# pxl-th/Trace.jl

Measured on AMD Instinct MI355X. Metric: Mray/s (all bounces), higher is better.
Workload: dtype f32

## Files before the change

trace.jl_amd/csrc/th_host.h:

```cpp
#pragma once
#include <hip/hip_runtime.h>

#include <algorithm>
#include <chrono>
#include <cstdarg>
#include <cstdio>
#include <cstdlib>
#include <cstring>
#include <memory>
#include <string>
#include <thread>
#include <vector>

#pragma GCC visibility push(default)
#include "../../include/tracehip.h"
#pragma GCC visibility pop
#include "th_bvh.h"
#include "th_kernels.h"
#include "th_trace2.h"
#include "th_trace8.h"
#ifdef TRHIP_EXPERIMENTS
#include "th_trace4.h"
#include "th_trace7.h"
#endif
#include "th_trace3c.h"
#include "th_comm.h"

using namespace th;

extern thread_local std::string g_init_error;

struct DevBuf {
    void* p = nullptr;
    size_t bytes = 0;
};

constexpr int kMaxPipes = 8;
struct Pipe {
    hipStream_t st = nullptr, st2 = nullptr;
    hipEvent_t ev_shade = nullptr, ev_any = nullptr, ev_any2 = nullptr, ev_done = nullptr;
    DevBuf q[2][3], sq[3], sq2[3], hits, counters, overflow[2];
};

struct Timer;
struct trhip_ctx {
    int device = 0;
    Timer* active_timer = nullptr;
    hipStream_t stream = nullptr;
    hipStream_t stream2 = nullptr;
    std::string err;
    int num_cu = 256;
    bool count_visits = false;
    bool timing = true;
    uint64_t batch_paths = 0;
    int pipelines = 1;
    Pipe pipes[kMaxPipes];
    uint32_t debug_trace_budget = 0;
    double bvh_device_ms = 0.0;
    int bvh_builder = -1;
    bool film_transpose = false;
    bool occluder_pretest = true;
    int stream2_priority = -1;
    bool leaf_kernel = true;
    int slab_margin_log2 = 14;
    int band_tile_rows = 0;
    uint32_t tiny_scene_prims = 16;
    int film_block = 5;
    bool film_relayout = true;
    bool warned_idle_accelerator = false;
    bool warned_fallback_cliff = false;
    double last_fallback_share = 0.0;
    int any_on_accelerator = -1;
    bool wide4 = true;
    bool leaf_queue = false;
    int node_layout = 0;
    bool film_swizzle = false;
    bool film_tiled = false;
    bool overlap = true;
    int compose_spheres = -1;
    int traversal = 3;
    bool leaf_sorted = false;
    bool film_fused = true;
    uint32_t last_L_layout = 0, last_L_npix = 1, last_L_spp = 1;
    bool trace3_spec = true;
    bool hybrid = true;
    bool trace7_cheap = true;
    DevBuf q[2][3], sq[3], hits, Lbuf, pfilm, counters, sensor, table, film, scratch[4], overflow, wh_L, wh_parent, wh_coef, wh_pdf, wh_flags, occl, film_Lt, surv_list, surv_counts;
    uint64_t last_L_count = 0;
    DevBuf sp_vp[7], sp_Ld, sp_tau, sp_radius, sp_N, sp_phi, sp_M, sp_counts, sp_starts, sp_entries, sp_grid, sp_ldist, sp_snap_M, sp_snap_phi, sp_snap_p, sp_snap_beta;
    DevBuf sp_terms, sp_rec[3], sp_rec_valid, sp_raysnap;
    DevBuf st_terms, st_tags[2], st_frozen, st_counts, st_list[2][2][7];
    int streaming = 0;
    uint32_t stream_budget_shift = 12;
    uint32_t stream_list_cap = 0;
    uint32_t stream_budget_min = 2048;
    uint64_t sppm_batch = 0;
    uint32_t sp_pixels = 0;
    int64_t sp_photons = 0;
    DevBuf film_side;
    DevBuf fdesc;
    DevBuf poison;
    DevBuf cert_cold;
    DevBuf aov_rec;
    DevBuf cb_rc;
    DevBuf ov8[2], fb_list[2], fb_counts[2];
    Comm comm;
};

struct HostPrim {
    uint32_t kind;
    float v[9];
    float n[9];
    uint32_t meta;
    uint32_t sphere_id;
};

inline void release(DevBuf& b);

struct SceneGeometry {
    uint64_t id = 0;
    int max_node_primitives = -1;
    std::vector<MaterialRec> materials;
    std::vector<float> base_colour;
    std::vector<HostPrim> prims;
    std::vector<float> prim_tan, prim_uv;
    std::vector<SphereRec> spheres;
    std::vector<HostAABB> sphere_bounds;
    FlatBVH bvh;
    FlatBVH acc;
    std::vector<uint32_t> occ_slots;
    std::vector<float> occ_boxes;
    DevBuf d_leaf_boxes;
    DevBuf d_nodes, d_prims, d_nrm, d_tan, d_shade, d_spheres, d_materials, d_base_colour, d_wnodes, d_w8nodes, d_w8tris;
    DevBuf d_acc_w4nodes;
    DevBuf d_acc_wnodes, d_acc_prims, d_slot_boxes, d_sphere_boxes, d_sphere_slots, d_sphere_cert;
    SceneGeometry() = default;
    SceneGeometry(const SceneGeometry&) = delete;
    SceneGeometry& operator=(const SceneGeometry&) = delete;
    ~SceneGeometry() {
        for (DevBuf* b : {&d_leaf_boxes, &d_nodes, &d_prims, &d_nrm, &d_tan, &d_shade, &d_spheres, &d_materials, &d_base_colour, &d_wnodes, &d_w8nodes, &d_w8tris, &d_acc_w4nodes, &d_acc_wnodes,
                          &d_acc_prims, &d_slot_boxes, &d_sphere_boxes, &d_sphere_slots, &d_sphere_cert})
            release(*b);
    }
// ... 222 lines not shown
```

trace.jl_amd/csrc/th_kernels.h:

```cpp
#pragma once
#include "th_device.h"

namespace th {

constexpr int kBlock = 256;
constexpr int kStackLds = 32;
constexpr int kStackSpill = 32;

struct PathQueue {
    float4* o;
    float4* d;
    float4* beta;
};
struct ShadowQueue {
    float4* o;
    float4* d;
    float4* c;
};
constexpr int kMaxDepth = 62;
constexpr int kSeg = 32;
constexpr uint32_t kSegGran = 256;
#ifndef TH_CTR_STRIDE
#define TH_CTR_STRIDE 32
#endif
// ... 228 lines not shown
    float tx_min = ((negx ? n1.x : n0.x) - o.x) * inv_d.x;
    float tx_max = ((negx ? n0.x : n1.x) - o.x) * inv_d.x;
    const float ty_min = ((negy ? n1.y : n0.y) - o.y) * inv_d.y;
    const float ty_max = ((negy ? n0.y : n1.y) - o.y) * inv_d.y;
    if (tx_min > ty_max || ty_min > tx_max) return false;
    if (ty_min > tx_min) tx_min = ty_min;
    if (ty_max > tx_max) tx_max = ty_max;
    const float tz_min = ((negz ? n1.z : n0.z) - o.z) * inv_d.z;
    const float tz_max = ((negz ? n0.z : n1.z) - o.z) * inv_d.z;
    if (tx_min > tz_max || tz_min > tx_max) return false;
    if (tz_min > tx_min) tx_min = tz_min;
    if (tz_max < tx_max) tx_max = tz_max;
    return tx_min < t_max && tx_max > 0.0f;
}

template <bool ANY, bool COUNT>
TH_D bool traverse(const DeviceScene& sc, f3 o, f3 d, float t_max, uint32_t (*stk)[kBlock], Hit* hit, uint32_t& n_nodes, uint32_t& n_prims) {
    const f3 inv_d = mk3(1.0f / d.x, 1.0f / d.y, 1.0f / d.z);
    const bool negx = d.x < 0.0f, negy = d.y < 0.0f, negz = d.z < 0.0f;
    uint32_t spill[kStackSpill];
    int sp = 0;
    uint32_t cur = 0;
    bool found = false;
    if (sc.n_nodes == 0) return false;
    const uint32_t tid = threadIdx.x;
    while (true) {
        const float4 n0 = sc.nodes[2 * cur], n1 = sc.nodes[2 * cur + 1];
        if (COUNT) n_nodes++;
        bool pop = true;
        if (slab_test(n0, n1, o, inv_d, negx, negy, negz, t_max)) {
            const uint32_t a = __float_as_uint(n0.w), flags = __float_as_uint(n1.w);
            if ((flags & 3u) == 3u) {
                const uint32_t cnt = flags >> 2;
                for (uint32_t k = 0; k < cnt; ++k) {
                    const uint32_t slot = a + k;
                    const float4 p0 = sc.prims[3 * slot];
                    const uint32_t meta = __float_as_uint(p0.w);
                    if (COUNT) n_prims++;
                    if (meta & PRIM_SPHERE) {
                        SphereHit sh;
                        if (sphere_intersect<false>(sc.spheres[__float_as_uint(p0.x)], o, d, t_max, sh)) {
                            if (ANY) return true;
                            t_max = sh.t;
                            found = true;
                            hit->prim = (int)slot;
                            hit->b1 = hit->b2 = 0.0f;
                        }
                    } else {
                        const float4 p1 = sc.prims[3 * slot + 1], p2 = sc.prims[3 * slot + 2];
                        TriTest tt;
                        if (tri_intersect<!ANY>(mk3(p0.x, p0.y, p0.z), mk3(p1.x, p1.y, p1.z), mk3(p2.x, p2.y, p2.z), o, d, t_max, &tt)) {
                            if (ANY) return true;
                            t_max = tt.t;
                            found = true;
                            hit->prim = (int)slot;
                            hit->b1 = tt.bary.x;
                            hit->b2 = tt.bary.y;
                        }
                    }
                }
            } else {
                const uint32_t axis = flags & 3u;
                const bool neg = axis == 0 ? negx : (axis == 1 ? negy : negz);
                const uint32_t far_child = neg ? cur + 1 : a;
                cur = neg ? a : cur + 1;
                if (sp < kStackLds)
                    stk[sp][tid] = far_child;
                else if (sp < kStackLds + kStackSpill)
                    spill[sp - kStackLds] = far_child;
                sp++;
                pop = false;
            }
        }
        if (pop) {
            if (sp == 0) break;
            sp--;
            cur = sp < kStackLds ? stk[sp][tid] : (sp < kStackLds + kStackSpill ? spill[sp - kStackLds] : 0u);
        }
    }
    if (!ANY) hit->t = t_max;
    return found;
}

template <bool COUNT>
__global__ __launch_bounds__(kBlock) void k_trace_closest(DeviceScene sc, SegQueue q, const float4* __restrict__ ro, const float4* __restrict__ rd, const float* __restrict__ tmax_or_null,
                                                          float4* __restrict__ hits, Counters* ctr) {
    __shared__ uint32_t stk[kStackLds][kBlock];
    __shared__ SegView sv;
    seg_load(q, sv);
    const uint32_t total = sv.prefix[kSeg];
    uint32_t nn = 0, np = 0;
    uint32_t seg = 0;
    for (uint32_t flat = blockIdx.x * kBlock + threadIdx.x; flat < total; flat += gridDim.x * kBlock) {
        uint32_t lb;
        seg_locate_from(sv, flat & ~63u, seg, lb);
        const uint32_t local = lb + (flat & 63u);
        if (local >= sv.count[seg]) continue;
        const uint32_t i = seg_phys(q, seg, local);
        const float4 o4 = ro[i], d4 = rd[i];
        Hit h;
        h.prim = -1;
        h.b1 = h.b2 = 0.0f;
        const float t0 = tmax_or_null ? tmax_or_null[i] : kInf;
        const bool found = traverse<false, COUNT>(sc, mk3(o4.x, o4.y, o4.z), mk3(d4.x, d4.y, d4.z), t0, stk, &h, nn, np);
        hits[i] = make_float4(found ? h.t : kInf, __int_as_float(found ? h.prim : -1), h.b1, h.b2);
    }
    if (ctr) {
        if (blockIdx.x == 0 && threadIdx.x == 0) atomicAdd(&ctr->closest_total, (unsigned long long)seg_total(sv));
        if (COUNT) {
            const unsigned long long sn = wave_sum(nn), spr = wave_sum(np);
            if (lane_id() == 0) {
                atomicAdd(&ctr->nodes_closest, sn);
                atomicAdd(&ctr->prims_closest, spr);
            }
        }
    }
}

template <bool COUNT>
__global__ __launch_bounds__(kBlock) void k_trace_any(DeviceScene sc, SegQueue q, const float4* __restrict__ ro, const float4* __restrict__ rd, const float4* __restrict__ contrib,
                                                      const float* __restrict__ tmax_or_null, float4* __restrict__ L, uint8_t* __restrict__ occluded, Counters* ctr) {
    __shared__ uint32_t stk[kStackLds][kBlock];
    __shared__ SegView sv;
    seg_load(q, sv);
    const uint32_t total = sv.prefix[kSeg];
    uint32_t nn = 0, np = 0;
    uint32_t seg = 0;
    for (uint32_t flat = blockIdx.x * kBlock + threadIdx.x; flat < total; flat += gridDim.x * kBlock) {
        uint32_t lb;
        seg_locate_from(sv, flat & ~63u, seg, lb);
        const uint32_t local = lb + (flat & 63u);
        if (local >= sv.count[seg]) continue;
        const uint32_t i = seg_phys(q, seg, local);
        const float4 o4 = ro[i], d4 = rd[i];
        const float t0 = tmax_or_null ? tmax_or_null[i] : kInf;
        const bool occ = traverse<true, COUNT>(sc, mk3(o4.x, o4.y, o4.z), mk3(d4.x, d4.y, d4.z), t0, stk, nullptr, nn, np);
        if (L) {
            const uint32_t slot = __float_as_uint(o4.w);
            if (!occ) {
                const float4 c = contrib[i];
                float4 l = L[slot];
                l.x += c.x;
                l.y += c.y;
                l.z += c.z;
                L[slot] = l;
            } else {
                const uint32_t poison = __float_as_uint(d4.w);
                if (poison) {
                    float4 l = L[slot];
                    const float nanv = __builtin_nanf("");
                    if (poison & 1u) l.x += nanv;
                    if (poison & 2u) l.y += nanv;
                    if (poison & 4u) l.z += nanv;
                    L[slot] = l;
                }
            }
        } else {
            occluded[i] = occ ? 1 : 0;
        }
    }
    if (ctr) {
        if (blockIdx.x == 0 && threadIdx.x == 0) atomicAdd(&ctr->shadow_total, (unsigned long long)seg_total(sv));
        if (COUNT) {
            const unsigned long long sn = wave_sum(nn), spr = wave_sum(np);
            if (lane_id() == 0) {
                atomicAdd(&ctr->nodes_shadow, sn);
                atomicAdd(&ctr->prims_shadow, spr);
            }
        }
    }
}

template <bool TRI_ONLY = false, bool TAN = true>
TH_D bool rebuild_shading(const DeviceScene& sc, int prim, f3 o, f3 d, Shading& sh, uint32_t& material, const float4* bary = nullptr, f3* fast_r = nullptr) {
    const float4* rec = sc.shade + 8 * (size_t)prim;
    const float4 p0 = rec[0], p1 = rec[1], p2 = rec[2];
    const float4 na = rec[3], nb = rec[4], nc = rec[5];
    const float4 cn = rec[6], cs = rec[7];
    const uint32_t meta = __float_as_uint(p0.w);
    material = meta & PRIM_MATERIAL_MASK;
    if (fast_r) *fast_r = mk3(na.w, nb.w, nc.w);
    if (!TRI_ONLY && (meta & PRIM_SPHERE)) {
        const SphereRec& s = sc.spheres[__float_as_uint(p0.x)];
        SphereHit h;
        if (!sphere_intersect<true>(s, o, d, kInf, h)) return false;
        sh = shade_sphere(s, h, d);
        return true;
    }
    const f3 v0 = mk3(p0.x, p0.y, p0.z), v1 = mk3(p1.x, p1.y, p1.z), v2 = mk3(p2.x, p2.y, p2.z);
    TriTest tt;
    if (bary)
        tt.bary = mk3(bary->z, bary->w, bary->x);
    else if (!tri_intersect<true>(v0, v1, v2, o, d, kInf, &tt))
        return false;
    const bool has_n = (meta & PRIM_HAS_NORMALS) != 0;
    const TriConstants tc{mk3(cn.x, cn.y, cn.z), mk3(cs.x, cs.y, cs.z)};
    const float4* tan = (TAN && sc.tri_tan && (meta & PRIM_HAS_TANGENTS)) ? sc.tri_tan + 3 * (size_t)prim : nullptr;
    sh = shade_triangle(v0, v1, v2, has_n, mk3(na.x, na.y, na.z), mk3(nb.x, nb.y, nb.z), mk3(nc.x, nc.y, nc.z), (meta & PRIM_FLIP) != 0, tt.bary, d, &tc, tan);
    return true;
}
template <int TH_ONE_COPY = 0> __global__ __launch_bounds__(kBlock) void k_shade_constants(float4* __restrict__ shade, const float4* __restrict__ prims, const float4* __restrict__ nrm, const float4* __restrict__ uv, uint32_t n_prims) {
    for (uint32_t k = blockIdx.x * kBlock + threadIdx.x; k < n_prims; k += gridDim.x * kBlock) {
        float4* rec = shade + 8 * (size_t)k;
        const float4 p0 = prims[3 * (size_t)k], p1 = prims[3 * (size_t)k + 1], p2 = prims[3 * (size_t)k + 2];
        rec[0] = p0;
        rec[1] = p1;
        rec[2] = p2;
        for (int j = 0; j < 3; ++j) rec[3 + j] = nrm[3 * (size_t)k + j];
        float4 c6 = make_float4(0.0f, 0.0f, 0.0f, 0.0f), c7 = c6;
        if (!(__float_as_uint(p0.w) & PRIM_SPHERE)) {
            float uvs[6];
            bool has_uv = false;
            if (uv) {
                const float4 a = uv[2 * (size_t)k], b = uv[2 * (size_t)k + 1];
                uvs[0] = a.x, uvs[1] = a.y, uvs[2] = a.z, uvs[3] = a.w, uvs[4] = b.x, uvs[5] = b.y;
                has_uv = b.z != 0.0f;
            }
            const TriConstants tc = triangle_constants(mk3(p0.x, p0.y, p0.z), mk3(p1.x, p1.y, p1.z), mk3(p2.x, p2.y, p2.z), has_uv ? uvs : nullptr);
            c6 = make_float4(tc.n.x, tc.n.y, tc.n.z, 0.0f);
            c7 = make_float4(tc.ss.x, tc.ss.y, tc.ss.z, 0.0f);
        }
        rec[6] = c6;
        rec[7] = c7;
    }
}

#ifndef TH_SHADE_WAVES
#define TH_SHADE_WAVES 4
#endif
struct ShadeStream {
    const uint32_t* tags_in;
    uint32_t* tags_out;
    uint32_t term_stride;
    uint8_t* poison;
};
struct ShadeOut {
    bool want_shadow, want_next;
    float4 so4, sd4, sc4, no4, nd4, nb4;
    uint32_t next_depth;
};
template <bool STREAM, bool FAST, bool TAN = true, bool DIRL = false>
TH_D void shade_vertex(const DeviceScene& sc, const PathQueue& qin, const float4* __restrict__ hits, float4* __restrict__ L, uint32_t i, int depth_fixed, int max_depth,
                       uint32_t hits_have_bary, const ShadeStream& ss, ShadeOut& out) {
    const float4 h4 = hits[i];
    const int prim = __float_as_int(h4.y);
    const float4 o4 = qin.o[i], d4 = qin.d[i], b4 = qin.beta[i];
    const int depth = STREAM ? (int)ss.tags_in[i] : depth_fixed;
    const uint32_t slot = STREAM ? (uint32_t)(depth - 1) * ss.term_stride + __float_as_uint(o4.w) : __float_as_uint(o4.w);
    const f3 o = mk3(o4.x, o4.y, o4.z), d = mk3(d4.x, d4.y, d4.z);
    f3 beta = mk3(b4.x, b4.y, b4.z);
    Shading sh;
    uint32_t material;
    f3 fast_r;
    if (!(rebuild_shading<FAST, TAN>(sc, prim, o, d, sh, material, hits_have_bary ? &h4 : nullptr, &fast_r) && material != PRIM_NO_MATERIAL)) return;
    const LobeSet& bsdf = sc.materials[FAST ? 0u : material].set[1];
    const bool lambert = FAST || bsdf_is_single_lambert(bsdf);
    Lobe lam;
    if (FAST) {
        lam.kind = LOBE_LAMBERT_R;
        lam.type = BSDF_DIFFUSE | BSDF_REFLECTION;
        lam.r[0] = fast_r.x;
        lam.r[1] = fast_r.y;
        lam.r[2] = fast_r.z;
    } else if (lambert) {
        lam = bsdf.lobe[0];
    }
    const uint64_t key = ((uint64_t)__float_as_uint(b4.w) << 32) | (uint64_t)__float_as_uint(d4.w);
    const uint32_t v = (uint32_t)(depth - 1);
    const f3 wo = -d;
    const uint32_t poison = ((isnan_(beta.x) || isinf_(beta.x)) ? 1u : 0u) | ((isnan_(beta.y) || isinf_(beta.y)) ? 2u : 0u) | ((isnan_(beta.z) || isinf_(beta.z)) ? 4u : 0u);
    bool direct_added = false;
    if (sc.n_lights > 0) {
        const int nl = (int)sc.n_lights;
        int ln = (int)__builtin_ceilf(ts_uniform(key, ts_vertex_dim(v, TS_V_LIGHT_PICK)) * (float)nl);
        if (ln > nl) ln = nl;
        if (ln < 1) ln = 1;
        const float light_pdf = 1.0f / (float)nl;
        const LightRec light = nl == 1 ? uniform_load(sc.lights, 0u) : sc.lights[ln - 1];
        const LightSample ls = sample_li<DIRL>(light, sh.p);
        if (ls.pdf > 0.0f && !is_black(ls.radiance)) {
            const f3 f = (lambert ? lambert_bsdf_f(lam, sh, sh.wo, ls.wi) : bsdf_f(bsdf, sh, sh.wo, ls.wi, BSDF_ALL & ~BSDF_SPECULAR)) * fabs_(dot(ls.wi, sh.ns));
            if (!is_black(f)) {
                const f3 fl = f * ls.radiance;
                const f3 Ld1 = splat3(0.0f) + (ls.pdf == 1.0f ? fl : fl / ls.pdf);
                const f3 Ld = light_pdf == 1.0f ? Ld1 : Ld1 / light_pdf;
                const f3 c = beta * Ld;
                const f3 lp = light_target<DIRL>(light, sh.p);
                const f3 dir = lp - sh.p;
                const f3 org = sh.p + 1e-6f * dir;
                const f3 cd = check_direction(dir);
                out.so4 = make_float4(org.x, org.y, org.z, __uint_as_float(slot));
                out.sd4 = make_float4(cd.x, cd.y, cd.z, __uint_as_float(poison));
                out.sc4 = make_float4(c.x, c.y, c.z, 0.0f);
                out.want_shadow = true;
                direct_added = true;
            }
        }
    }
    if (!direct_added && poison && ss.poison) {
        ss.poison[slot] |= (uint8_t)poison;
    } else if (!direct_added && poison) {
        float4 l = L[slot];
        const float nanv = __builtin_nanf("");
        if (poison & 1u) l.x += nanv;
        if (poison & 2u) l.y += nanv;
        if (poison & 4u) l.z += nanv;
        L[slot] = l;
    }
    if (depth < max_depth) {
        const f2 u{ts_uniform(key, ts_vertex_dim(v, TS_V_BSDF_U0)), ts_uniform(key, ts_vertex_dim(v, TS_V_BSDF_U1))};
        const BsdfSample bs = lambert ? lambert_bsdf_sample_f(lam, sh, wo, u) : bsdf_sample_f(bsdf, sh, wo, u, BSDF_ALL);
        if (!(bs.pdf == 0.0f || is_black(bs.f))) {
            beta = beta * (bs.f * fabs_(dot(bs.wi, sh.ns)) / bs.pdf);
            const float by = to_Y(beta);
            bool alive = true;
            if (by < 0.25f) {
                const float cont = jmin(1.0f, by);
                if (ts_uniform(key, ts_vertex_dim(v, TS_V_RR)) > cont)
                    alive = false;
                else
                    beta = beta / cont;
            }
            if (alive) {
                const f3 org = sh.p + 1e-6f * bs.wi;
                const f3 nd = check_direction(bs.wi);
                out.no4 = make_float4(org.x, org.y, org.z, o4.w);
                out.nd4 = make_float4(nd.x, nd.y, nd.z, d4.w);
                out.nb4 = make_float4(beta.x, beta.y, beta.z, b4.w);
                out.next_depth = (uint32_t)(depth + 1);
                out.want_next = true;
            }
        }
    }
}

template <bool STREAM, bool TAN = true, bool DIRL = false>
__global__ __launch_bounds__(kBlock) __attribute__((amdgpu_waves_per_eu(TH_SHADE_WAVES))) void k_shade_path(DeviceScene sc, const DeviceSensor* __restrict__ sep, PathQueue qin, PathQueue qout, ShadowQueue sq, uint32_t cap,
                                                       const float4* __restrict__ hits, float4* __restrict__ L, Counters* ctr, int row, int depth_fixed, int max_depth, uint32_t hits_have_bary,
                                                       ShadeStream ss) {
    __shared__ SegView sv;
    __shared__ uint32_t s_ring[kBlock / 64][128];
    const SegQueue qv{ctr->n_queue[row], cap, 0u};
    seg_load(qv, sv);
    const uint32_t total = sv.prefix[kSeg];
    const uint32_t lane = lane_id(), wv = threadIdx.x >> 6;
    const unsigned long long lt_mask = (1ull << lane) - 1ull;
    const uint32_t seg_out = ((blockIdx.x * kBlock + threadIdx.x) >> 6) % kSeg;
    uint32_t ring_head = 0, ring_cnt = 0;
    auto emit = [&](const ShadeOut& e) {
        uint32_t si, ni;
        wave_compact2(e.want_shadow, &ctr->n_shadow[row][seg_out * kCtrStride], e.want_next, &ctr->n_queue[row + 1][seg_out * kCtrStride], si, ni);
        si += seg_out * cap;
        ni += seg_out * cap;
        if (e.want_shadow) {
            sq.o[si] = e.so4;
            sq.d[si] = e.sd4;
            sq.c[si] = e.sc4;
        }
        if (e.want_next) {
            qout.o[ni] = e.no4;
            qout.d[ni] = e.nd4;
            qout.beta[ni] = e.nb4;
            if (STREAM) ss.tags_out[ni] = e.next_depth;
        }
    };
    uint32_t seg_in = 0;
    for (uint32_t flat = blockIdx.x * kBlock + threadIdx.x; flat < total; flat += gridDim.x * kBlock) {
        uint32_t lb;
        seg_locate_from(sv, flat & ~63u, seg_in, lb);
        const uint32_t local = lb + (flat & 63u);
        const uint32_t i = seg_in * cap + local;
        int cls = 0;
        if (local < sv.count[seg_in]) {
            const int prim = __float_as_int(hits[i].y);
            if (prim >= 0) {
                cls = (__float_as_uint(sc.shade[8 * (size_t)prim].w) & PRIM_FAST) ? 1 : 2;
            }
        }
        ShadeOut e;
        e.want_shadow = e.want_next = false;
        e.next_depth = 0;
        if (cls == 1) shade_vertex<STREAM, true, TAN, DIRL>(sc, qin, hits, L, i, depth_fixed, max_depth, hits_have_bary, ss, e);
        emit(e);
        const unsigned long long m2 = __ballot(cls == 2);
        if (m2) {
            if (cls == 2) s_ring[wv][(ring_head + ring_cnt + (uint32_t)__popcll(m2 & lt_mask)) & 127u] = i;
            ring_cnt += (uint32_t)__popcll(m2);
            __builtin_amdgcn_fence(__ATOMIC_ACQ_REL, "wavefront");
            if (ring_cnt >= 64u) {
                const uint32_t j = s_ring[wv][(ring_head + lane) & 127u];
                ShadeOut g;
                g.want_shadow = g.want_next = false;
                g.next_depth = 0;
                shade_vertex<STREAM, false, TAN, DIRL>(sc, qin, hits, L, j, depth_fixed, max_depth, hits_have_bary, ss, g);
                emit(g);
                ring_head = (ring_head + 64u) & 127u;
                ring_cnt -= 64u;
                __builtin_amdgcn_fence(__ATOMIC_ACQ_REL, "wavefront");
            }
        }
    }
    if (ring_cnt) {
        ShadeOut g;
        g.want_shadow = g.want_next = false;
        g.next_depth = 0;
        if (lane < ring_cnt) shade_vertex<STREAM, false, TAN, DIRL>(sc, qin, hits, L, s_ring[wv][(ring_head + lane) & 127u], depth_fixed, max_depth, hits_have_bary, ss, g);
        emit(g);
    }
}
template <int TH_ONE_COPY = 0> __global__ __launch_bounds__(kBlock) void k_fold_terms(const float4* __restrict__ terms, uint64_t n_slots, uint32_t n_depths, float4* __restrict__ L) {
    for (uint64_t i = (uint64_t)blockIdx.x * kBlock + threadIdx.x; i < n_slots; i += (uint64_t)gridDim.x * kBlock) {
        float4 l = make_float4(0.0f, 0.0f, 0.0f, 0.0f);
        for (uint32_t dd = 0; dd < n_depths; ++dd) {
            const float4 t = terms[(uint64_t)dd * n_slots + i];
            l.x += t.x;
            l.y += t.y;
            l.z += t.z;
        }
        L[i] = l;
    }
}
template <int TH_ONE_COPY = 0> __global__ __launch_bounds__(kBlock) void k_fill_u32(uint32_t* __restrict__ p, uint64_t n, uint32_t v) {
    for (uint64_t i = (uint64_t)blockIdx.x * kBlock + threadIdx.x; i < n; i += (uint64_t)gridDim.x * kBlock) p[i] = v;
}

template <int TH_ONE_COPY = 0> __global__ __launch_bounds__(kBlock) void k_film_transpose(const float4* __restrict__ L, uint32_t npix, uint32_t spp, float4* __restrict__ Lt) {
    const uint32_t groups = (npix + 63u) >> 6;
    const uint64_t chunks = (uint64_t)groups * spp;
    const uint32_t lane = threadIdx.x & 63u;
    for (uint64_t c = ((uint64_t)blockIdx.x * kBlock + threadIdx.x) >> 6; c < chunks; c += ((uint64_t)gridDim.x * kBlock) >> 6) {
        const uint32_t s = (uint32_t)(c / groups), g = (uint32_t)(c - (uint64_t)s * groups);
        const uint32_t pix = g * 64u + lane;
        if (pix < npix) Lt[film_index(1u, npix, spp, s, pix)] = L[(size_t)s * npix + pix];
    }
}
template <int TH_ONE_COPY = 0> __global__ __launch_bounds__(kBlock) void k_film_positions(const DeviceSensor* __restrict__ sep, uint64_t n, uint64_t seed, uint32_t sample_offset, float2* __restrict__ pfilm, uint32_t layout,
                                                           uint32_t spp) {
    const DeviceSensor& se = *sep;
    for (uint64_t slot = (uint64_t)blockIdx.x * kBlock + threadIdx.x; slot < n; slot += (uint64_t)gridDim.x * kBlock) {
        const SlotInfo si = slot_info(se, (uint32_t)slot);
        const uint64_t key = ts_stream_key(seed, si.px, si.py, sample_offset + si.sample);
        pfilm[film_index(layout, (uint32_t)(se.sb_w * se.band_rows), spp, si.sample, si.pix)] = make_float2((float)si.px + ts_uniform(key, TS_DIM_FILM_X), (float)si.py + ts_uniform(key, TS_DIM_FILM_Y));
    }
}
template <int TH_ONE_COPY = 0> __global__ __launch_bounds__(kBlock) void k_film_gather(const DeviceSensor* __restrict__ sep, const float* __restrict__ table, const float4* __restrict__ L,
                                                        const float2* __restrict__ pfilm, uint32_t spp, uint32_t layout, float4* __restrict__ out) {
    const DeviceSensor& se = *sep;
    const uint32_t npx = (uint32_t)(se.film_w * se.film_h);
    const uint32_t npix = (uint32_t)(se.sb_w * se.band_rows);
    const float rx = se.filter_radius[0], ry = se.filter_radius[1];
    const float inv_rx = 1.0f / rx, inv_ry = 1.0f / ry;
    for (uint32_t idx = blockIdx.x * kBlock + threadIdx.x; idx < npx; idx += gridDim.x * kBlock) {
        const int fy = (int)(idx / (uint32_t)se.film_w), fx = (int)(idx - (uint32_t)fy * (uint32_t)se.film_w);
        const float X = se.crop_min[0] + (float)fx, Y = se.crop_min[1] + (float)fy;
        int sx_lo = (int)__builtin_floorf(X - 1.5f - rx), sx_hi = (int)__builtin_ceilf(X + rx + 0.5f);
        int sy_lo = (int)__builtin_floorf(Y - 1.5f - ry), sy_hi = (int)__builtin_ceilf(Y + ry + 0.5f);
        sx_lo = max(sx_lo, se.sb_min[0]);
        sy_lo = max(sy_lo, se.sb_min[1]);
        sx_hi = min(sx_hi, se.sb_max[0]);
        sy_hi = min(sy_hi, se.sb_max[1]);
        f3 xyz = splat3(0.0f);
        float wsum = 0.0f;
        if (se.accumulate) {
            const float4 prev = out[idx];
            xyz = mk3(prev.x, prev.y, prev.z);
            wsum = prev.w;
        }
        if (sx_lo <= sx_hi && sy_lo <= sy_hi) {
            const int ty_lo = max((sy_lo - se.sb_min[1]) >> 4, se.band_ty0), ty_hi = min((sy_hi - se.sb_min[1]) >> 4, se.band_ty1);
            const int tx_lo = (sx_lo - se.sb_min[0]) >> 4, tx_hi = (sx_hi - se.sb_min[0]) >> 4;
            for (int ty = ty_lo; ty <= ty_hi; ++ty)
                for (int tx = tx_lo; tx <= tx_hi; ++tx) {
                    const float tbx0 = (float)se.sb_min[0] + (float)tx * 16.0f, tby0 = (float)se.sb_min[1] + (float)ty * 16.0f;
                    const float tbx1 = jmin(tbx0 + 15.0f, (float)se.sb_max[0]), tby1 = jmin(tby0 + 15.0f, (float)se.sb_max[1]);
                    const float bx0 = jmax(__builtin_ceilf(tbx0 - 0.5f - rx), se.crop_min[0]), by0 = jmax(__builtin_ceilf(tby0 - 0.5f - ry), se.crop_min[1]);
                    const float bx1 = jmin(__builtin_floorf(tbx1 - 0.5f + rx) + 1.0f, se.crop_max[0]), by1 = jmin(__builtin_floorf(tby1 - 0.5f + ry) + 1.0f, se.crop_max[1]);
                    if (X < bx0 || X > bx1 || Y < by0 || Y > by1) continue;
                    f3 csum = splat3(0.0f);
                    float fws = 0.0f;
                    const int y0 = max(sy_lo, (int)tby0), y1 = min(sy_hi, (int)tby1);
                    const int x0 = max(sx_lo, (int)tbx0), x1 = min(sx_hi, (int)tbx1);
                    for (int sy = y0; sy <= y1; ++sy)
                        for (int sx = x0; sx <= x1; ++sx) {
                            const uint32_t pix = (uint32_t)(sy - se.band_y0) * (uint32_t)se.sb_w + (uint32_t)(sx - se.sb_min[0]);
                            for (uint32_t s = 0; s < spp; ++s) {
                                const float2 pf = pfilm[film_index(layout, npix, spp, s, pix)];
                                const float dpx = pf.x - 0.5f, dpy = pf.y - 0.5f;
                                float p0x = __builtin_ceilf(dpx - rx), p0y = __builtin_ceilf(dpy - ry);
                                float p1x = __builtin_floorf(dpx + rx) + 1.0f, p1y = __builtin_floorf(dpy + ry) + 1.0f;
// ... 756 lines not shown
```

trace.jl_amd/csrc/th_trace2.h:

```cpp
#pragma once
#include "th_kernels.h"

namespace th {

#ifndef TH_STACK2_LDS
#define TH_STACK2_LDS 16
#endif
#ifndef TH_TRACE2_MIN_WAVES
#define TH_TRACE2_MIN_WAVES 1
#endif
constexpr int kStack2Lds = TH_STACK2_LDS;
constexpr int kStack2Total = 64;
#ifndef TH_TRACE3_WAVES_CLOSEST
#define TH_TRACE3_WAVES_CLOSEST 6
#endif
#ifndef TH_TRACE3_LDS_CLOSEST
#define TH_TRACE3_LDS_CLOSEST 12
#endif
#ifndef TH_TRACE3_WAVES_ANY
#define TH_TRACE3_WAVES_ANY 6
#endif
#ifndef TH_TRACE3_LDS_ANY
#define TH_TRACE3_LDS_ANY 10
#endif
constexpr int kStack3MinLds = TH_TRACE3_LDS_CLOSEST < TH_TRACE3_LDS_ANY ? TH_TRACE3_LDS_CLOSEST : TH_TRACE3_LDS_ANY;
constexpr int kStackMinLds = kStack2Lds < kStack3MinLds ? kStack2Lds : kStack3MinLds;
#ifdef TRHIP_EXPERIMENTS
constexpr int kStackSlabLevels = (kStack2Total - kStackMinLds) > 112 ? (kStack2Total - kStackMinLds) : 112;
#else
constexpr int kStackSlabLevels = kStack2Total - kStackMinLds;
#endif
constexpr uint32_t kRefNone = 0xffffffffu;
#ifndef TH_TRACE_REFILL
#define TH_TRACE_REFILL 12
#endif
constexpr int kChunk = 256;

struct WideScene {
    const float4* wnodes;
    float root_box[6];
    uint32_t root_ref, root_cnt;
    uint32_t n_wnodes;
    const float4* w4nodes;
    uint32_t n_w4nodes;
    float tight_scale;
    const uint32_t* leaf_order;
    uint32_t leaf_tight;
    float sphere_lag;
    uint32_t spec_spheres;
    float spec_box[8][6];
};

TH_D float slab_margin(const float* __restrict__ root_box, float scale, f3 o) {
    const float D = fmaxf(fmaxf(fmaxf(fabsf(root_box[0] - o.x), fabsf(root_box[3] - o.x)), fmaxf(fabsf(root_box[1] - o.y), fabsf(root_box[4] - o.y))),
                          fmaxf(fabsf(root_box[2] - o.z), fabsf(root_box[5] - o.z)));
    return D * scale;
}
TH_D bool slab_test2(float bx0, float by0, float bz0, float bx1, float by1, float bz1, f3 o, f3 inv_d, float em, bool tight, bool negx, bool negy, bool negz, float& tmin_out) {
    const float tx_min = ((negx ? bx1 : bx0) - o.x) * inv_d.x;
    const float tx_max = ((negx ? bx0 : bx1) - o.x) * inv_d.x;
    const float ty_min = ((negy ? by1 : by0) - o.y) * inv_d.y;
    const float ty_max = ((negy ? by0 : by1) - o.y) * inv_d.y;
    const float tz_min = ((negz ? bz1 : bz0) - o.z) * inv_d.z;
    const float tz_max = ((negz ? bz0 : bz1) - o.z) * inv_d.z;
    const bool miss_xy = (tx_min > ty_max) | (ty_min > tx_max);
    const float a = ty_min > tx_min ? ty_min : tx_min;
    const float b = ty_max > tx_max ? ty_max : tx_max;
    const bool miss_z = (a > tz_max) | (tz_min > b);
    const float t_in = tz_min > a ? tz_min : a;
    const float t_out = tz_max < b ? tz_max : b;
    const float exit_xy = fminf(__fmaf_rn(em, fabsf(inv_d.x), tx_max), __fmaf_rn(em, fabsf(inv_d.y), ty_max));
    const bool miss_tight = tight & ((__fmaf_rn(-em, fabsf(inv_d.z), tz_min) > exit_xy) | (exit_xy < 0.0f));
    tmin_out = t_in;
    return !(miss_xy | miss_z | miss_tight) & (t_out > 0.0f);
}

struct TraceOut {
    float4* hits;
    float4* L;
    const float4* contrib;
    uint8_t* occluded;
    uint32_t bary_mode;
    uint32_t far_hint;
    uint32_t zero_mode;
    uint32_t* zero_flag;
    uint32_t any_acc_hint;
};

struct SuspendList {
    float4* o;
    float4* d;
    float4* b;
    float4* trav;
    uint4* st;
    uint32_t* depth;
    uint2* stack;
    uint32_t cap;
};
struct StreamCtl {
    SuspendList in, out;
    const uint32_t* in_count;
    uint32_t* in_cursor;
    uint32_t* out_count;
    uint32_t budget_min;
    uint32_t budget_shift;
    const float4* beta_in;
    const uint32_t* depth_in;
    float4 *app_o, *app_d, *app_b, *app_hits;
    uint32_t* app_depth;
    uint32_t* app_counts;
    uint32_t app_cap;
};

template <bool ANY, bool COUNT, bool STREAM = false>
__global__ __launch_bounds__(kBlock, TH_TRACE2_MIN_WAVES) void k_trace2(DeviceScene sc, WideScene ws, SegQueue q, const float4* __restrict__ ro, const float4* __restrict__ rd, const float* __restrict__ tmax_or_null,
                                                   TraceOut out, uint32_t* __restrict__ work , uint2* __restrict__ overflow, Counters* ctr, uint32_t debug_budget,
                                                   StreamCtl sx = StreamCtl{}) {
    __shared__ uint32_t s_ref[kStack2Lds][kBlock];
    __shared__ float s_tmin[kStack2Lds][kBlock];
    __shared__ SegView sv;
    seg_load(q, sv);
    const uint32_t tid = threadIdx.x;
    const uint32_t gthreads = gridDim.x * kBlock;
    const uint32_t gtid = blockIdx.x * kBlock + tid;
    const uint32_t lane = lane_id();
    const unsigned long long lt_mask = (1ull << lane) - 1ull;

    bool active = false, exhausted = false;
    uint32_t wseg = (gtid >> 6) % kSeg, dry = 0, pool_next = 0, pool_end = 0;
    uint32_t idx = 0, cur = kRefNone, cur_cnt = 0;
    int sp = 0;
    uint32_t steps = 0;
    f3 o = splat3(0.0f), d = splat3(0.0f), inv_d = splat3(0.0f);
    float em = 0.0f;
    const bool tight_on = ws.tight_scale > 0.0f;
    RayShear shear{0, 0.0f, 0.0f, 0.0f};
    bool negx = false, negy = false, negz = false;
    float t_max = 0.0f, b1 = 0.0f, b2 = 0.0f, hx = 0.0f, slot_w = 0.0f, flag_w = 0.0f;
    int hit_prim = -1;
    bool found = false;
    uint32_t nn = 0, np = 0;
    bool resume_done = !STREAM, resumed = false, no_suspend = false;
    uint32_t rj = 0;
    const uint32_t n_in = STREAM ? min(*sx.in_count, sx.in.cap) : 0u;
    const uint32_t budget = STREAM && sx.budget_min ? max(sx.budget_min, sv.prefix[kSeg] >> sx.budget_shift) : 0u;

    while (true) {
        const unsigned long long idle = __ballot(!active);
        const uint32_t n_idle = (uint32_t)__popcll(idle);
        if (STREAM && !resume_done && n_idle > 0u) {
            uint32_t base = 0;
            if (lane == 0) base = atomicAdd(sx.in_cursor, n_idle);
            base = __shfl(base, 0);
            if (base >= n_in) {
                resume_done = true;
            } else {
                if (!active) {
                    const uint32_t j = base + (uint32_t)__popcll(idle & lt_mask);
                    if (j < n_in) {
                        const float4 o4 = sx.in.o[j], d4 = sx.in.d[j], tv = sx.in.trav[j];
                        const uint4 st = sx.in.st[j];
                        o = mk3(o4.x, o4.y, o4.z);
                        d = mk3(d4.x, d4.y, d4.z);
                        slot_w = o4.w;
                        flag_w = d4.w;
                        inv_d = mk3(1.0f / d.x, 1.0f / d.y, 1.0f / d.z);
                        em = slab_margin(ws.root_box, ws.tight_scale, o);
                        shear = ray_shear(d);
                        negx = d.x < 0.0f;
// ... 45 lines not shown
                    }
                }
                const uint32_t avail = pool_end - pool_next;
                if (avail && !active) {
                    const uint32_t rank = (uint32_t)__popcll(idle & lt_mask);
                    if (rank < avail) {
                        idx = seg_phys(q, wseg, pool_next + rank);
                        const float4 o4 = ro[idx], d4 = rd[idx];
                        o = mk3(o4.x, o4.y, o4.z);
                        d = mk3(d4.x, d4.y, d4.z);
                        slot_w = o4.w;
                        flag_w = d4.w;
                        inv_d = mk3(1.0f / d.x, 1.0f / d.y, 1.0f / d.z);
                        em = slab_margin(ws.root_box, ws.tight_scale, o);
                        shear = ray_shear(d);
                        negx = d.x < 0.0f;
                        negy = d.y < 0.0f;
                        negz = d.z < 0.0f;
                        t_max = tmax_or_null ? tmax_or_null[idx] : kInf;
                        sp = 0;
                        steps = 0;
                        found = false;
                        hit_prim = -1;
                        b1 = b2 = 0.0f;
                        resumed = false;
                        no_suspend = false;
                        active = true;
                        float tmin;
                        if (COUNT) nn++;
                        if (ws.root_ref != kRefNone && slab_test2(ws.root_box[0], ws.root_box[1], ws.root_box[2], ws.root_box[3], ws.root_box[4], ws.root_box[5], o, inv_d, em, false, negx, negy, negz, tmin) &&
                            tmin < t_max) {
                            cur = ws.root_ref;
                            cur_cnt = ws.root_cnt;
                        } else {
                            cur = kRefNone;
                        }
                    }
                }
                pool_next += min(n_idle, avail);
            }
            if (__ballot(active) == 0ull) {
                if (exhausted && resume_done) break;
                continue;
            }
        }
#pragma unroll 1
        for (int rep = 0; rep < 4; ++rep) {
            if (!active) continue;
            bool pop = true;
            bool finished = false;
            if (cur == kRefNone) {
                pop = true;
            } else if (cur_cnt > 0) {
                for (uint32_t k = 0; k < cur_cnt; ++k) {
                    const uint32_t slot = cur + k;
                    const float4 p0 = sc.prims[3 * slot];
                    const float4 p1 = sc.prims[3 * slot + 1], p2 = sc.prims[3 * slot + 2];
                    const uint32_t meta = __float_as_uint(p0.w);
                    if (COUNT) np++;
                    if (meta & PRIM_SPHERE) {
                        SphereHit sh;
                        if (sphere_intersect<false>(sc.spheres[__float_as_uint(p0.x)], o, d, t_max, sh)) {
                            if (ANY) {
                                found = true;
                                finished = true;
                                break;
                            }
                            t_max = sh.t;
                            found = true;
                            hit_prim = (int)slot;
                            b1 = b2 = 0.0f;
                            hx = sh.t;
                        }
                    } else {
                        TriTest tt;
                        if (!(meta & PRIM_DEGENERATE) && tri_intersect_sheared<!ANY>(mk3(p0.x, p0.y, p0.z), mk3(p1.x, p1.y, p1.z), mk3(p2.x, p2.y, p2.z), o, shear, t_max, &tt)) {
                            if (ANY) {
                                found = true;
                                finished = true;
                                break;
                            }
                            t_max = tt.t;
                            found = true;
                            hit_prim = (int)slot;
                            b1 = tt.bary.x;
                            b2 = tt.bary.y;
                            hx = out.bary_mode ? tt.bary.z : tt.t;
                        }
                    }
                }
            } else {
                const float4 a0 = ws.wnodes[4 * (size_t)cur], a1 = ws.wnodes[4 * (size_t)cur + 1], a2 = ws.wnodes[4 * (size_t)cur + 2], a3 = ws.wnodes[4 * (size_t)cur + 3];
                if (COUNT) nn += 2;
                if (debug_budget && ++steps > debug_budget) {
                    sp = 0;
                    cur = kRefNone;
                    continue;
                }
                if (STREAM && budget && !no_suspend && ++steps > budget) {
                    const uint32_t j = atomicAdd(sx.out_count, 1u);
                    if (j < sx.out.cap) {
                        sx.out.o[j] = make_float4(o.x, o.y, o.z, slot_w);
                        sx.out.d[j] = make_float4(d.x, d.y, d.z, flag_w);
                        if (ANY) {
                            sx.out.b[j] = resumed ? sx.in.b[rj] : out.contrib[idx];
                        } else {
                            sx.out.b[j] = resumed ? sx.in.b[rj] : sx.beta_in[idx];
                            sx.out.depth[j] = resumed ? sx.in.depth[rj] : sx.depth_in[idx];
                            if (!resumed) out.hits[idx] = make_float4(0.0f, __int_as_float(-2), 0.0f, 0.0f);
                        }
                        sx.out.trav[j] = make_float4(t_max, hx, b1, b2);
                        sx.out.st[j] = make_uint4(cur, cur_cnt, (uint32_t)sp, (found ? 0x80000000u : 0u) | (uint32_t)(hit_prim + 1));
                        for (int lvl = 0; lvl < sp && lvl < kStack2Total; ++lvl) {
                            uint2 e;
                            if (lvl < kStack2Lds)
                                e = make_uint2(s_ref[lvl][tid], __float_as_uint(s_tmin[lvl][tid]));
                            else
                                e = overflow[(size_t)(lvl - kStack2Lds) * gthreads + gtid];
                            sx.out.stack[(size_t)lvl * sx.out.cap + j] = e;
                        }
                        active = false;
                        continue;
                    }
                    no_suspend = true;
                }
                float tl, tr;
                const bool hl = slab_test2(a0.x, a0.y, a0.z, a0.w, a1.x, a1.y, o, inv_d, em, tight_on && !(__float_as_uint(a3.z) & 4u), negx, negy, negz, tl);
                const bool hr = slab_test2(a1.z, a1.w, a2.x, a2.y, a2.z, a2.w, o, inv_d, em, tight_on && !(__float_as_uint(a3.z) & 8u), negx, negy, negz, tr);
                const uint32_t lenc = __float_as_uint(a3.x), renc = __float_as_uint(a3.y), axis = __float_as_uint(a3.z) & 3u;
                const uint32_t lref = lenc & 0x00ffffffu, rref = renc & 0x00ffffffu, lcnt = lenc >> 24, rcnt = renc >> 24;
                const bool neg = axis == 0 ? negx : (axis == 1 ? negy : negz);
                const bool hn = neg ? hr : hl, hf = neg ? hl : hr;
                const float tn = neg ? tr : tl, tf = neg ? tl : tr;
                const uint32_t nref = neg ? rref : lref, fref = neg ? lref : rref, ncnt = neg ? rcnt : lcnt, fcnt = neg ? lcnt : rcnt;
                const bool near_ok = hn && tn < t_max;
                if (near_ok) {
                    if (hf) {
                        const uint32_t enc = fref | (fcnt << 24);
                        if (sp < kStack2Lds) {
                            s_ref[sp][tid] = enc;
                            s_tmin[sp][tid] = tf;
                        } else if (sp < kStack2Total) {
                            overflow[(size_t)(sp - kStack2Lds) * gthreads + gtid] = make_uint2(enc, __float_as_uint(tf));
                        }
                        sp++;
                    }
                    cur = nref;
                    cur_cnt = ncnt;
                    pop = false;
                } else if (hf && tf < t_max) {
                    cur = fref;
                    cur_cnt = fcnt;
                    pop = false;
                }
            }
            if (pop && !finished) {
                finished = true;
                while (sp > 0) {
                    sp--;
                    uint32_t enc;
                    float tm;
                    if (sp < kStack2Lds) {
                        enc = s_ref[sp][tid];
                        tm = s_tmin[sp][tid];
                    } else if (sp < kStack2Total) {
                        const uint2 e = overflow[(size_t)(sp - kStack2Lds) * gthreads + gtid];
                        enc = e.x;
// ... 55 lines not shown
    if (ctr) {
        if (blockIdx.x == 0 && threadIdx.x == 0) atomicAdd(ANY ? &ctr->shadow_total : &ctr->closest_total, (unsigned long long)seg_total(sv));
        if (COUNT) {
            const unsigned long long sn = wave_sum(nn), spr = wave_sum(np);
            if (lane_id() == 0) {
                atomicAdd(ANY ? &ctr->nodes_shadow : &ctr->nodes_closest, sn);
                atomicAdd(ANY ? &ctr->prims_shadow : &ctr->prims_closest, spr);
            }
        }
    }
}

#ifndef TH_TRACE_LEAF_WAVES
#define TH_TRACE_LEAF_WAVES 5
#endif
template <bool ANY, bool COUNT, bool FULL_ONLY>
__global__ __launch_bounds__(kBlock, FULL_ONLY ? TH_TRACE_LEAF_WAVES : 4) void k_trace_leaf(DeviceScene sc, WideScene ws, SegQueue q, const float4* __restrict__ ro, const float4* __restrict__ rd,
                                                                            const float* __restrict__ tmax_or_null, TraceOut out, Counters* ctr) {
    __shared__ SegView sv;
    seg_load(q, sv);
    const uint32_t total = sv.prefix[kSeg];
    const uint32_t first = ws.root_ref, cnt = ws.root_cnt;
    uint32_t nn = 0, np = 0;
    uint32_t seg = 0;
    for (uint32_t flat = blockIdx.x * kBlock + threadIdx.x; flat < total; flat += gridDim.x * kBlock) {
        uint32_t lb;
        seg_locate_from(sv, flat & ~63u, seg, lb);
        const uint32_t local = lb + (flat & 63u);
        const bool valid = local < sv.count[seg];
        const uint32_t idx = valid ? seg_phys(q, seg, local) : 0u;
        float4 o4 = make_float4(0.0f, 0.0f, 0.0f, 0.0f), d4 = make_float4(0.0f, 0.0f, 1.0f, 0.0f);
        if (valid) {
            o4 = ro[idx];
            d4 = rd[idx];
        }
        const f3 o = mk3(o4.x, o4.y, o4.z), d = mk3(d4.x, d4.y, d4.z);
        float t_max = (valid && tmax_or_null) ? tmax_or_null[idx] : kInf;
        bool live = false;
        if (valid) {
            const f3 inv_d = mk3(1.0f / d.x, 1.0f / d.y, 1.0f / d.z);
            float tmin;
            if (COUNT) nn++;
            live = slab_test2(ws.root_box[0], ws.root_box[1], ws.root_box[2], ws.root_box[3], ws.root_box[4], ws.root_box[5], o, inv_d, 0.0f, false, d.x < 0.0f, d.y < 0.0f, d.z < 0.0f, tmin) &&
                   tmin < t_max;
        }
        const RayShear shear = ray_shear(d);
        bool found = false;
        int hit_prim = -1;
        float hx = 0.0f, b1 = 0.0f, b2 = 0.0f;
#pragma unroll 1
        for (uint32_t k = 0; k < cnt; ++k) {
            if (__ballot(live) == 0ull) break;
            const uint32_t slot = first + k;
            const float4 p0 = uniform_load(sc.prims, 3 * slot);
            const uint32_t meta = __float_as_uint(p0.w);
            if (meta & PRIM_SPHERE) {
                const SphereRec sr = uniform_load(sc.spheres, __float_as_uint(p0.x));
                if (live) {
                    if (COUNT) np++;
                    SphereHit sh;
                    if (sphere_intersect<false, FULL_ONLY>(sr, o, d, t_max, sh)) {
                        found = true;
                        if (ANY) {
                            live = false;
                        } else {
                            t_max = sh.t;
                            hit_prim = (int)slot;
                            b1 = b2 = 0.0f;
                            hx = sh.t;
                        }
                    }
                }
            } else if (!(meta & PRIM_DEGENERATE)) {
                const float4 p1 = uniform_load(sc.prims, 3 * slot + 1), p2 = uniform_load(sc.prims, 3 * slot + 2);
                if (live) {
                    if (COUNT) np++;
                    TriTest tt;
                    if (tri_intersect_sheared<!ANY>(mk3(p0.x, p0.y, p0.z), mk3(p1.x, p1.y, p1.z), mk3(p2.x, p2.y, p2.z), o, shear, t_max, &tt)) {
                        found = true;
                        if (ANY) {
                            live = false;
                        } else {
                            t_max = tt.t;
                            hit_prim = (int)slot;
                            b1 = tt.bary.x;
                            b2 = tt.bary.y;
                            hx = out.bary_mode ? tt.bary.z : tt.t;
                        }
                    }
                }
            } else if (COUNT && live) {
                np++;
            }
        }
        if (!valid) continue;
        if (ANY) {
            if (out.L) {
                const uint32_t slot = __float_as_uint(o4.w);
                if (!found) {
                    const float4 c = out.contrib[idx];
                    float4 l = out.L[slot];
                    l.x += c.x;
                    l.y += c.y;
                    l.z += c.z;
                    out.L[slot] = l;
                } else {
                    const uint32_t poison = __float_as_uint(d4.w);
                    if (poison) {
                        float4 l = out.L[slot];
                        const float nanv = __builtin_nanf("");
                        if (poison & 1u) l.x += nanv;
                        if (poison & 2u) l.y += nanv;
                        if (poison & 4u) l.z += nanv;
                        out.L[slot] = l;
                    }
                }
            } else {
                out.occluded[idx] = found ? 1 : 0;
            }
        } else {
            out.hits[idx] = make_float4(found ? hx : kInf, __int_as_float(found ? hit_prim : -1), b1, b2);
        }
    }
    if (ctr) {
        if (blockIdx.x == 0 && threadIdx.x == 0) atomicAdd(ANY ? &ctr->shadow_total : &ctr->closest_total, (unsigned long long)seg_total(sv));
        if (COUNT) {
            const unsigned long long sn = wave_sum(nn), spr = wave_sum(np);
            if (lane_id() == 0) {
                atomicAdd(ANY ? &ctr->nodes_shadow : &ctr->nodes_closest, sn);
                atomicAdd(ANY ? &ctr->prims_shadow : &ctr->prims_closest, spr);
            }
        }
    }
}

#ifndef TH_LEAF_STAGE_A
#define TH_LEAF_STAGE_A 3
#endif
template <bool COUNT, bool FULL_ONLY>
__global__ __launch_bounds__(kBlock, FULL_ONLY ? TH_TRACE_LEAF_WAVES : 4) void k_any_leaf(DeviceScene sc, WideScene ws, SegQueue q, const float4* __restrict__ ro, const float4* __restrict__ rd,
                                                                          const float* __restrict__ tmax_or_null, TraceOut out, Counters* ctr) {
    __shared__ SegView sv;
    __shared__ uint32_t s_ring[kBlock / 64][128];
    seg_load(q, sv);
    const uint32_t total = sv.prefix[kSeg];
    const uint32_t first = ws.root_ref, cnt = ws.root_cnt;
    const uint32_t lane = lane_id(), wv = threadIdx.x >> 6;
    const unsigned long long lt_mask = (1ull << lane) - 1ull;
    const uint32_t n_a = min(cnt, (uint32_t)TH_LEAF_STAGE_A);
    uint32_t nn = 0, np = 0;
    uint32_t ring_head = 0, ring_cnt = 0;
    auto run = [&](uint32_t idx, f3 o, f3 d, uint32_t k0, uint32_t k1, bool& live) {
        const float t_max = (live && tmax_or_null) ? tmax_or_null[idx] : kInf;
        const RayShear shear = ray_shear(d);
        bool found = false;
#pragma unroll 1
        for (uint32_t k = k0; k < k1; ++k) {
            if (__ballot(live) == 0ull) break;
            const uint32_t slot = first + (ws.leaf_order ? uniform_load(ws.leaf_order, k) : k);
            const float4 p0 = uniform_load(sc.prims, 3 * slot);
            const uint32_t meta = __float_as_uint(p0.w);
            if (COUNT && lane == 0) np++;
            if (meta & PRIM_SPHERE) {
                const SphereRec sr = uniform_load(sc.spheres, __float_as_uint(p0.x));
                if (live) {
                    SphereHit sh;
                    if (sphere_intersect<false, FULL_ONLY>(sr, o, d, t_max, sh)) {
// ... 539 lines not shown
                }
#endif
                if (SPEC && spec_ok && pend == kRefNone && cur != kRefNone && cur_cnt > 0) {
                    pend = cur | (cur_cnt << 24);
                    cur = kRefNone;
                    cur_cnt = 0;
                }
#if TH_TRACE3_LEAF_PREFETCH
                if (cur != kRefNone && cur_cnt > 0) {
                    const float4* rec = sc.prims + 3 * (size_t)cur;
                    asm volatile("s_waitcnt vmcnt(0)\n\tglobal_load_dword %0, %2, off\n\tglobal_load_dword %1, %2, off offset:44" : "+v"(pf0), "+v"(pf1) : "v"(rec) : "memory");
                }
#endif
            }
#ifdef TH_DIAG_PHASES
            ph_cyc[2] += __builtin_readcyclecounter() - ph_t_node;
            ph_lan[2] += (unsigned long long)__popcll(ph_node_m);
            ph_cnt[2] += 1ull;
#endif
            const uint32_t n_desc = (uint32_t)__popcll(__ballot(active && cur_cnt == 0 && !(SPEC && pend != kRefNone && cur == kRefNone && sp == 0)));
            if (n_desc <= (uint32_t)TH_TRACE3_LEAF_WAIT) break;
        }
#ifdef TH_DIAG_PHASES
        const unsigned long long ph_leaf_m = __ballot(active && ((SPEC && pend != kRefNone) || (cur != kRefNone && cur_cnt > 0)));
        const unsigned long long ph_t_leaf = __builtin_readcyclecounter();
#endif
        const bool has_pend = SPEC && pend != kRefNone;
        if (active && (has_pend || (cur != kRefNone && cur_cnt > 0))) {
            bool hit_any = false;
            const uint32_t leaf_ref = has_pend ? (pend & 0x00ffffffu) : cur, leaf_cnt = has_pend ? (pend >> 24) : cur_cnt;
#if TH_TRACE3_INLINE_POP
            uint32_t top_enc = kRefNone;
            float top_tm = kInf;
            if (sp > 0) {
                if (sp - 1 < kLds) {
                    top_enc = s_ref[sp - 1][tid];
                    top_tm = s_tmin[sp - 1][tid];
                } else if (sp - 1 < kStack2Total) {
                    const uint2 e = overflow[(size_t)(sp - 1 - kLds) * gthreads + gtid];
                    top_enc = e.x;
                    top_tm = __uint_as_float(e.y);
                }
            }
#endif
            for (uint32_t k = 0; k < leaf_cnt; ++k) {
                const uint32_t slot = leaf_ref + k;
                const float4 p0 = sc.prims[3 * slot];
                const float4 p1 = sc.prims[3 * slot + 1], p2 = sc.prims[3 * slot + 2];
#if TH_TRACE3_LEAF_BURST
                asm volatile("" ::"v"(p1.x), "v"(p1.y), "v"(p1.z), "v"(p2.x), "v"(p2.y), "v"(p2.z));
#endif
#ifdef TH_DIAG_PHASES
                asm volatile("s_waitcnt vmcnt(0)" ::: "memory");
                ph_load += __builtin_readcyclecounter() - ph_t_leaf;
#endif
                const uint32_t meta = __float_as_uint(p0.w);
                if (COUNT) np++;
                if (meta & PRIM_SPHERE) {
                    const float4 d4 = rd[idx];
                    const f3 d = mk3(d4.x, d4.y, d4.z);
                    SphereHit sh;
                    const bool sphere_hit = sphere_intersect<false, FULL_ONLY>(sc.spheres[__float_as_uint(p0.x)], o, d, t_max, sh);
                    inv_d = mk3(1.0f / d.x, 1.0f / d.y, 1.0f / d.z);
                    em = slab_margin(ws.root_box, ws.tight_scale, o);
                    shear = ray_shear(d);
                    if (sphere_hit) {
                        if (ANY) {
                            hit_any = true;
                            break;
                        }
                        t_max = sh.t;
                        found = true;
                        out.hits[idx] = make_float4(sh.t, __int_as_float((int)slot), 0.0f, 0.0f);
                    }
                } else {
                    TriTest tt;
                    if (!(meta & PRIM_DEGENERATE) && tri_intersect_sheared<!ANY>(mk3(p0.x, p0.y, p0.z), mk3(p1.x, p1.y, p1.z), mk3(p2.x, p2.y, p2.z), o, shear, t_max, &tt)) {
                        if (ANY) {
                            hit_any = true;
                            break;
                        }
                        t_max = tt.t;
                        found = true;
                        out.hits[idx] = make_float4(out.bary_mode ? tt.bary.z : tt.t, __int_as_float((int)slot), tt.bary.x, tt.bary.y);
                    }
                }
            }
            bool keep_cur = false;
            if (has_pend) {
                pend = kRefNone;
                if (cur != kRefNone && cur_cnt > 0) {
                    if (cur_tm < t_max) pend = cur | (cur_cnt << 24);
                } else if (cur != kRefNone) {
                    keep_cur = true;
                }
            }
            if (!keep_cur) {
                cur = kRefNone;
                cur_cnt = 0;
            }
            if (ANY && hit_any) {
                found = true;
                sp = 0;
            }
#if TH_TRACE3_INLINE_POP
            else if (!keep_cur && sp > 0) {
                sp--;
                if (top_tm < t_max && sp < kStack2Total) {
                    cur = top_enc & 0x00ffffffu;
                    cur_cnt = top_enc >> 24;
                    if (SPEC) cur_tm = top_tm;
                    if (SPEC && spec_ok && pend == kRefNone && cur_cnt > 0) {
                        pend = cur | (cur_cnt << 24);
                        cur = kRefNone;
                        cur_cnt = 0;
                    }
                }
            }
#endif
        }
#ifdef TH_DIAG_PHASES
        ph_cyc[3] += __builtin_readcyclecounter() - ph_t_leaf;
        ph_lan[3] += (unsigned long long)__popcll(ph_leaf_m);
        ph_cnt[3] += 1ull;
#endif
    }
#ifdef TH_DIAG_PHASES
    {
        float f = (float)ph_load;
        for (int off = 32; off > 0; off >>= 1) f = fmaxf(f, __shfl_xor(f, off));
        ph_load = (unsigned long long)f;
    }
    if (!ANY && lane == 0) atomicAdd(&g_phase[12], ph_load);
    if (!ANY && lane == 0)
        for (int k4 = 0; k4 < 4; ++k4) {
            atomicAdd(&g_phase[3 * k4], ph_cyc[k4]);
            atomicAdd(&g_phase[3 * k4 + 1], ph_lan[k4]);
            atomicAdd(&g_phase[3 * k4 + 2], ph_cnt[k4]);
        }
#endif
    if (ctr) {
        if (blockIdx.x == 0 && threadIdx.x == 0 && !q.no_total) atomicAdd(ANY ? &ctr->shadow_total : &ctr->closest_total, (unsigned long long)seg_total(sv));
        if (COUNT) {
            const unsigned long long sn = wave_sum(nn), spr = wave_sum(np);
            if (lane_id() == 0) {
                atomicAdd(ANY ? &ctr->nodes_shadow : &ctr->nodes_closest, sn);
                atomicAdd(ANY ? &ctr->prims_shadow : &ctr->prims_closest, spr);
            }
        }
    }
}

}
```

trace.jl_amd/csrc/th_trace3c.h:

```cpp
#pragma once
#include "th_trace2.h"
#include "th_trace8.h"

namespace th {

#ifndef TH_TRACE3C_WAVES
#define TH_TRACE3C_WAVES 6
#endif
#ifndef TH_TRACE3C_AXIS_LESS
#define TH_TRACE3C_AXIS_LESS 0
#endif
#ifndef TH_TRACE3C_REFILL
#define TH_TRACE3C_REFILL TH_TRACE_REFILL
#endif
#ifndef TH_TRACE3C_LDS
#define TH_TRACE3C_LDS 11
#endif
#ifndef TH_TRACE3C_LEAF_WAIT
#define TH_TRACE3C_LEAF_WAIT 32
#endif
#ifndef TH_TRACE3C_POP_MIN
#define TH_TRACE3C_POP_MIN 8
#endif
#ifndef TH_TRACE3C_MAX_A
// ... 391 lines not shown
                    bl = hl ? (AXIS ? gl : vl) : kInf;
                    br = hr ? (AXIS ? gr_ : vr) : kInf;
                    const uint32_t axis = meta & 3u;
                    neg = axis == 0 ? negx : (axis == 1 ? negy : negz);
                    const float bn = neg ? br : bl, bf = neg ? bl : br;
                    const float vn = AXIS ? (neg ? vr : vl) : bn, vf = AXIS ? (neg ? vl : vr) : bf;
                    const uint32_t nenc = neg ? renc : lenc, fenc = neg ? lenc : renc;
                    const bool go_n = bn < t_cull, go_f = bf < t_cull;
                    if (go_n && go_f) {
                        if (sp < kLds) {
                            s_stk[sp][tid] = make_uint2(fenc, __float_as_uint(vf));
                        } else if (sp < kStack2Total) {
                            overflow[(size_t)(sp - kLds) * gthreads + gtid] = make_uint2(fenc, __float_as_uint(vf));
                        }
                        sp++;
                    }
                    any_child = go_n || go_f;
                    cur = any_child ? (go_n ? nenc : fenc) : kRefNone;
                    ex_new = go_n ? vn : vf;
                }
                if (!any_child && sp > 0) {
                    sp--;
                    const float t_pop = AXIS ? __fmaf_rn(growth(), inv_max(), t_cull) : t_cull;
                    if (top_tm < t_pop && sp < kStack2Total) {
                        cur = top_enc;
                        ex_new = top_tm;
                    }
                }
                s_ex[tid] = ex_new;
            }
#ifdef TH_DIAG_PHASES
            ph_cyc[2] += __builtin_readcyclecounter() - ph_t_node;
            ph_lan[2] += (unsigned long long)__popcll(ph_node_m);
            ph_cnt[2] += 1ull;
#endif
            const uint32_t n_desc = (uint32_t)__popcll(__ballot(active && (cur < kLeafBit || cur == kRefNone)));
            if (n_desc <= (uint32_t)TH_TRACE3C_LEAF_WAIT) break;
        }
#ifdef TH_DIAG_PHASES
        const unsigned long long ph_leaf_m = __ballot(active && cur >= kLeafBit && cur != kRefNone);
        const unsigned long long ph_t_leaf = __builtin_readcyclecounter();
#endif
        if (active && cur >= kLeafBit && cur != kRefNone) {
            bool flagged = false;
            const uint32_t leaf_ref = cur & 0x00ffffffu, leaf_cnt = cur >> 24;
            uint32_t top_enc = kRefNone;
            float top_tm = kInf;
            if (sp > 0) {
                if (sp - 1 < kLds) {
                    const uint2 e = s_stk[sp - 1][tid];
                    top_enc = e.x;
                    top_tm = __uint_as_float(e.y);
                } else if (sp - 1 < kStack2Total) {
                    const uint2 e = overflow[(size_t)(sp - 1 - kLds) * gthreads + gtid];
                    top_enc = e.x;
                    top_tm = __uint_as_float(e.y);
                }
            }
            for (uint32_t k = 0; k < leaf_cnt; ++k) {
                const uint32_t slot = leaf_ref + k;
                const float4 p0 = sc.prims[3 * slot];
                const float4 p1 = sc.prims[3 * slot + 1], p2 = sc.prims[3 * slot + 2];
                asm volatile("" ::"v"(p1.x), "v"(p1.y), "v"(p1.z), "v"(p1.w), "v"(p2.x), "v"(p2.y), "v"(p2.z), "v"(p2.w));
                const uint32_t meta = __float_as_uint(p0.w);
                if (COUNT) np++;
                TriTest tt;
                if (!(meta & (PRIM_SPHERE | PRIM_DEGENERATE)) && tri_intersect_sheared<true>(mk3(p0.x, p0.y, p0.z), mk3(p1.x, p1.y, p1.z), mk3(p2.x, p2.y, p2.z), o, shear, t_lim, &tt)) {
                    bool counts = true;
                    const uint32_t st = s_st[tid];
                    if (st >> 8) {
                        const uint32_t ow = __float_as_uint(p2.w) >> (3u * ((st >> 8) - 1u));
                        const uint32_t ax = ow & 3u;
                        const bool second = (ow & 4u) != 0u;
                        counts = ax == 3u ? second : (second != (ax == 0u ? negx : (ax == 1u ? negy : negz)));
                    }
                    if (counts) {
                        const float dt = margin_t();
                        if (!(tt.t <= t_lim - 4.0f * dt) || !(s_ex[tid] <= tt.t + dt)) {
                            if (COUNT && !flagged) why = 2u;
                            flagged = true;
                        } else if (!flagged) {
                            t_lim = tt.t + 2.0f * dt;
                            s_st[tid] = st | 3u;
                            out.hits[s_idx[tid]] = make_float4(out.bary_mode ? tt.bary.z : tt.t, p1.w , tt.bary.x, tt.bary.y);
                        }
                    }
                }
            }
            cur = kRefNone;
            if (flagged) {
                active = false;
                to_fb = true;
                sp = 0;
                if (COUNT) n_why[why & 3u]++;
            } else if (sp > 0) {
                sp--;
                const float t_pop = t_lim + (AXIS ? __fmaf_rn(growth(), inv_max(), mb) : mb);
                if (top_tm < t_pop && sp < kStack2Total) {
                    cur = top_enc;
                    s_ex[tid] = top_tm;
                }
            }
        }
#ifdef TH_DIAG_PHASES
        ph_cyc[3] += __builtin_readcyclecounter() - ph_t_leaf;
        ph_lan[3] += (unsigned long long)__popcll(ph_leaf_m);
        ph_cnt[3] += 1ull;
#endif
    }
#ifdef TH_DIAG_PHASES
    if (lane == 0)
        for (int k4 = 0; k4 < 4; ++k4) {
            atomicAdd(&g_phase[3 * k4], ph_cyc[k4]);
            atomicAdd(&g_phase[3 * k4 + 1], ph_lan[k4]);
            atomicAdd(&g_phase[3 * k4 + 2], ph_cnt[k4]);
        }
#endif
    if (ctr) {
        if (blockIdx.x == 0 && threadIdx.x == 0 && !q.no_total) atomicAdd(&ctr->closest_total, (unsigned long long)seg_total(sv));
        if (lane_id() == 0 && n_fb) atomicAdd(&ctr->fallback_total, (unsigned long long)n_fb);
        if (COUNT) {
            const unsigned long long sn = wave_sum(nn), spr = wave_sum(np);
            if (lane_id() == 0) {
                atomicAdd(&ctr->nodes_closest, sn);
                atomicAdd(&ctr->prims_closest, spr);
            }
            for (int k = 0; k < 4; ++k) {
                const unsigned long long w = wave_sum(n_why[k]);
                if (lane_id() == 0 && w) atomicAdd(&ctr->fallback_why[k], w);
            }
        }
    }
}
#undef negx
#undef negy
#undef negz

#ifndef TH_TRACE_LEAF_C_WAVES
#define TH_TRACE_LEAF_C_WAVES TH_TRACE_LEAF_WAVES
#endif
#ifndef TH_LEAF_C_DEFER
#define TH_LEAF_C_DEFER 2
#endif
template <bool COUNT, bool FULL_ONLY>
__global__ __launch_bounds__(kBlock, FULL_ONLY ? TH_TRACE_LEAF_C_WAVES : 4) void k_trace_leaf_c(DeviceScene sc , WideScene ws ,
                                                                              CertScene cs, SegQueue q, const float4* __restrict__ ro, const float4* __restrict__ rd,
                                                                              const float* __restrict__ tmax_or_null, TraceOut out, Counters* ctr, FallbackList fb) {
    __shared__ SegView sv;
    seg_load(q, sv);
    const uint32_t total = sv.prefix[kSeg];
    const uint32_t first = ws.root_ref, cnt = ws.root_cnt;
    const uint32_t gtid = blockIdx.x * kBlock + threadIdx.x;
    uint32_t nn = 0, np = 0;
    unsigned long long n_fb = 0;
    uint32_t seg = 0;
    for (uint32_t flat = gtid; flat < total; flat += gridDim.x * kBlock) {
        uint32_t lb;
        seg_locate_from(sv, flat & ~63u, seg, lb);
        const uint32_t local = lb + (flat & 63u);
        const bool valid = local < sv.count[seg];
        uint32_t idx = valid ? seg_phys(q, seg, local) : 0u;
        if (valid && q.indirect) idx = q.indirect[idx];
        float4 o4 = make_float4(0.0f, 0.0f, 0.0f, 0.0f), d4 = make_float4(0.0f, 0.0f, 1.0f, 0.0f);
        if (valid) {
            o4 = ro[idx];
            d4 = rd[idx];
        }
        const f3 o = mk3(o4.x, o4.y, o4.z), d = mk3(d4.x, d4.y, d4.z);
        const f3 inv_d = mk3(1.0f / d.x, 1.0f / d.y, 1.0f / d.z);
        const bool negx = d.x < 0.0f, negy = d.y < 0.0f, negz = d.z < 0.0f;
        float t_max = (valid && tmax_or_null) ? tmax_or_null[idx] : kInf;
        const RayShear shear = ray_shear(d, inv_d);
        const float D = slab_margin(ws.root_box, 1.0f, o);
        const float dt = kCertDt * D * fabsf(shear.sz);
        float t_lim = t_max + 2.0f * dt;
        bool live = false, flagged = false;
        if (valid) {
            const bool plain = d.x != 0.0f && d.y != 0.0f && d.z != 0.0f && dt < kInf && fabsf(o.x) < kInf && fabsf(o.y) < kInf && fabsf(o.z) < kInf && fabsf(inv_d.x) < kInf && fabsf(inv_d.y) < kInf &&
                               fabsf(inv_d.z) < kInf && t_max == t_max;
            float tmin;
            if (COUNT) nn++;
            if (!plain)
                flagged = true;
            else
                live = slab_test2(ws.root_box[0], ws.root_box[1], ws.root_box[2], ws.root_box[3], ws.root_box[4], ws.root_box[5], o, inv_d, 0.0f, false, negx, negy, negz, tmin) && tmin < t_lim;
        }
        bool found = false, sticky = false;
#if TH_LEAF_C_DEFER == 2
        uint32_t best_slot = 0u;
        float4 best_r4 = make_float4(kInf, __int_as_float(-1), 0.0f, 0.0f);
#pragma unroll 1
        for (uint32_t ks = 0; ks < cs.n_spheres; ++ks) {
            if (__ballot(live) == 0ull) break;
            const uint32_t slot = uniform_load(cs.sphere_slots, ks);
            const float4 p0 = uniform_load(sc.prims, 3 * slot);
            const SphereRec sr = uniform_load(sc.spheres, __float_as_uint(p0.x));
            if (live) {
                if (COUNT) np++;
                float t_c = 0.0f;
                const int r = sphere_candidate_c<FULL_ONLY>(sr, o, d, t_lim, t_c);
                if (r == 2) {
                    flagged = true;
                } else if (r != 0) {
                    if (sticky || !(t_c <= t_max - 2.0f * dt)) {
                        flagged = true;
                    } else {
                        t_max = t_c;
                        t_lim = t_c + 2.0f * dt;
                        found = true;
                        sticky = r == 3;
                        best_slot = slot;
                        best_r4 = make_float4(t_c, __int_as_float((int)slot), 0.0f, 0.0f);
                    }
                }
                if (flagged) live = false;
            }
        }
#pragma unroll 1
        for (uint32_t k = 0; k < cnt; ++k) {
            if (__ballot(live) == 0ull) break;
            const uint32_t slot = first + k;
            const float4 p0 = uniform_load(sc.prims, 3 * slot);
            const uint32_t meta = __float_as_uint(p0.w);
            if (meta & (PRIM_SPHERE | PRIM_DEGENERATE)) {
                if (COUNT && live && (meta & PRIM_DEGENERATE)) np++;
                continue;
            }
            const float4 p1 = uniform_load(sc.prims, 3 * slot + 1), p2 = uniform_load(sc.prims, 3 * slot + 2);
            if (COUNT && live) np++;
            TriTest tt;
            tt.t = 0.0f;
            tt.bary = mk3(0.0f, 0.0f, 0.0f);
            const bool hit = live && tri_intersect_sheared<true>(mk3(p0.x, p0.y, p0.z), mk3(p1.x, p1.y, p1.z), mk3(p2.x, p2.y, p2.z), o, shear, t_lim, &tt);
            const bool acc = hit && !sticky && (tt.t <= t_max - 2.0f * dt);
            flagged = flagged || (hit && !acc);
            live = live && !(hit && !acc);
            found = found || acc;
            t_max = acc ? tt.t : t_max;
            t_lim = acc ? tt.t + 2.0f * dt : t_lim;
            best_slot = acc ? slot : best_slot;
            best_r4.x = acc ? (out.bary_mode ? tt.bary.z : tt.t) : best_r4.x;
            best_r4.y = acc ? __int_as_float((int)slot) : best_r4.y;
            best_r4.z = acc ? tt.bary.x : best_r4.z;
            best_r4.w = acc ? tt.bary.y : best_r4.w;
        }
        if (valid && found && !flagged) {
            const float* bx = cs.slot_boxes + 6 * (size_t)best_slot;
            float ex;
            if (COUNT) nn++;
            if (!slab_test2(bx[0], bx[1], bx[2], bx[3], bx[4], bx[5], o, inv_d, 0.0f, false, negx, negy, negz, ex) || !(ex <= (sticky ? 0.0f : t_max + dt))) flagged = true;
        }
        if (valid && found && !flagged) out.hits[idx] = best_r4;
#elif TH_LEAF_C_DEFER
        uint32_t best_slot = 0u;
        float4 best_r4 = make_float4(kInf, __int_as_float(-1), 0.0f, 0.0f);
#pragma unroll 1
        for (uint32_t k = 0; k < cnt; ++k) {
            if (__ballot(live) == 0ull) break;
            const uint32_t slot = first + k;
            const float4 p0 = uniform_load(sc.prims, 3 * slot);
            const uint32_t meta = __float_as_uint(p0.w);
            float t_c = 0.0f;
            float4 r4 = make_float4(0.0f, __int_as_float((int)slot), 0.0f, 0.0f);
            bool cand = false, inside = false;
            if (meta & PRIM_SPHERE) {
                const SphereRec sr = uniform_load(sc.spheres, __float_as_uint(p0.x));
                if (live) {
                    if (COUNT) np++;
                    const int r = sphere_candidate_c<FULL_ONLY>(sr, o, d, t_lim, t_c);
                    if (r == 1 || r == 3) {
                        cand = true;
                        inside = r == 3;
                        r4.x = t_c;
                    } else if (r == 2) {
                        flagged = true;
                    }
                }
            } else if (!(meta & PRIM_DEGENERATE)) {
                const float4 p1 = uniform_load(sc.prims, 3 * slot + 1), p2 = uniform_load(sc.prims, 3 * slot + 2);
                if (live) {
                    if (COUNT) np++;
                    TriTest tt;
                    if (tri_intersect_sheared<true>(mk3(p0.x, p0.y, p0.z), mk3(p1.x, p1.y, p1.z), mk3(p2.x, p2.y, p2.z), o, shear, t_lim, &tt)) {
                        cand = true;
                        t_c = tt.t;
                        r4 = make_float4(out.bary_mode ? tt.bary.z : tt.t, __int_as_float((int)slot), tt.bary.x, tt.bary.y);
                    }
                }
            } else if (COUNT && live) {
                np++;
            }
            if (cand) {
                if (sticky || !(t_c <= t_max - 2.0f * dt)) {
                    flagged = true;
                } else {
                    t_max = t_c;
                    t_lim = t_c + 2.0f * dt;
                    found = true;
                    sticky = inside;
                    best_slot = slot;
                    best_r4 = r4;
                }
            }
            if (flagged) live = false;
        }
        if (valid && found && !flagged) {
            const float* bx = cs.slot_boxes + 6 * (size_t)best_slot;
            float ex;
            if (COUNT) nn++;
            if (!slab_test2(bx[0], bx[1], bx[2], bx[3], bx[4], bx[5], o, inv_d, 0.0f, false, negx, negy, negz, ex) || !(ex <= (sticky ? 0.0f : t_max + dt))) flagged = true;
        }
        if (valid && found && !flagged) out.hits[idx] = best_r4;
#else
#pragma unroll 1
        for (uint32_t k = 0; k < cnt; ++k) {
            if (__ballot(live) == 0ull) break;
            const uint32_t slot = first + k;
            const float4 p0 = uniform_load(sc.prims, 3 * slot);
            const uint32_t meta = __float_as_uint(p0.w);
            float t_c = 0.0f;
            float4 r4 = make_float4(0.0f, __int_as_float((int)slot), 0.0f, 0.0f);
            bool cand = false, inside = false, clipped = false;
            if (meta & PRIM_SPHERE) {
                const SphereRec sr = uniform_load(sc.spheres, __float_as_uint(p0.x));
                if (live) {
                    if (COUNT) np++;
                    const int r = sphere_candidate_c<FULL_ONLY>(sr, o, d, t_lim, t_c);
                    if (r == 1 || r == 3) {
                        cand = true;
                        inside = r == 3;
                        r4.x = t_c;
                    } else if (r == 2) {
                        clipped = true;
                    }
                }
            } else if (!(meta & PRIM_DEGENERATE)) {
                const float4 p1 = uniform_load(sc.prims, 3 * slot + 1), p2 = uniform_load(sc.prims, 3 * slot + 2);
                if (live) {
                    if (COUNT) np++;
                    TriTest tt;
                    if (tri_intersect_sheared<true>(mk3(p0.x, p0.y, p0.z), mk3(p1.x, p1.y, p1.z), mk3(p2.x, p2.y, p2.z), o, shear, t_lim, &tt)) {
                        cand = true;
                        t_c = tt.t;
                        r4 = make_float4(out.bary_mode ? tt.bary.z : tt.t, __int_as_float((int)slot), tt.bary.x, tt.bary.y);
                    }
                }
            } else if (COUNT && live) {
                np++;
            }
            if (__ballot(cand | clipped) != 0ull) {
                const float* bx = cs.slot_boxes + 6 * (size_t)slot;
                const float b0 = uniform_load(bx, 0), b1 = uniform_load(bx, 1), b2 = uniform_load(bx, 2), b3 = uniform_load(bx, 3), b4 = uniform_load(bx, 4), b5 = uniform_load(bx, 5);
                float ex;
                if (COUNT && cand) nn++;
                if ((cand | clipped) && slab_test2(b0, b1, b2, b3, b4, b5, o, inv_d, 0.0f, false, negx, negy, negz, ex)) {
                    if (clipped || sticky || !(t_c <= t_max - 2.0f * dt) || !(ex <= t_c + dt)) {
                        flagged = true;
                    } else {
                        t_max = t_c;
                        t_lim = t_c + 2.0f * dt;
                        found = true;
                        sticky = inside;
                        out.hits[idx] = r4;
                    }
                }
            }
            if (flagged) live = false;
        }
#endif
        const bool to_fb = valid && flagged;
        if (__ballot(to_fb) != 0ull) {
            uint32_t fseg = __builtin_amdgcn_readfirstlane((gtid >> 6) % kSeg);
            bool pending = to_fb;
            for (int tries = 0; tries < kSeg && __ballot(pending) != 0ull; ++tries) {
                const uint32_t j = wave_compact(pending, &fb.counts[fseg * kCtrStride]);
                if (pending && j < fb.cap) {
                    fb.list[(size_t)fseg * fb.cap + j] = idx;
                    n_fb++;
                    pending = false;
                }
                fseg = (fseg + 1) % kSeg;
            }
        }
        if (valid && !flagged && !found) out.hits[idx] = make_float4(kInf, __int_as_float(-1), 0.0f, 0.0f);
    }
    if (ctr) {
        if (blockIdx.x == 0 && threadIdx.x == 0 && !q.no_total) atomicAdd(&ctr->closest_total, (unsigned long long)seg_total(sv));
        const unsigned long long sfb = wave_sum(n_fb);
        if (lane_id() == 0 && sfb) atomicAdd(&ctr->fallback_total, sfb);
        if (COUNT) {
            const unsigned long long sn = wave_sum(nn), spr = wave_sum(np);
            if (lane_id() == 0) {
                atomicAdd(&ctr->nodes_closest, sn);
                atomicAdd(&ctr->prims_closest, spr);
            }
        }
    }
}

template <bool COUNT, bool FULL_ONLY>
__global__ __launch_bounds__(kBlock, FULL_ONLY ? TH_TRACE_LEAF_WAVES : 4) void k_any_leaf_c(DeviceScene sc, WideScene ws, CertScene cs, SegQueue q, const float4* __restrict__ ro,
                                                                            const float4* __restrict__ rd, const float* __restrict__ tmax_or_null, TraceOut out, Counters* ctr,
                                                                            FallbackList fb) {
    __shared__ SegView sv;
    __shared__ uint32_t s_ring[kBlock / 64][128];
    seg_load(q, sv);
    const uint32_t total = sv.prefix[kSeg];
    const uint32_t first = ws.root_ref, cnt = ws.root_cnt;
    const uint32_t lane = lane_id(), wv = threadIdx.x >> 6;
    const uint32_t gtid = blockIdx.x * kBlock + threadIdx.x;
    const unsigned long long lt_mask = (1ull << lane) - 1ull;
    const uint32_t n_a = min(cnt, (uint32_t)TH_LEAF_STAGE_A);
    uint32_t nn = 0, np = 0;
    unsigned long long n_fb = 0;
    uint32_t ring_head = 0, ring_cnt = 0;
    auto run = [&](uint32_t idx, f3 o, f3 d, uint32_t k0, uint32_t k1, bool& live) {
        const float t_max = (live && tmax_or_null) ? tmax_or_null[idx] : kInf;
        const RayShear shear = ray_shear(d);
        const f3 inv_d = mk3(1.0f / d.x, 1.0f / d.y, 1.0f / d.z);
        bool found = false;
#pragma unroll 1
        for (uint32_t k = k0; k < k1; ++k) {
            if (__ballot(live) == 0ull) break;
            const uint32_t slot = first + (ws.leaf_order ? uniform_load(ws.leaf_order, k) : k);
            const float4 p0 = uniform_load(sc.prims, 3 * slot);
            const uint32_t meta = __float_as_uint(p0.w);
            const float* bx = cs.slot_boxes + 6 * (size_t)slot;
// ... 133 lines not shown
```

trace.jl_amd/csrc/th_trace3c4.h:

```cpp
#pragma once
#include "th_trace3c.h"

namespace th {

#ifndef TH_TRACE3C4_WAVES
#define TH_TRACE3C4_WAVES 5
#endif
#ifndef TH_TRACE3C4_FETCH_BURST
#define TH_TRACE3C4_FETCH_BURST 1
#endif
#ifndef TH_TRACE3C4_REFILL_LEAN
#define TH_TRACE3C4_REFILL_LEAN 1
#endif
#ifndef TH_TRACE3C4_LEAF_ONE
#define TH_TRACE3C4_LEAF_ONE 1
#endif
#ifndef TH_TRACE3C4_LDS
#define TH_TRACE3C4_LDS 12
#endif
#ifndef TH_TRACE3C4_CHEAP
#define TH_TRACE3C4_CHEAP 0
#endif
#ifndef TH_TRACE3C4_TOP
#define TH_TRACE3C4_TOP 36
// ... 441 lines not shown
                    if (top_tm < t_pop && sp < kStack2Total) {
                        cur = top_enc;
                        ex_new = top_tm;
                    }
                }
#if !TH_TRACE3C4_CHEAP
                s_ex[tid] = ex_new;
#else
                (void)ex_new;
#endif
            }
#ifdef TH_DIAG_PHASES
            ph_cyc[2] += __builtin_readcyclecounter() - ph_t_node;
            ph_lan[2] += (unsigned long long)__popcll(ph_node_m);
            ph_cnt[2] += 1ull;
#endif
            const uint32_t n_desc = (uint32_t)__popcll(__ballot(active && (cur < kLeafBit || cur == kRefNone)));
            if (n_desc <= (uint32_t)TH_TRACE3C_LEAF_WAIT) break;
        }
#ifdef TH_DIAG_PHASES
        const unsigned long long ph_leaf_m = __ballot(active && cur >= kLeafBit && cur != kRefNone);
        const unsigned long long ph_t_leaf = __builtin_readcyclecounter();
#endif
        if (active && cur >= kLeafBit && cur != kRefNone) {
            bool flagged = false;
            const uint32_t leaf_ref = cur & 0x00ffffffu, leaf_cnt = cur >> 24;
            uint32_t top_enc = kRefNone;
            float top_tm = kInf;
            if (sp > 0 && (!TH_TRACE3C4_LEAF_ONE || leaf_cnt == 1u)) {
                if (sp - 1 < kLds) {
                    const uint2 e = s_stk[sp - 1][tid];
                    top_enc = e.x;
                    top_tm = __uint_as_float(e.y);
                } else if (sp - 1 < kStack2Total) {
                    const uint2 e = overflow[(size_t)(sp - 1 - kLds) * gthreads + gtid];
                    top_enc = e.x;
                    top_tm = __uint_as_float(e.y);
                }
            }
            for (uint32_t k = 0; k < (TH_TRACE3C4_LEAF_ONE ? 1u : leaf_cnt); ++k) {
                const uint32_t slot = leaf_ref + k;
                const float4 p0 = sc.prims[3 * slot];
                const float4 p1 = sc.prims[3 * slot + 1], p2 = sc.prims[3 * slot + 2];
                asm volatile("" ::"v"(p1.x), "v"(p1.y), "v"(p1.z), "v"(p1.w), "v"(p2.x), "v"(p2.y), "v"(p2.z), "v"(p2.w));
                const uint32_t meta = __float_as_uint(p0.w);
                if (COUNT) np++;
                TriTest tt;
                if (!(meta & (PRIM_SPHERE | PRIM_DEGENERATE)) && tri_intersect_sheared<true>(mk3(p0.x, p0.y, p0.z), mk3(p1.x, p1.y, p1.z), mk3(p2.x, p2.y, p2.z), o, shear, t_lim, &tt)) {
                    bool counts = true;
                    const uint32_t st = s_st[tid];
                    if (st >> 8) {
                        const uint32_t ow = __float_as_uint(p2.w) >> (3u * ((st >> 8) - 1u));
                        const uint32_t ax = ow & 3u;
                        const bool second = (ow & 4u) != 0u;
                        counts = ax == 3u ? second : (second != (ax == 0u ? negx : (ax == 1u ? negy : negz)));
                    }
#if TH_TRACE3C4_CHEAP
                    float ex_leaf = 0.0f;
                    bool unverified = false;
                    if (counts) {
                        const v2f bx = v2f{amin3(p0.x, p1.x, p2.x), amax3(p0.x, p1.x, p2.x)}, by = v2f{amin3(p0.y, p1.y, p2.y), amax3(p0.y, p1.y, p2.y)}, bz = v2f{amin3(p0.z, p1.z, p2.z), amax3(p0.z, p1.z, p2.z)};
                        const v2f p_a = v2f{o.x, o.y}, p_b = v2f{o.z, inv_d.x}, p_c = v2f{inv_d.y, inv_d.z};
                        const v2f Tx = pk_mul_h<1>(pk_sub_h<0>(bx, p_a), p_b), Ty = pk_mul_h<0>(pk_sub_h<1>(by, p_a), p_c), Tz = pk_mul_h<1>(pk_sub_h<0>(bz, p_b), p_c);
                        const float nx = amin(Tx.x, Tx.y), fx = amax(Tx.x, Tx.y), ny = amin(Ty.x, Ty.y), fy = amax(Ty.x, Ty.y), nz = amin(Tz.x, Tz.y), fz = amax(Tz.x, Tz.y);
                        const float a = amax(nx, ny), b = amax(fx, fy);
                        ex_leaf = amax(a, nz);
                        const float t_out = amin(fz, b);
                        const bool ref = !(nx > fy) && !(ny > fx) && !(a > fz) && !(nz > b) && (t_out > 0.0f);
                        const float exit_xy = amin(fx + em * fabsf(inv_d.x), fy + em * fabsf(inv_d.y));
                        unverified = !(ref && !(nz - em * fabsf(inv_d.z) > exit_xy) && !(exit_xy < 0.0f));
                    }
#else
                    const float ex_leaf = s_ex[tid];
                    const bool unverified = false;
#endif
                    if (counts) {
                        const float dt = margin_t();
                        if (unverified || !(tt.t <= t_lim - 4.0f * dt) || !(ex_leaf <= tt.t + dt)) {
                            if (COUNT && !flagged) why = 2u;
                            flagged = true;
                        } else if (!flagged) {
                            t_lim = tt.t + 2.0f * dt;
                            s_st[tid] = st | 3u;
                            out.hits[s_idx[tid]] = make_float4(out.bary_mode ? tt.bary.z : tt.t, p1.w , tt.bary.x, tt.bary.y);
                        }
                    }
                }
            }
            cur = (TH_TRACE3C4_LEAF_ONE && !flagged && leaf_cnt > 1u) ? ((leaf_ref + 1u) | ((leaf_cnt - 1u) << 24)) : kRefNone;
            if (cur != kRefNone) {
            } else if (flagged) {
                active = false;
                to_fb = true;
                sp = 0;
                if (COUNT) n_why[why & 3u]++;
            } else if (sp > 0) {
                sp--;
                const float t_pop = t_lim + mb;
                if (top_tm < t_pop && sp < kStack2Total) {
                    cur = top_enc;
#if !TH_TRACE3C4_CHEAP
                    s_ex[tid] = top_tm;
#endif
                }
            }
        }
#ifdef TH_DIAG_PHASES
        ph_cyc[3] += __builtin_readcyclecounter() - ph_t_leaf;
        ph_lan[3] += (unsigned long long)__popcll(ph_leaf_m);
        ph_cnt[3] += 1ull;
#endif
    }
#ifdef TH_DIAG_PHASES
    if (lane == 0)
        for (int k4 = 0; k4 < 4; ++k4) {
            atomicAdd(&g_phase[3 * k4], ph_cyc[k4]);
            atomicAdd(&g_phase[3 * k4 + 1], ph_lan[k4]);
            atomicAdd(&g_phase[3 * k4 + 2], ph_cnt[k4]);
        }
#endif
    if (ctr) {
        if (blockIdx.x == 0 && threadIdx.x == 0 && !q.no_total) atomicAdd(&ctr->closest_total, (unsigned long long)seg_total(sv));
        if (lane_id() == 0 && n_fb) atomicAdd(&ctr->fallback_total, (unsigned long long)n_fb);
        if (COUNT) {
            const unsigned long long sn = wave_sum(nn), spr = wave_sum(np);
            if (lane_id() == 0) {
                atomicAdd(&ctr->nodes_closest, sn);
                atomicAdd(&ctr->prims_closest, spr);
            }
            for (int k = 0; k < 4; ++k) {
                const unsigned long long w = wave_sum(n_why[k]);
                if (lane_id() == 0 && w) atomicAdd(&ctr->fallback_why[k], w);
            }
        }
    }
}
#undef negx
#undef negy
#undef negz

}
```

trace.jl_amd/csrc/tu_api.hip:

```cpp
#include "th_host.h"

thread_local std::string g_init_error;

extern "C" {

int trhip_version(void) { return 3001; }

int trhip_init(trhip_ctx** out, int device_id) {
    if (!out) return fail(nullptr, TRHIP_ERR_INVALID, "ctx out pointer is null");
    *out = nullptr;
    int n = 0;
    hipError_t e = hipGetDeviceCount(&n);
    if (e != hipSuccess || n == 0) return fail(nullptr, TRHIP_ERR_HIP, "no HIP device available (%s): libtracehip has no CPU fallback", hipGetErrorString(e));
    if (device_id < 0 || device_id >= n) return fail(nullptr, TRHIP_ERR_INVALID, "device %d out of range (%d devices)", device_id, n);
    hipDeviceProp_t prop;
    if ((e = hipGetDeviceProperties(&prop, device_id)) != hipSuccess) return fail(nullptr, TRHIP_ERR_HIP, "hipGetDeviceProperties: %s", hipGetErrorString(e));
    if (std::strncmp(prop.gcnArchName, "gfx950", 6) != 0) return fail(nullptr, TRHIP_ERR_HIP, "device %d is %s; this library is built for gfx950 only", device_id, prop.gcnArchName);
    auto ctx = new trhip_ctx();
    ctx->device = device_id;
    ctx->num_cu = prop.multiProcessorCount;
    if ((e = hipSetDevice(device_id)) != hipSuccess || (e = hipStreamCreate(&ctx->stream)) != hipSuccess || (e = hipStreamCreate(&ctx->stream2)) != hipSuccess) {
        delete ctx;
        return fail(nullptr, TRHIP_ERR_HIP, "stream creation failed: %s", hipGetErrorString(e));
    }
// ... 86 lines not shown
    if (!ctx || !id128) return fail(ctx, TRHIP_ERR_INVALID, "null argument");
    if (n_ranks < 1 || rank < 0 || rank >= n_ranks) return fail(ctx, TRHIP_ERR_INVALID, "rank %d of %d", rank, n_ranks);
    if (ctx->comm.comm) return fail(ctx, TRHIP_ERR_INVALID, "the context already has a communicator (trhip_comm_destroy first)");
    RcclApi* api = rccl_api();
    if (!api->error.empty()) return fail(ctx, TRHIP_ERR_UNSUPPORTED, "%s", api->error.c_str());
    HIP_TRY(ctx, hipSetDevice(ctx->device));
    ncclUniqueId id;
    std::memcpy(&id, id128, sizeof id);
    NCCL_TRY(ctx, api->CommInitRank(&ctx->comm.comm, n_ranks, id, rank));
    ctx->comm.rank = rank;
    ctx->comm.n_ranks = n_ranks;
    return 0;
}
int trhip_comm_destroy(trhip_ctx* ctx) {
    if (!ctx) return fail(ctx, TRHIP_ERR_INVALID, "null argument");
    if (ctx->comm.comm) {
        (void)hipSetDevice(ctx->device);
        NCCL_TRY(ctx, rccl_api()->CommDestroy(ctx->comm.comm));
    }
    ctx->comm = Comm{};
    return 0;
}
int trhip_comm_rank(const trhip_ctx* ctx, int* rank, int* n_ranks) {
    if (!ctx) return TRHIP_ERR_INVALID;
    if (rank) *rank = ctx->comm.rank;
    if (n_ranks) *n_ranks = ctx->comm.n_ranks;
    return 0;
}
static int film_collective(trhip_ctx* ctx, void* d_xyzw, uint64_t n_pixels, int root, bool all) {
    if (!ctx || !d_xyzw) return fail(ctx, TRHIP_ERR_INVALID, "null argument");
    if (!ctx->comm.comm) return 0;
    if (!all && (root < 0 || root >= ctx->comm.n_ranks)) return fail(ctx, TRHIP_ERR_INVALID, "root %d of %d ranks", root, ctx->comm.n_ranks);
    HIP_TRY(ctx, hipSetDevice(ctx->device));
    RcclApi* api = rccl_api();
    if (all)
        NCCL_TRY(ctx, api->AllReduce(d_xyzw, d_xyzw, (size_t)n_pixels * 4, ncclFloat32, ncclSum, ctx->comm.comm, ctx->stream));
    else
        NCCL_TRY(ctx, api->Reduce(d_xyzw, d_xyzw, (size_t)n_pixels * 4, ncclFloat32, ncclSum, root, ctx->comm.comm, ctx->stream));
    HIP_TRY(ctx, hipStreamSynchronize(ctx->stream));
    return 0;
}
int trhip_film_reduce(trhip_ctx* ctx, void* d_xyzw, uint64_t n_pixels, int root) { return film_collective(ctx, d_xyzw, n_pixels, root, false); }
int trhip_film_allreduce(trhip_ctx* ctx, void* d_xyzw, uint64_t n_pixels) { return film_collective(ctx, d_xyzw, n_pixels, 0, true); }

#ifdef TRHIP_EXPERIMENTS
static constexpr bool kExperiments = true;
#else
static constexpr bool kExperiments = false;
#endif
static const char* const kNeedsExperiments = "needs the EXPERIMENTS build of the library (-DTRHIP_EXPERIMENTS): not in the default binary";
static bool experiments_only(const char* name, int64_t value) {
    if (!std::strcmp(name, "traversal")) return value == 4 || value == 6 || value == 7;
    if (!std::strcmp(name, "bvh_builder")) return value == 1;
    if (!std::strcmp(name, "leaf_sorted") || !std::strcmp(name, "leaf_queue")) return value != 0;
    return false;
}
int trhip_option_in_build(const char* name, int64_t value) { return (name && (kExperiments || !experiments_only(name, value))) ? 1 : 0; }
int trhip_set_option(trhip_ctx* ctx, const char* name, int64_t value) {
    if (!ctx || !name) return fail(ctx, TRHIP_ERR_INVALID, "null argument");
    if (!std::strcmp(name, "count_visits"))
        ctx->count_visits = value != 0;
    else if (!std::strcmp(name, "timing"))
        ctx->timing = value != 0;
    else if (!std::strcmp(name, "debug_trace_budget"))
        ctx->debug_trace_budget = (uint32_t)value;
    else if (!std::strcmp(name, "streaming"))
        ctx->streaming = value < 0 ? -1 : (value != 0 ? 1 : 0);
    else if (!std::strcmp(name, "stream_budget_shift"))
        ctx->stream_budget_shift = (uint32_t)std::max<int64_t>(0, std::min<int64_t>(31, value));
    else if (!std::strcmp(name, "stream_list_cap"))
        ctx->stream_list_cap = (uint32_t)std::max<int64_t>(0, value);
    else if (!std::strcmp(name, "stream_budget_min"))
        ctx->stream_budget_min = (uint32_t)std::max<int64_t>(1, value);
    else if (!std::strcmp(name, "sppm_batch"))
        ctx->sppm_batch = (uint64_t)std::max<int64_t>(0, value);
    else if (!std::strcmp(name, "bvh_builder")) {
        if (value == 1 && !kExperiments) return fail(ctx, TRHIP_ERR_UNSUPPORTED, "bvh_builder = 1 (the linear BVH) %s", kNeedsExperiments);
        ctx->bvh_builder = value < 0 ? -1 : (value > 4 ? 4 : (int)value);
    }
    else if (!std::strcmp(name, "hybrid"))
        ctx->hybrid = value != 0;
    else if (!std::strcmp(name, "film_transpose"))
        ctx->film_transpose = value != 0;
    else if (!std::strcmp(name, "band_tile_rows"))
        ctx->band_tile_rows = (int)std::max<int64_t>(0, value);
    else if (!std::strcmp(name, "compose_spheres"))
        ctx->compose_spheres = value < 0 ? -1 : (value != 0 ? 1 : 0);
    else if (!std::strcmp(name, "occluder_pretest"))
        ctx->occluder_pretest = value != 0;
    else if (!std::strcmp(name, "stream2_priority"))
        ctx->stream2_priority = (int)value;
    else if (!std::strcmp(name, "leaf_sorted")) {
        if (value != 0 && !kExperiments) return fail(ctx, TRHIP_ERR_UNSUPPORTED, "leaf_sorted %s", kNeedsExperiments);
        ctx->leaf_sorted = value != 0;
    }
    else if (!std::strcmp(name, "film_fused"))
        ctx->film_fused = value != 0;
    else if (!std::strcmp(name, "trace3_spec"))
        ctx->trace3_spec = value != 0;
    else if (!std::strcmp(name, "trace7_cheap"))
        ctx->trace7_cheap = value != 0;
    else if (!std::strcmp(name, "leaf_kernel"))
        ctx->leaf_kernel = value != 0;
    else if (!std::strcmp(name, "slab_margin_log2"))
        ctx->slab_margin_log2 = (int)std::max<int64_t>(0, std::min<int64_t>(20, value));
    else if (!std::strcmp(name, "tiny_scene_prims"))
        ctx->tiny_scene_prims = (uint32_t)std::max<int64_t>(0, std::min<int64_t>(255, value));
    else if (!std::strcmp(name, "film_block"))
        ctx->film_block = (int)std::max<int64_t>(0, std::min<int64_t>(13, value));
    else if (!std::strcmp(name, "film_relayout"))
        ctx->film_relayout = value != 0;
    else if (!std::strcmp(name, "any_on_accelerator"))
        ctx->any_on_accelerator = value < 0 ? -1 : (value != 0 ? 1 : 0);
    else if (!std::strcmp(name, "leaf_queue")) {
        if (value != 0 && !kExperiments) return fail(ctx, TRHIP_ERR_UNSUPPORTED, "leaf_queue %s", kNeedsExperiments);
        ctx->leaf_queue = value != 0;
    }
    else if (!std::strcmp(name, "wide4"))
        ctx->wide4 = value != 0;
    else if (!std::strcmp(name, "node_layout")) {
        if (value < 0 || value > 1) return fail(ctx, TRHIP_ERR_INVALID, "node_layout: 0 (depth-first) or 1 (sibling pairs per 128-byte line)");
        ctx->node_layout = (int)value;
    } else if (!std::strcmp(name, "film_swizzle"))
        ctx->film_swizzle = value != 0;
    else if (!std::strcmp(name, "film_tiled"))
        ctx->film_tiled = value != 0;
    else if (!std::strcmp(name, "pipelines")) {
        if (value < 1 || value > kMaxPipes) return fail(ctx, TRHIP_ERR_INVALID, "pipelines must be in 1..%d", kMaxPipes);
        ctx->pipelines = (int)value;
    } else if (!std::strcmp(name, "overlap"))
        ctx->overlap = value != 0;
    else if (!std::strcmp(name, "traversal")) {
        if (value < 1 || value > 7 || value == 5) return fail(ctx, TRHIP_ERR_INVALID, "traversal must be 1, 2, 3, 4, 6 or 7");
        if ((value == 4 || value == 6 || value == 7) && !kExperiments) return fail(ctx, TRHIP_ERR_UNSUPPORTED, "traversal %d %s", (int)value, kNeedsExperiments);
        ctx->traversal = (int)value;
    } else if (!std::strcmp(name, "batch_paths")) {
        if (value < 0) return fail(ctx, TRHIP_ERR_INVALID, "batch_paths must be >= 0 (0 = auto)");
        ctx->batch_paths = (uint64_t)value;
    } else
        return fail(ctx, TRHIP_ERR_INVALID, "unknown option %s", name);
    return 0;
}

}

namespace {
TH_HD float detmath_eval(int fn, float x, float y) {
    switch (fn) {
    case 0: return tm_sinf(x);
    case 1: return tm_cosf(x);
    case 2: return tm_tanf(x);
    case 3: return tm_atan2f(y, x);
    case 4: return tm_acosf(x);
    case 5: return tm_logf(x);
    default: {
        float sn, cs;
        tm_sincosf(x, &sn, &cs);
        return fn == 6 ? sn : cs;
    }
    }
}
__global__ void k_detmath(int fn, const float* __restrict__ x, const float* __restrict__ y, uint64_t n, float* __restrict__ out) {
    for (uint64_t i = (uint64_t)blockIdx.x * blockDim.x + threadIdx.x; i < n; i += (uint64_t)gridDim.x * blockDim.x) out[i] = detmath_eval(fn, x[i], y ? y[i] : 0.0f);
}
}
extern "C" int trhip_detmath_f32_device(trhip_ctx* ctx, int fn, const float* x, const float* y, uint64_t n, float* out) {
// ... 35 lines not shown
```

trace.jl_amd/csrc/tu_path.hip:

```cpp
#include "th_host.h"

void derive_sensor(const trhip_sensor* sn, DeviceSensor& d) {
    std::memcpy(d.raster_to_camera, sn->raster_to_camera, sizeof d.raster_to_camera);
    std::memcpy(d.camera_to_world, sn->camera_to_world, sizeof d.camera_to_world);
    d.lens_radius = sn->lens_radius;
    d.focal_distance = sn->focal_distance;
    d.shutter_open = sn->shutter_open;
    d.shutter_close = sn->shutter_close;
    for (int i = 0; i < 2; ++i) {
        d.crop_min[i] = sn->crop_min[i];
        d.crop_max[i] = sn->crop_max[i];
        d.filter_radius[i] = sn->filter_radius[i];
        d.sb_min[i] = (int)std::floor(sn->crop_min[i] + 0.5f - sn->filter_radius[i]);
        d.sb_max[i] = (int)std::ceil(sn->crop_max[i] - 0.5f + sn->filter_radius[i]);
    }
    d.scale = sn->scale;
    d.sb_w = d.sb_max[0] - d.sb_min[0] + 1;
    d.sb_h = d.sb_max[1] - d.sb_min[1] + 1;
    d.film_w = (int)std::fabs(sn->crop_max[0] - (sn->crop_min[0] - 1.0f));
    d.film_h = (int)std::fabs(sn->crop_max[1] - (sn->crop_min[1] - 1.0f));
    d.tiles_x = (int)std::floor(((float)(d.sb_max[0] - d.sb_min[0]) + 16.0f) / 16.0f);
    d.tiles_y = (int)std::floor(((float)(d.sb_max[1] - d.sb_min[1]) + 16.0f) / 16.0f);
    d.band_y0 = d.sb_min[1];
    d.band_rows = d.sb_h;
// ... 31 lines not shown
void launch_film(trhip_ctx* ctx, hipStream_t st, const DeviceSensor& ds, const DeviceSensor* dsp, const float4* L, uint64_t total_slots, uint32_t spp, uint64_t seed, uint32_t sample_offset,
                 float4* d_film, bool fused) {
    if (film_uses_packed(ctx, ds)) {
        const uint32_t npix_b = (uint32_t)(ds.sb_w * ds.band_rows);
        const uint64_t padded = (uint64_t)((npix_b + 63u) / 64u) * 64u * spp;
        uint32_t layout = 0;
        FilmSideTable side{ctx->film_side.p ? (uint4*)ctx->film_side.p + 1 : nullptr, (uint32_t*)ctx->film_side.p, 0};
        if (fused) {
            layout = 1;
        } else {
            bool ok = false;
            side = film_side_table(ctx, st, total_slots, &ok);
            if (!ok) return;
        }
        if (fused) {
        } else if (ctx->film_relayout && total_slots == (uint64_t)npix_b * spp && ensure(ctx, ctx->film_Lt, padded * sizeof(float4)) == 0) {
            layout = 1;
            hipLaunchKernelGGL(k_film_pack_transpose, dim3(grid_for(ctx, padded, 8)), dim3(kBlock), 0, st, dsp, npix_b, spp, seed, sample_offset, L, (float4*)ctx->film_Lt.p, side);
            L = (const float4*)ctx->film_Lt.p;
        } else {
            hipLaunchKernelGGL(k_film_pack_w, dim3(grid_for(ctx, total_slots, 8)), dim3(kBlock), 0, st, dsp, total_slots, seed, sample_offset, const_cast<float4*>(L), side);
        }
        const float* tb = (const float*)ctx->table.p;
        auto threads = [&](int bx, int by) { return (uint64_t)((ds.film_w + bx - 1) / bx) * (uint64_t)((ds.film_h + by - 1) / by); };
#define TH_FILM_PACKED(BXV, BYV) hipLaunchKernelGGL((k_film_gather_packed<BXV, BYV>), dim3(grid_for(ctx, threads(BXV, BYV), 8)), dim3(kBlock), 0, st, dsp, tb, L, spp, seed, sample_offset, layout, (const uint4*)side.desc, d_film, ctx->film_swizzle ? 1u : 0u)
        switch (ctx->film_block) {
        case 4: TH_FILM_PACKED(1, 4); break;
        case 7: TH_FILM_PACKED(2, 2); break;
        case 8: TH_FILM_PACKED(4, 2); break;
        case 9: TH_FILM_PACKED(8, 4); break;
        case 10: TH_FILM_PACKED(1, 8); break;
        case 11: TH_FILM_PACKED(1, 16); break;
        case 12: TH_FILM_PACKED(1, 2); break;
        case 13: TH_FILM_PACKED(1, 1); break;
        case 6: TH_FILM_PACKED(4, 4); break;
        default: TH_FILM_PACKED(2, 4); break;
        }
#undef TH_FILM_PACKED
        return;
    }
    if (film_uses_desc(ctx, ds) && ctx->fdesc.bytes >= total_slots * sizeof(uint4)) {
        hipLaunchKernelGGL(k_film_descriptors, dim3(grid_for(ctx, total_slots, 8)), dim3(kBlock), 0, st, dsp, total_slots, seed, sample_offset, (uint4*)ctx->fdesc.p);
        const uint64_t nthreads = (uint64_t)ds.film_w * ((ds.film_h + 3) / 4);
        hipLaunchKernelGGL((k_film_gather_desc<4>), dim3(grid_for(ctx, nthreads, 8)), dim3(kBlock), 0, st, dsp, (const float*)ctx->table.p, L, (const uint4*)ctx->fdesc.p, spp, d_film);
        return;
    }
    const uint32_t npix = (uint32_t)(ds.sb_w * ds.band_rows);
    const uint64_t padded = (uint64_t)((npix + 63u) / 64u) * 64u * spp;
    uint32_t layout = 0;
    const bool whole = ds.band_rows == ds.sb_h;
    if (whole && ctx->film_transpose && spp > 1 && total_slots == (uint64_t)npix * spp && ensure(ctx, ctx->pfilm, padded * sizeof(float2)) == 0 && ensure(ctx, ctx->film_Lt, padded * sizeof(float4)) == 0) {
        layout = 1;
        hipLaunchKernelGGL(k_film_transpose, dim3(grid_for(ctx, padded, 8)), dim3(kBlock), 0, st, L, npix, spp, (float4*)ctx->film_Lt.p);
        L = (const float4*)ctx->film_Lt.p;
    }
    hipLaunchKernelGGL(k_film_positions, dim3(grid_for(ctx, total_slots, 8)), dim3(kBlock), 0, st, dsp, total_slots, seed, sample_offset, (float2*)ctx->pfilm.p, layout, spp);
    const float rmax = std::fmax(ds.filter_radius[0], ds.filter_radius[1]);
    if (whole && ctx->film_tiled && rmax <= 6.0f) {
        const uint32_t budget = 24 * 1024 / 20;
        const uint32_t nc_max = 16 + 2 * (uint32_t)std::ceil(rmax) + 4;
        uint32_t cols, ns;
        if (spp <= budget) {
            ns = spp;
            cols = std::max(1u, std::min(nc_max, budget / spp));
        } else {
            cols = 1;
            ns = budget;
        }
        const dim3 grid((ds.film_w + 15) / 16, (ds.film_h + 15) / 16);
        hipLaunchKernelGGL(k_film_gather_tiled, grid, dim3(kBlock), (size_t)cols * ns * 20 + 16, st, dsp, (const float*)ctx->table.p, L, (const float2*)ctx->pfilm.p, spp, layout, cols, ns, d_film);
    } else {
        const uint64_t npx = (uint64_t)ds.film_w * ds.film_h;
        const int fblock = ctx->film_block >= 4 ? 2 : ctx->film_block;
        if (fblock == 1)
            hipLaunchKernelGGL((k_film_gather_block<2, 2>), dim3(grid_for(ctx, (npx + 3) / 4, 8)), dim3(kBlock), 0, st, dsp, (const float*)ctx->table.p, L, (const float2*)ctx->pfilm.p, spp, layout, d_film);
        else if (fblock == 2)
            hipLaunchKernelGGL((k_film_gather_block<TH_FILM_BX, TH_FILM_BY>), dim3(grid_for(ctx, (npx + TH_FILM_BX * TH_FILM_BY - 1) / (TH_FILM_BX * TH_FILM_BY), 8)), dim3(kBlock), 0, st, dsp, (const float*)ctx->table.p, L, (const float2*)ctx->pfilm.p, spp, layout, d_film);
        else
            hipLaunchKernelGGL(k_film_gather, dim3(grid_for(ctx, npx, 8)), dim3(kBlock), 0, st, dsp, (const float*)ctx->table.p, L, (const float2*)ctx->pfilm.p, spp, layout, d_film);
    }
}

namespace {
int render_stream_impl(trhip_ctx* ctx, const trhip_scene* scene, const trhip_sensor* sensor, const DeviceSensor& ds, uint32_t spp, int max_depth, uint64_t seed, uint32_t sample_offset, void* out,
                       bool out_is_device, trhip_stats* stats, bool* declined) {
    *declined = true;
    const uint64_t npix = (uint64_t)ds.sb_w * ds.sb_h;
    const uint64_t total_slots = npix * spp;
    const int R_b = max_depth + 16, R = R_b + max_depth;
    if (R + 1 > kMaxDepth + 1) return 0;
    if ((uint64_t)max_depth * total_slots >= (1ull << 32)) return 0;
    if (total_slots >= (1ull << 31)) return 0;
    const uint64_t P = total_slots;
    const uint32_t list_cap = ctx->stream_list_cap ? ctx->stream_list_cap : (uint32_t)std::max<uint64_t>(65536, P / 128);
    const uint32_t cap = (uint32_t)(((P + kSeg - 1) / kSeg + 2 * kSegGran + list_cap / kSeg + 64 + kSegGran - 1) / kSegGran * kSegGran);
    const uint64_t Pphys = (uint64_t)cap * kSeg;
    const size_t list_bytes = (size_t)list_cap * (4 * 16 + 16 + 4 + (size_t)kStack2Total * 8);
    const size_t terms_bytes = (size_t)max_depth * total_slots * sizeof(float4);
    const size_t need = terms_bytes + Pphys * (10 * 16 + 2 * 4) + 4 * list_bytes + total_slots * 24 + (3ull << 30);
    {
        size_t free_b = 0, total_b = 0;
        HIP_TRY(ctx, hipMemGetInfo(&free_b, &total_b));
        size_t held = ctx->Lbuf.bytes + ctx->pfilm.bytes + ctx->st_terms.bytes + ctx->st_tags[0].bytes + ctx->st_tags[1].bytes;
        Pipe& p0 = ctx->pipes[0];
        held += p0.hits.bytes;
        for (auto& a : p0.q)
            for (auto& b : a) held += b.bytes;
        for (auto& b : p0.sq) held += b.bytes;
        for (auto& a : ctx->st_list)
            for (auto& b : a)
                for (auto& c : b) held += c.bytes;
        if ((double)need > 0.9 * (double)(free_b + held)) return 0;
    }
    *declined = false;
    Pipe& pp = ctx->pipes[0];
    if (!pp.st) {
        HIP_TRY(ctx, hipStreamCreate(&pp.st));
        HIP_TRY(ctx, hipStreamCreate(&pp.st2));
        HIP_TRY(ctx, hipEventCreateWithFlags(&pp.ev_shade, hipEventDisableTiming));
        HIP_TRY(ctx, hipEventCreateWithFlags(&pp.ev_any, hipEventDisableTiming));
        HIP_TRY(ctx, hipEventCreateWithFlags(&pp.ev_done, hipEventDisableTiming));
    }
    if (int rc = upload(ctx, ctx->sensor, &ds, sizeof ds)) return rc;
    if (int rc = upload(ctx, ctx->table, sensor->filter_table, 256 * sizeof(float))) return rc;
    for (int k = 0; k < 2; ++k)
        for (int j = 0; j < 3; ++j)
            if (int rc = ensure(ctx, pp.q[k][j], Pphys * sizeof(float4))) return rc;
    for (int j = 0; j < 3; ++j)
        if (int rc = ensure(ctx, pp.sq[j], Pphys * sizeof(float4))) return rc;
    if (int rc = ensure(ctx, pp.hits, Pphys * sizeof(float4))) return rc;
    if (int rc = ensure(ctx, pp.counters, sizeof(Counters))) return rc;
    const size_t slab_bytes = (size_t)trace_grid(ctx) * kBlock * (size_t)kStackSlabLevels * sizeof(uint2);
    for (int k = 0; k < 2; ++k)
        if (int rc = ensure(ctx, pp.overflow[k], slab_bytes)) return rc;
    if (int rc = ensure(ctx, ctx->Lbuf, total_slots * sizeof(float4))) return rc;
    if (int rc = ensure_film_samples(ctx, ds, total_slots)) return rc;
    if (int rc = ensure(ctx, ctx->st_terms, terms_bytes)) return rc;
    for (int k = 0; k < 2; ++k)
        if (int rc = ensure(ctx, ctx->st_tags[k], Pphys * sizeof(uint32_t))) return rc;
    const size_t row_bytes = (size_t)kSeg * kCtrStride * sizeof(uint32_t);
    if (int rc = ensure(ctx, ctx->st_frozen, row_bytes)) return rc;
    if (int rc = ensure(ctx, ctx->st_counts, 16 * sizeof(uint32_t))) return rc;
    const size_t field_bytes[7] = {16, 16, 16, 16, 16, 4, (size_t)kStack2Total * 8};
    for (int kind = 0; kind < 2; ++kind)
        for (int pg = 0; pg < 2; ++pg)
            for (int f = 0; f < 7; ++f)
                if (int rc = ensure(ctx, ctx->st_list[kind][pg][f], (size_t)list_cap * field_bytes[f])) return rc;
    const size_t film_bytes = (size_t)ds.film_w * ds.film_h * sizeof(float4);
    void* d_film = out;
    if (!out_is_device) {
        if (int rc = ensure(ctx, ctx->film, film_bytes)) return rc;
        d_film = ctx->film.p;
    }
    auto list_of = [&](int kind, int pg) {
        DevBuf* b = ctx->st_list[kind][pg];
        return SuspendList{(float4*)b[0].p, (float4*)b[1].p, (float4*)b[2].p, (float4*)b[3].p, (uint4*)b[4].p, (uint32_t*)b[5].p, (uint2*)b[6].p, list_cap};
    };
    uint32_t* lc = (uint32_t*)ctx->st_counts.p;
    hipStream_t st = ctx->stream, ps = pp.st, ps2 = ctx->overlap ? pp.st2 : pp.st;
    const DeviceSensor* dsp = (const DeviceSensor*)ctx->sensor.p;
    float4* L = (float4*)ctx->Lbuf.p;
    float4* terms = (float4*)ctx->st_terms.p;
    Counters* ctr = (Counters*)pp.counters.p;
    PathQueue pq[2];
    for (int k = 0; k < 2; ++k) pq[k] = PathQueue{(float4*)pp.q[k][0].p, (float4*)pp.q[k][1].p, (float4*)pp.q[k][2].p};
    uint32_t* tags[2] = {(uint32_t*)ctx->st_tags[0].p, (uint32_t*)ctx->st_tags[1].p};
    ShadowQueue sq{(float4*)pp.sq[0].p, (float4*)pp.sq[1].p, (float4*)pp.sq[2].p};
    float4* hits = (float4*)pp.hits.p;
    uint32_t* frozen = (uint32_t*)ctx->st_frozen.p;

    Timer tm(ctx, ctx->timing && stats);
    hipEvent_t e0, e1, ev_start;
    HIP_TRY(ctx, hipEventCreate(&e0));
    HIP_TRY(ctx, hipEventCreate(&e1));
    HIP_TRY(ctx, hipEventCreateWithFlags(&ev_start, hipEventDisableTiming));
    HIP_TRY(ctx, hipEventRecord(e0, st));
    HIP_TRY(ctx, hipMemsetAsync(terms, 0, terms_bytes, st));
    HIP_TRY(ctx, hipEventRecord(ev_start, st));
    HIP_TRY(ctx, hipStreamWaitEvent(ps, ev_start, 0));
    HIP_TRY(ctx, hipMemsetAsync(ctr, 0, sizeof(Counters), ps));
    HIP_TRY(ctx, hipMemsetAsync(lc, 0, 16 * sizeof(uint32_t), ps));
    tm.begin(0, ps);
    hipLaunchKernelGGL(k_raygen, dim3(grid_for(ctx, P, 8)), dim3(kBlock), 0, ps, dsp, 0u, (uint32_t)P, seed, sample_offset, pq[0], cap, ctr);
    hipLaunchKernelGGL(k_fill_u32, dim3(grid_for(ctx, Pphys, 8)), dim3(kBlock), 0, ps, tags[0], Pphys, 1u);
    tm.end(0, ps);
    const int g_shade = ctx->num_cu * 8;
    int cur = 0;
    for (int r = 0; r < R; ++r) {
        const uint32_t budget_min = r < R_b ? ctx->stream_budget_min : 0u;
        const int in_pg = r & 1, out_pg = (r + 1) & 1;
        HIP_TRY(ctx, hipMemcpyAsync(frozen, ctr->n_queue[r], row_bytes, hipMemcpyDeviceToDevice, ps));
        HIP_TRY(ctx, hipMemsetAsync(&lc[out_pg], 0, sizeof(uint32_t), ps));
        HIP_TRY(ctx, hipMemsetAsync(&lc[2], 0, sizeof(uint32_t), ps));
        StreamCtl sc_c{list_of(0, in_pg), list_of(0, out_pg), &lc[in_pg], &lc[2], &lc[out_pg], budget_min, ctx->stream_budget_shift, pq[cur].beta, tags[cur], pq[cur].o, pq[cur].d, pq[cur].beta, hits, tags[cur],
                       ctr->n_queue[r], cap};
        const SegQueue qc{frozen, cap, 0u};
        const TraceOut oc{hits, nullptr, nullptr, nullptr, 1u};
        tm.begin(1, ps);
        launch_trace2_stream(ctx, ps, scene, false, qc, pq[cur].o, pq[cur].d, oc, ctr->work_closest[r], pp.overflow[0].p, ctr, sc_c);
        tm.end(1, ps);
        if (ps2 != ps && r > 0) HIP_TRY(ctx, hipStreamWaitEvent(ps, pp.ev_any, 0));
        tm.begin(2, ps);
        const ShadeStream sst{tags[cur], tags[cur ^ 1], (uint32_t)total_slots};
        if (has_directional_light(scene)) {
            if (scene->dev.tri_tan)
                hipLaunchKernelGGL((k_shade_path<true, true, true>), dim3(g_shade), dim3(kBlock), 0, ps, scene->dev, dsp, pq[cur], pq[cur ^ 1], sq, cap, hits, terms, ctr, r, 0, max_depth, 1u, sst);
            else
                hipLaunchKernelGGL((k_shade_path<true, false, true>), dim3(g_shade), dim3(kBlock), 0, ps, scene->dev, dsp, pq[cur], pq[cur ^ 1], sq, cap, hits, terms, ctr, r, 0, max_depth, 1u, sst);
        } else if (scene->dev.tri_tan) {
            hipLaunchKernelGGL(k_shade_path<true>, dim3(g_shade), dim3(kBlock), 0, ps, scene->dev, dsp, pq[cur], pq[cur ^ 1], sq, cap, hits, terms, ctr, r, 0, max_depth, 1u, sst);
        } else {
            hipLaunchKernelGGL((k_shade_path<true, false>), dim3(g_shade), dim3(kBlock), 0, ps, scene->dev, dsp, pq[cur], pq[cur ^ 1], sq, cap, hits, terms, ctr, r, 0, max_depth, 1u, sst);
        }
        tm.end(2, ps);
        if (ps2 != ps) {
            HIP_TRY(ctx, hipEventRecord(pp.ev_shade, ps));
            HIP_TRY(ctx, hipStreamWaitEvent(ps2, pp.ev_shade, 0));
        }
        HIP_TRY(ctx, hipMemsetAsync(&lc[4 + out_pg], 0, sizeof(uint32_t), ps2));
        HIP_TRY(ctx, hipMemsetAsync(&lc[6], 0, sizeof(uint32_t), ps2));
        StreamCtl sc_a{list_of(1, in_pg), list_of(1, out_pg), &lc[4 + in_pg], &lc[6], &lc[4 + out_pg], budget_min, ctx->stream_budget_shift, nullptr, nullptr, nullptr, nullptr, nullptr, nullptr, nullptr, nullptr, 0u};
        const SegQueue qa{ctr->n_shadow[r], cap, 0u};
        const TraceOut oa{nullptr, terms, sq.c, nullptr, 0u};
        tm.begin(3, ps2);
        launch_trace2_stream(ctx, ps2, scene, true, qa, sq.o, sq.d, oa, ctr->work_shadow[r], pp.overflow[1].p, ctr, sc_a);
        tm.end(3, ps2);
        if (ps2 != ps) HIP_TRY(ctx, hipEventRecord(pp.ev_any, ps2));
        cur ^= 1;
    }
    if (ps2 != ps) HIP_TRY(ctx, hipStreamWaitEvent(ps, pp.ev_any, 0));
    tm.begin(2, ps);
    hipLaunchKernelGGL(k_fold_terms, dim3(grid_for(ctx, total_slots, 8)), dim3(kBlock), 0, ps, (const float4*)terms, total_slots, (uint32_t)max_depth, L);
    tm.end(2, ps);
    HIP_TRY(ctx, hipEventRecord(pp.ev_done, ps));
    HIP_TRY(ctx, hipStreamWaitEvent(st, pp.ev_done, 0));
    tm.begin(4, st);
    launch_film(ctx, st, ds, dsp, L, total_slots, spp, seed, sample_offset, (float4*)d_film, false);
    tm.end(4, st);
    HIP_TRY(ctx, hipEventRecord(e1, st));
    HIP_TRY(ctx, hipGetLastError());
    HIP_TRY(ctx, hipStreamSynchronize(st));
    ctx->last_L_count = total_slots;
    ctx->last_L_layout = 0;
    if (!out_is_device) HIP_TRY(ctx, hipMemcpy(out, d_film, film_bytes, hipMemcpyDeviceToHost));
    uint32_t left[8];
    HIP_TRY(ctx, hipMemcpy(left, lc, sizeof left, hipMemcpyDeviceToHost));
    if (stats) {
        std::memset(stats, 0, sizeof *stats);
        stats->camera_samples = total_slots;
        Counters h;
        HIP_TRY(ctx, hipMemcpy(&h, ctr, sizeof h, hipMemcpyDeviceToHost));
        stats->closest_rays = h.closest_total;
        stats->shadow_rays = h.shadow_total;
        stats->nodes_visited = h.nodes_closest;
        stats->prims_tested = h.prims_closest;
        stats->nodes_visited_shadow = h.nodes_shadow;
        stats->prims_tested_shadow = h.prims_shadow;
        stats->fallback_rays = h.fallback_total;
        stats->nodes_visited_fallback = h.nodes_fallback;
        stats->prims_tested_fallback = h.prims_fallback;
        float ms = 0;
        (void)hipEventElapsedTime(&ms, e0, e1);
        stats->ms_total = ms;
        stats->ms_raygen = tm.total(0, &stats->launches_raygen);
        stats->ms_trace_closest = tm.total(1, &stats->launches_trace_closest);
        stats->ms_fallback = tm.fallback_total(&stats->launches_fallback);
        stats->ms_shade = tm.total(2, &stats->launches_shade);
        stats->ms_trace_any = tm.total(3, &stats->launches_trace_any);
        stats->ms_film = tm.total(4, &stats->launches_film);
        stats->n_batches = 1;
        stats->max_depth_reached = (uint32_t)max_depth;
        traversal_info(ctx, scene, &stats->traversal, &stats->node_bytes);
    }
    (void)hipEventDestroy(e0);
    (void)hipEventDestroy(e1);
    (void)hipEventDestroy(ev_start);
    if (left[R & 1] || left[4 + (R & 1)]) return fail(ctx, TRHIP_ERR_HIP, "streaming wavefront: %u + %u rays still suspended after the drain rounds", left[R & 1], left[4 + (R & 1)]);
    return 0;
}

int render_impl_band(trhip_ctx* ctx, const trhip_scene* scene, const trhip_sensor* sensor, int integrator, uint32_t spp, int max_depth, uint64_t seed, uint32_t sample_offset, void* out,
                     bool out_is_device, trhip_stats* stats, const DeviceSensor* band) {
    HostClock hclk;
    if (!ctx || !scene || !sensor || !out) return fail(ctx, TRHIP_ERR_INVALID, "null argument");
    if (!scene->committed) return fail(ctx, TRHIP_ERR_INVALID, "scene not committed");
    if (integrator != 0 && integrator != 1) return fail(ctx, TRHIP_ERR_INVALID, "unknown integrator %d", integrator);
    if (scene->has_materialless_prim)
            return fail(ctx, TRHIP_ERR_UNSUPPORTED, "rendering a scene with a material-less primitive is not supported (the trace entry points accept it)");
    if (spp == 0 || max_depth < 1 || max_depth > kMaxDepth) return fail(ctx, TRHIP_ERR_INVALID, "spp must be >= 1 and max_depth in 1..%d", kMaxDepth);
    if (!ctx->warned_idle_accelerator && ctx->hybrid) {
        const char* why = hybrid_idle_reason(ctx, scene);
        if (why[0]) {
            ctx->warned_idle_accelerator = true;
            std::fprintf(stderr, "[tracehip] this scene holds the reference's tree and an accelerator, but the accelerator is idle: %s\n", why);
        }
// ... 57 lines not shown
            held += pp.hits.bytes;
            for (auto& a : pp.q)
                for (auto& b : a) held += b.bytes;
            for (auto& b : pp.sq) held += b.bytes;
        }
        const double avail = 0.85 * (double)(free_b + held) - (double)total_slots * (sizeof(float4) + sizeof(float2)) - 2.5e9;
        batch_paths = avail > 0 ? (uint64_t)(avail / 212.0) : npix;
    }
    uint64_t spp_batch = std::max<uint64_t>(1, batch_paths / npix);
    spp_batch = std::min<uint64_t>(spp_batch, spp);
    const int want_pipes = std::max(1, std::min(ctx->pipelines, kMaxPipes));
    spp_batch = std::max<uint64_t>(1, std::min<uint64_t>(spp_batch / want_pipes, (spp + want_pipes - 1) / want_pipes));
    while (npix * spp_batch >= (1ull << 31)) spp_batch = (spp_batch + 1) / 2;
    const uint64_t n_batches_total = (spp + spp_batch - 1) / spp_batch;
    const int NP = (int)std::min<uint64_t>(want_pipes, n_batches_total);
    const uint64_t P = npix * spp_batch;
    const uint32_t cap = (uint32_t)(((P + kSeg - 1) / kSeg + 2 * kSegGran + kSegGran - 1) / kSegGran * kSegGran);
    const uint64_t Pphys = (uint64_t)cap * kSeg;
    if (int rc = upload(ctx, ctx->sensor, &ds, sizeof ds)) return rc;
    if (int rc = upload(ctx, ctx->table, sensor->filter_table, 256 * sizeof(float))) return rc;
    const size_t slab_bytes = (size_t)trace_grid(ctx) * kBlock * (size_t)kStackSlabLevels * sizeof(uint2);
    for (int pi = 0; pi < NP; ++pi) {
        Pipe& pp = ctx->pipes[pi];
        if (!pp.st) {
            int prio_lo = 0, prio_hi = 0;
            (void)hipDeviceGetStreamPriorityRange(&prio_lo, &prio_hi);
            HIP_TRY(ctx, hipStreamCreate(&pp.st));
            if (ctx->stream2_priority && prio_hi != prio_lo)
                HIP_TRY(ctx, hipStreamCreateWithPriority(&pp.st2, hipStreamDefault, ctx->stream2_priority > 0 ? prio_hi : prio_lo));
            else
                HIP_TRY(ctx, hipStreamCreate(&pp.st2));
            HIP_TRY(ctx, hipEventCreateWithFlags(&pp.ev_shade, hipEventDisableTiming));
            HIP_TRY(ctx, hipEventCreateWithFlags(&pp.ev_any, hipEventDisableTiming));
            HIP_TRY(ctx, hipEventCreateWithFlags(&pp.ev_done, hipEventDisableTiming));
        }
        for (int k = 0; k < 2; ++k)
            for (int j = 0; j < 3; ++j)
                if (int rc = ensure(ctx, pp.q[k][j], Pphys * sizeof(float4))) return rc;
        for (int j = 0; j < 3; ++j)
            if (int rc = ensure(ctx, pp.sq[j], Pphys * sizeof(float4))) return rc;
        if (ctx->overlap)
            for (int j = 0; j < 3; ++j)
                if (int rc = ensure(ctx, pp.sq2[j], Pphys * sizeof(float4))) return rc;
        if (!pp.ev_any2) HIP_TRY(ctx, hipEventCreateWithFlags(&pp.ev_any2, hipEventDisableTiming));
        if (int rc = ensure(ctx, pp.hits, Pphys * sizeof(float4))) return rc;
        if (int rc = ensure(ctx, pp.counters, sizeof(Counters))) return rc;
        for (int k = 0; k < 2; ++k)
            if (int rc = ensure(ctx, pp.overflow[k], slab_bytes)) return rc;
    }
    const bool fused = film_fused(ctx, ds, spp);
    const uint64_t l_slots = fused ? ((npix + 63u) / 64u) * 64u * (uint64_t)spp : total_slots;
    if (int rc = ensure(ctx, ctx->poison, l_slots)) return rc;
    if (int rc = ensure(ctx, ctx->Lbuf, l_slots * sizeof(float4))) return rc;
    if (int rc = ensure_film_samples(ctx, ds, total_slots)) return rc;
    const size_t film_bytes = (size_t)ds.film_w * ds.film_h * sizeof(float4);
    void* d_film = out;
    if (!out_is_device) {
        if (int rc = ensure(ctx, ctx->film, film_bytes)) return rc;
        d_film = ctx->film.p;
    }
    hipStream_t st = ctx->stream;
    const DeviceSensor* dsp = (const DeviceSensor*)ctx->sensor.p;
    float4* L = (float4*)ctx->Lbuf.p;

    hclk.tick("setup (budget, buffers)");
    Timer tm(ctx, ctx->timing && stats);
    hipEvent_t e0, e1, ev_start;
    HIP_TRY(ctx, hipEventCreate(&e0));
    HIP_TRY(ctx, hipEventCreate(&e1));
    HIP_TRY(ctx, hipEventCreateWithFlags(&ev_start, hipEventDisableTiming));
    HIP_TRY(ctx, hipEventRecord(e0, st));
    FilmSideTable fside{nullptr, nullptr, 0};
    if (fused) {
        bool ok = false;
        fside = film_side_table(ctx, st, total_slots, &ok);
        if (!ok) return TRHIP_ERR_HIP;
    } else {
        HIP_TRY(ctx, hipMemsetAsync(L, 0, total_slots * sizeof(float4), st));
    }
    HIP_TRY(ctx, hipMemsetAsync(ctx->poison.p, 0, l_slots, st));
    HIP_TRY(ctx, hipEventRecord(ev_start, st));
    const int g_shade = ctx->num_cu * 8;
    const uint32_t bary_mode = (ctx->traversal >= 2 && scene->wide_ok) ? 1u : 0u;
    uint32_t n_batches = 0;
    for (int pi = 0; pi < NP; ++pi) {
        HIP_TRY(ctx, hipStreamWaitEvent(ctx->pipes[pi].st, ev_start, 0));
        HIP_TRY(ctx, hipMemsetAsync(ctx->pipes[pi].counters.p, 0, sizeof(Counters), ctx->pipes[pi].st));
    }
    for (uint64_t s0 = 0; s0 < spp; s0 += spp_batch) {
        Pipe& pp = ctx->pipes[n_batches % NP];
        n_batches++;
        const uint64_t nb = std::min<uint64_t>(spp_batch, spp - s0) * npix;
        hipStream_t ps = pp.st, ps2 = ctx->overlap ? pp.st2 : pp.st;
        Counters* ctr = (Counters*)pp.counters.p;
        PathQueue pq[2];
        for (int k = 0; k < 2; ++k) pq[k] = PathQueue{(float4*)pp.q[k][0].p, (float4*)pp.q[k][1].p, (float4*)pp.q[k][2].p};
        const bool two = ps2 != ps;
        const ShadowQueue sqs[2] = {ShadowQueue{(float4*)pp.sq[0].p, (float4*)pp.sq[1].p, (float4*)pp.sq[2].p},
                                    two ? ShadowQueue{(float4*)pp.sq2[0].p, (float4*)pp.sq2[1].p, (float4*)pp.sq2[2].p} : ShadowQueue{(float4*)pp.sq[0].p, (float4*)pp.sq[1].p, (float4*)pp.sq[2].p}};
        hipEvent_t ev_anys[2] = {pp.ev_any, pp.ev_any2};
        float4* hits = (float4*)pp.hits.p;
        HIP_TRY(ctx, hipMemsetAsync(ctr, 0, offsetof(Counters, closest_total), ps));
        tm.begin(0, ps);
        hipLaunchKernelGGL(k_raygen, dim3(grid_for(ctx, nb, 8)), dim3(kBlock), 0, ps, dsp, (uint32_t)(s0 * npix), (uint32_t)nb, seed, sample_offset, pq[0], cap, ctr, fused ? L : nullptr, spp, fside);
        tm.end(0, ps);
        int cur = 0;
        for (int depth = 1; depth <= max_depth; ++depth) {
            const ShadowQueue& sq = sqs[depth & 1];
            tm.begin(1, ps);
            launch_trace(ctx, ps, scene, false, SegQueue{ctr->n_queue[depth - 1], cap, 0u}, pq[cur].o, pq[cur].d, nullptr,
                         TraceOut{hits, nullptr, nullptr, nullptr, bary_mode, depth == 1 && far_camera(scene, sensor) ? 1u : 0u}, ctr->work_closest[depth - 1], ctr, pp.overflow[0].p);
            tm.end(1, ps);
            if (two && depth > 2) HIP_TRY(ctx, hipStreamWaitEvent(ps, ev_anys[depth & 1], 0));
            tm.begin(2, ps);
            const ShadeStream sst{nullptr, nullptr, 0u, two ? (uint8_t*)ctx->poison.p : nullptr};
            if (has_directional_light(scene)) {
                if (scene->dev.tri_tan)
                    hipLaunchKernelGGL((k_shade_path<false, true, true>), dim3(g_shade), dim3(kBlock), 0, ps, scene->dev, dsp, pq[cur], pq[cur ^ 1], sq, cap, hits, L, ctr, depth - 1, depth, max_depth, bary_mode, sst);
                else
                    hipLaunchKernelGGL((k_shade_path<false, false, true>), dim3(g_shade), dim3(kBlock), 0, ps, scene->dev, dsp, pq[cur], pq[cur ^ 1], sq, cap, hits, L, ctr, depth - 1, depth, max_depth, bary_mode, sst);
            } else if (scene->dev.tri_tan) {
                hipLaunchKernelGGL(k_shade_path<false>, dim3(g_shade), dim3(kBlock), 0, ps, scene->dev, dsp, pq[cur], pq[cur ^ 1], sq, cap, hits, L, ctr, depth - 1, depth, max_depth, bary_mode, sst);
            } else {
                hipLaunchKernelGGL((k_shade_path<false, false>), dim3(g_shade), dim3(kBlock), 0, ps, scene->dev, dsp, pq[cur], pq[cur ^ 1], sq, cap, hits, L, ctr, depth - 1, depth, max_depth, bary_mode, sst);
            }
            tm.end(2, ps);
            if (two) {
                HIP_TRY(ctx, hipEventRecord(pp.ev_shade, ps));
                HIP_TRY(ctx, hipStreamWaitEvent(ps2, pp.ev_shade, 0));
            }
            tm.begin(3, ps2);
            launch_trace(ctx, ps2, scene, true, SegQueue{ctr->n_shadow[depth - 1], cap, 0u}, sq.o, sq.d, nullptr, TraceOut{nullptr, L, sq.c, nullptr}, ctr->work_shadow[depth - 1], ctr, pp.overflow[1].p);
            tm.end(3, ps2);
            if (two) HIP_TRY(ctx, hipEventRecord(ev_anys[depth & 1], ps2));
            cur ^= 1;
        }
        if (two) {
            HIP_TRY(ctx, hipStreamWaitEvent(ps, ev_anys[max_depth & 1], 0));
            if (max_depth >= 2) HIP_TRY(ctx, hipStreamWaitEvent(ps, ev_anys[(max_depth - 1) & 1], 0));
        }
    }
    for (int pi = 0; pi < NP; ++pi) {
        HIP_TRY(ctx, hipEventRecord(ctx->pipes[pi].ev_done, ctx->pipes[pi].st));
        HIP_TRY(ctx, hipStreamWaitEvent(st, ctx->pipes[pi].ev_done, 0));
    }
    tm.begin(4, st);
    if (ctx->overlap) hipLaunchKernelGGL(k_apply_poison, dim3(grid_for(ctx, l_slots, 8)), dim3(kBlock), 0, st, L, (const uint8_t*)ctx->poison.p, l_slots);
    launch_film(ctx, st, ds, dsp, L, total_slots, spp, seed, sample_offset, (float4*)d_film, fused);
    tm.end(4, st);
    ctx->last_L_layout = fused ? 1u : 0u;
    ctx->last_L_npix = (uint32_t)npix;
    ctx->last_L_spp = spp;
    HIP_TRY(ctx, hipEventRecord(e1, st));
    HIP_TRY(ctx, hipGetLastError());
    hclk.tick("enqueue");
    HIP_TRY(ctx, hipStreamSynchronize(st));
    hclk.tick("stream sync");
    ctx->last_L_count = total_slots;
    if (!out_is_device) HIP_TRY(ctx, hipMemcpy(out, d_film, film_bytes, hipMemcpyDeviceToHost));
    if (stats) {
        std::memset(stats, 0, sizeof *stats);
        stats->camera_samples = total_slots;
        for (int pi = 0; pi < NP; ++pi) {
            Counters h;
            HIP_TRY(ctx, hipMemcpy(&h, ctx->pipes[pi].counters.p, sizeof h, hipMemcpyDeviceToHost));
            stats->closest_rays += h.closest_total;
            stats->shadow_rays += h.shadow_total;
            stats->nodes_visited += h.nodes_closest;
            stats->prims_tested += h.prims_closest;
            stats->nodes_visited_shadow += h.nodes_shadow;
            stats->prims_tested_shadow += h.prims_shadow;
            stats->fallback_rays += h.fallback_total;
            stats->nodes_visited_fallback += h.nodes_fallback;
            stats->prims_tested_fallback += h.prims_fallback;
            for (int k = 0; k < 4; ++k) stats->count_sub[k] += h.fallback_why[k];
        }
        float ms = 0;
        (void)hipEventElapsedTime(&ms, e0, e1);
        stats->ms_total = ms;
        stats->ms_raygen = tm.total(0, &stats->launches_raygen);
        stats->ms_trace_closest = tm.total(1, &stats->launches_trace_closest);
        stats->ms_fallback = tm.fallback_total(&stats->launches_fallback);
        stats->ms_shade = tm.total(2, &stats->launches_shade);
        stats->ms_trace_any = tm.total(3, &stats->launches_trace_any);
        stats->ms_film = tm.total(4, &stats->launches_film);
        stats->n_batches = n_batches;
        stats->max_depth_reached = (uint32_t)max_depth;
        traversal_info(ctx, scene, &stats->traversal, &stats->node_bytes);
        ctx->last_fallback_share = stats->closest_rays ? (double)stats->fallback_rays / (double)stats->closest_rays : 0.0;
        if (stats->traversal == 9 && ctx->last_fallback_share > 0.2 && !ctx->warned_fallback_cliff) {
            ctx->warned_fallback_cliff = true;
            std::fprintf(stderr, "[tracehip] the certified walk handed %.0f %% of this frame's closest-hit rays back to the reference-order walk (near-ties, grazed leaf boxes, rays in a "
                                 "primitive's plane): the frame is exact but the accelerator saves little on this scene\n", 100.0 * ctx->last_fallback_share);
        }
    }
    hclk.tick("counters + event times");
    (void)hipEventDestroy(e0);
    (void)hipEventDestroy(e1);
    (void)hipEventDestroy(ev_start);
    return 0;
}

int plan_rows_per_band(const DeviceSensor& ds, uint32_t spp, double budget_bytes, double bytes_per_sample) {
    const double row_bytes = (double)ds.sb_w * 16.0 * (double)spp * bytes_per_sample;
    int rows = (int)std::max(1.0, std::min((double)ds.tiles_y, std::floor(budget_bytes / row_bytes)));
    while (rows > 1 && (uint64_t)ds.sb_w * 16ull * (uint64_t)rows * spp >= (1ull << 32)) --rows;
    return rows;
// ... 195 lines not shown
```

trace.jl_amd/csrc/tu_scene.hip:

```cpp
#include "th_host.h"
#include "th_bvh_ref.h"

static uint32_t wide_node_order(const FlatBVH& t, int layout, std::vector<uint32_t>& widx) {
    const uint32_t n = (uint32_t)t.a.size();
    widx.assign(n, 0u);
    auto interior = [&](uint32_t i) { return (t.flags[i] & 3u) != 3u; };
    uint32_t next = 0;
    if (layout != 1) {
        for (uint32_t i = 0; i < n; ++i)
            if (interior(i)) widx[i] = next++;
        return next;
    }
    if (n == 0 || !interior(0)) return 0;
    widx[0] = next++;
    std::vector<uint32_t> stack{0u};
    while (!stack.empty()) {
        const uint32_t i = stack.back();
        stack.pop_back();
        const uint32_t c0 = i + 1, c1 = t.a[i];
        const bool i0 = c0 < n && interior(c0), i1 = c1 < n && interior(c1);
        if (i0 && i1) {
            next = (next + 1u) & ~1u;
            widx[c0] = next++;
            widx[c1] = next++;
// ... 118 lines not shown
                vr = roughness_to_alpha(vr);
            }
            if (!black(r)) {
                Lobe l = is_specular ? base_lobe(LOBE_SPECULAR_R, BSDF_SPECULAR | BSDF_REFLECTION) : microfacet_lobe(LOBE_MICROFACET_R, BSDF_REFLECTION | BSDF_GLOSSY, r, ur, vr);
                set_rgb(l.r, r);
                l.fresnel = FRESNEL_DIELECTRIC;
                l.fr_eta_i = 1.0f;
                l.fr_eta_t = eta;
                s.lobe[s.n++] = l;
            }
            if (!black(t)) {
                Lobe l = is_specular ? base_lobe(LOBE_SPECULAR_T, BSDF_SPECULAR | BSDF_TRANSMISSION) : microfacet_lobe(LOBE_MICROFACET_T, BSDF_TRANSMISSION | BSDF_GLOSSY, t, ur, vr);
                set_rgb(l.r, t);
                l.eta_a = 1.0f;
                l.eta_b = eta;
                l.fresnel = FRESNEL_DIELECTRIC;
                l.fr_eta_i = 1.0f;
                l.fr_eta_t = eta;
                s.lobe[s.n++] = l;
            }
            break;
        }
        case TRHIP_PLASTIC: {
            if (n != 8) return -1;
            float kd[3], ks[3];
            clamp_rgb(p, kd);
            if (!black(kd)) {
                Lobe l = base_lobe(LOBE_LAMBERT_R, BSDF_DIFFUSE | BSDF_REFLECTION);
                set_rgb(l.r, kd);
                s.lobe[s.n++] = l;
            }
            clamp_rgb(p + 3, ks);
            if (black(ks)) break;
            float rough = p[6];
            if (p[7] != 0.0f) rough = roughness_to_alpha(rough);
            Lobe l = microfacet_lobe(LOBE_MICROFACET_R, BSDF_REFLECTION | BSDF_GLOSSY, ks, rough, rough);
            l.fresnel = FRESNEL_DIELECTRIC;
            l.fr_eta_i = 1.5f;
            l.fr_eta_t = 1.0f;
            s.lobe[s.n++] = l;
            break;
        }
        default: return -1;
        }
    }
    return 0;
}

void material_base_colour(int kind, const float* p, float* out) {
    clamp_rgb(p, out);
    if (kind == TRHIP_GLASS) {
        float t[3];
        clamp_rgb(p + 3, t);
        if (!black(t)) set_rgb(out, t);
    }
}

HostAABB sphere_world_bound(const SphereRec& s) {
    HostAABB b;
    b.reset();
    const float lo[3] = {-s.radius, -s.radius, s.z_min}, hi[3] = {s.radius, s.radius, s.z_max};
    for (int c = 0; c < 8; ++c) {
        const f3 p = xf_point(s.o2w, mk3((c & 1) ? hi[0] : lo[0], (c & 2) ? hi[1] : lo[1], (c & 4) ? hi[2] : lo[2]));
        const float q[3] = {p.x, p.y, p.z};
        b.grow_point(q);
    }
    return b;
}
float det3(const float* m) {
    return m[0] * (m[5] * m[10] - m[6] * m[9]) - m[1] * (m[4] * m[10] - m[6] * m[8]) + m[2] * (m[4] * m[9] - m[5] * m[8]);
}

bool has_sphere_subtree(const trhip_scene* s, uint32_t root) {
    const uint32_t n_nodes = (uint32_t)s->g->bvh.a.size(), n_prims = (uint32_t)s->g->bvh.order.size();
    if (root >= n_nodes) return true;
    uint32_t end = root;
    while ((s->g->bvh.flags[end] & 3u) != 3u) end = s->g->bvh.a[end];
    for (uint32_t i = root; i <= end && i < n_nodes; ++i)
        if ((s->g->bvh.flags[i] & 3u) == 3u)
            for (uint32_t k = s->g->bvh.a[i]; k < s->g->bvh.a[i] + (s->g->bvh.flags[i] >> 2) && k < n_prims; ++k)
                if (s->g->prims[s->g->bvh.order[k]].kind == 1) return true;
    return false;
}
}

int upload_scene(trhip_scene* s) {
    trhip_ctx* ctx = s->ctx;
    CommitClock clk;
    const uint32_t n_nodes = (uint32_t)s->g->bvh.a.size(), n_prims = (uint32_t)s->g->bvh.order.size();
    RawArray<float4> nodes((size_t)n_nodes * 2), prims((size_t)n_prims * 3), nrm((size_t)n_prims * 3);
    parallel_for(n_nodes, [&](size_t i0, size_t i1) {
        for (size_t i = i0; i < i1; ++i) {
            const float* b = &s->g->bvh.bounds[6 * i];
            nodes[2 * i] = make_float4(b[0], b[1], b[2], __builtin_bit_cast(float, s->g->bvh.a[i]));
            nodes[2 * i + 1] = make_float4(b[3], b[4], b[5], __builtin_bit_cast(float, s->g->bvh.flags[i]));
        }
    });
    parallel_for(n_prims, [&](size_t k0, size_t k1) {
        for (size_t k = k0; k < k1; ++k) {
            const HostPrim& p = s->g->prims[s->g->bvh.order[k]];
            if (p.kind == 1) {
                prims[3 * k] = make_float4(__builtin_bit_cast(float, p.sphere_id), 0, 0, __builtin_bit_cast(float, p.meta));
                prims[3 * k + 1] = prims[3 * k + 2] = make_float4(0, 0, 0, 0);
                nrm[3 * k] = nrm[3 * k + 1] = nrm[3 * k + 2] = make_float4(0, 0, 0, 0);
            } else {
                prims[3 * k] = make_float4(p.v[0], p.v[1], p.v[2], __builtin_bit_cast(float, p.meta));
                prims[3 * k + 1] = make_float4(p.v[3], p.v[4], p.v[5], 0);
                prims[3 * k + 2] = make_float4(p.v[6], p.v[7], p.v[8], 0);
                const uint32_t mat = p.meta & PRIM_MATERIAL_MASK;
                const bool fast = mat != PRIM_NO_MATERIAL && mat < s->g->materials.size() && s->g->materials[mat].set[1].n == 1 && s->g->materials[mat].set[1].lobe[0].kind == LOBE_LAMBERT_R;
                if (fast) prims[3 * k].w = __builtin_bit_cast(float, p.meta | PRIM_FAST);
                for (int j = 0; j < 3; ++j) nrm[3 * k + j] = make_float4(p.n[3 * j], p.n[3 * j + 1], p.n[3 * j + 2], fast ? s->g->materials[mat].set[1].lobe[0].r[j] : 0.0f);
            }
        }
    });
    clk.tick("upload: node / prim records");
    if (int rc = upload(ctx, s->g->d_nodes, nodes.data(), nodes.size() * sizeof(float4))) return rc;
    if (int rc = upload(ctx, s->g->d_prims, prims.data(), prims.size() * sizeof(float4))) return rc;
    if (int rc = upload(ctx, s->g->d_nrm, nrm.data(), nrm.size() * sizeof(float4))) return rc;
    clk.tick("upload: 3 copies");
    const bool any_tan = !s->g->prim_tan.empty(), any_uv = !s->g->prim_uv.empty();
    if (any_tan) s->g->prim_tan.resize(9 * s->g->prims.size(), 0.0f);
    if (any_uv) s->g->prim_uv.resize(7 * s->g->prims.size(), 0.0f);
    s->has_materialless_prim = false;
    for (const HostPrim& p : s->g->prims) s->has_materialless_prim = s->has_materialless_prim || (p.meta & PRIM_MATERIAL_MASK) == PRIM_NO_MATERIAL;
    s->dev.tri_tan = nullptr;
    if (any_tan) {
        std::vector<float4> tan((size_t)n_prims * 3, make_float4(0, 0, 0, 0));
        parallel_for(n_prims, [&](size_t k0, size_t k1) {
            for (size_t k = k0; k < k1; ++k) {
                const uint32_t id = s->g->bvh.order[k];
                const HostPrim& p = s->g->prims[id];
                const float* tg = &s->g->prim_tan[9 * (size_t)id];
                if (p.kind == 0 && (p.meta & PRIM_HAS_TANGENTS))
                    for (int j = 0; j < 3; ++j) tan[3 * k + j] = make_float4(tg[3 * j], tg[3 * j + 1], tg[3 * j + 2], 0.0f);
            }
        });
        if (int rc = upload(ctx, s->g->d_tan, tan.data(), tan.size() * sizeof(float4))) return rc;
        s->dev.tri_tan = (const float4*)s->g->d_tan.p;
    } else {
        release(s->g->d_tan);
    }
    DevBuf d_uv;
    if (any_uv) {
        std::vector<float4> uvs((size_t)n_prims * 2, make_float4(0, 0, 0, 0));
        parallel_for(n_prims, [&](size_t k0, size_t k1) {
            for (size_t k = k0; k < k1; ++k) {
                const uint32_t id = s->g->bvh.order[k];
                const float* uv = &s->g->prim_uv[7 * (size_t)id];
                if (s->g->prims[id].kind == 0 && uv[6] != 0.0f) {
                    uvs[2 * k] = make_float4(uv[0], uv[1], uv[2], uv[3]);
                    uvs[2 * k + 1] = make_float4(uv[4], uv[5], 1.0f, 0.0f);
                }
            }
        });
        if (int rc = upload(ctx, d_uv, uvs.data(), uvs.size() * sizeof(float4))) {
            release(d_uv);
            return rc;
        }
    }
    {
        if (int rc = ensure(ctx, s->g->d_shade, (size_t)n_prims * 8 * sizeof(float4))) {
            release(d_uv);
            return rc;
        }
        hipLaunchKernelGGL(k_shade_constants, dim3(std::max(1u, std::min((n_prims + kBlock - 1) / kBlock, 4096u))), dim3(kBlock), 0, ctx->stream, (float4*)s->g->d_shade.p, (const float4*)s->g->d_prims.p, (const float4*)s->g->d_nrm.p, (const float4*)d_uv.p, n_prims);
        const hipError_t e1 = hipGetLastError(), e2 = hipStreamSynchronize(ctx->stream);
        release(d_uv);
        HIP_TRY(ctx, e1);
        HIP_TRY(ctx, e2);
    }
    clk.tick("upload: shade records");
    if (int rc = upload(ctx, s->g->d_spheres, s->g->spheres.data(), s->g->spheres.size() * sizeof(SphereRec))) return rc;
    if (int rc = upload(ctx, s->g->d_materials, s->g->materials.data(), s->g->materials.size() * sizeof(MaterialRec))) return rc;
    if (int rc = upload(ctx, s->g->d_base_colour, s->g->base_colour.data(), s->g->base_colour.size() * sizeof(float))) return rc;
    s->dev.nodes = (const float4*)s->g->d_nodes.p;
    s->dev.prims = (const float4*)s->g->d_prims.p;
    s->dev.tri_nrm = (const float4*)s->g->d_nrm.p;
    s->dev.shade = (const float4*)s->g->d_shade.p;
    s->dev.spheres = (const SphereRec*)s->g->d_spheres.p;
    s->dev.materials = (const MaterialRec*)s->g->d_materials.p;
    s->dev.lights = nullptr;
    s->dev.n_nodes = n_nodes;
    s->dev.n_prims = n_prims;
    s->dev.n_spheres = (uint32_t)s->g->spheres.size();
    s->dev.n_materials = (uint32_t)s->g->materials.size();
    s->dev.n_lights = 0;
    bool has_empty_leaf = false;
    s->wide_ok = false;
    std::memset(&s->wide, 0, sizeof s->wide);
    s->wide.root_ref = kRefNone;
    if (n_nodes > 0 && n_prims < (1u << 24) && !s->literal_only) {
        std::vector<uint32_t> widx;
// ... 500 lines not shown
        s->wide_acc.leaf_order = nullptr;
        s->hybrid_ok = true;
        clk.tick("accelerator: one leaf");
        return 0;
    }
    std::atomic<bool> bad{false};
    parallel_for(n_anodes, [&](size_t i0, size_t i1) {
        for (size_t i = i0; i < i1 && !bad; ++i) {
            if ((s->g->acc.flags[i] & 3u) != 3u) {
                if (s->g->acc.a[i] <= i + 1 || s->g->acc.a[i] >= n_anodes) bad = true;
                continue;
            }
            const uint32_t first = s->g->acc.a[i], cnt = s->g->acc.flags[i] >> 2;
            if (cnt == 0 || cnt > 255 || (uint64_t)first + cnt > n_prims) {
                bad = true;
                continue;
            }
            for (uint32_t k = first; k < first + cnt; ++k)
                if (std::memcmp(&s->g->acc.bounds[6 * i], &slot_box[6 * (size_t)cslot[s->g->acc.order[k]]], 6 * sizeof(float)) != 0) bad = true;
        }
    });
    if ((s->g->acc.flags[0] & 3u) == 3u) return 0;
    if (bad && conformed) return 0;
    if (bad) {
        FlatBVH out;
        if (!conform_accelerator(s->g->acc, cslot, leaf_of_slot, slot_box, n_prims, out)) return 0;
        s->g->acc = std::move(out);
        return upload_accelerator_conformed(s);
    }
    if (std::memcmp(&s->g->acc.bounds[0], &s->g->bvh.bounds[0], 6 * sizeof(float)) != 0) return 0;
    clk.tick("accelerator: leaf boxes");
    std::vector<uint32_t> order_word(n_prims, 0u);
    {
        auto leftmost = [&](uint32_t i, uint32_t& slot) {
            for (uint32_t guard = 0; guard < 4096u && i < n_cnodes; ++guard) {
                if ((s->g->bvh.flags[i] & 3u) == 3u) {
                    slot = s->g->bvh.a[i];
                    return true;
                }
                ++i;
            }
            return false;
        };
        for (uint32_t sid = 0; sid < std::min<uint32_t>((uint32_t)s->g->spheres.size(), kCertOrderSpheres); ++sid) {
            const uint32_t ks = sph_slot[sid], sh = 3u * sid;
            uint32_t i = 0, lo = 0, hi = n_prims;
            bool ok = false;
            for (uint32_t guard = 0; guard < 4096u && i < n_cnodes; ++guard) {
                if ((s->g->bvh.flags[i] & 3u) == 3u) {
                    const uint32_t first = s->g->bvh.a[i], cnt = s->g->bvh.flags[i] >> 2;
                    ok = ks - first < cnt && first == lo && first + cnt == hi;
                    for (uint32_t k = first; ok && k < first + cnt; ++k)
                        if (k != ks) order_word[k] |= (3u | (k > ks ? 4u : 0u)) << sh;
                    break;
                }
                const uint32_t second = s->g->bvh.a[i], axis = s->g->bvh.flags[i] & 3u;
                uint32_t lo2 = 0;
                if (second <= i + 1 || second >= n_cnodes || !leftmost(second, lo2) || lo2 < lo || lo2 > hi) break;
                if (ks >= lo2) {
                    for (uint32_t k = lo; k < lo2; ++k) order_word[k] |= axis << sh;
                    lo = lo2;
                    i = second;
                } else {
                    for (uint32_t k = lo2; k < hi; ++k) order_word[k] |= (axis | 4u) << sh;
                    hi = lo2;
                    i = i + 1;
                }
            }
            if (!ok) return 0;
        }
    }
    RawArray<float4> aprims((size_t)n_prims * 3);
    std::vector<uint8_t> is_sphere(n_prims, 0);
    parallel_for(n_prims, [&](size_t k0, size_t k1) {
        for (size_t k = k0; k < k1; ++k) {
            const HostPrim& p = s->g->prims[s->g->acc.order[k]];
            const float cs = __builtin_bit_cast(float, cslot[s->g->acc.order[k]]);
            if (p.kind == 1) {
                aprims[3 * k] = make_float4(__builtin_bit_cast(float, p.sphere_id), 0, 0, __builtin_bit_cast(float, p.meta));
                aprims[3 * k + 1] = make_float4(0, 0, 0, cs);
                aprims[3 * k + 2] = make_float4(0, 0, 0, 0);
                is_sphere[k] = 1;
            } else {
                aprims[3 * k] = make_float4(p.v[0], p.v[1], p.v[2], __builtin_bit_cast(float, p.meta));
                aprims[3 * k + 1] = make_float4(p.v[3], p.v[4], p.v[5], cs);
                aprims[3 * k + 2] = make_float4(p.v[6], p.v[7], p.v[8], __builtin_bit_cast(float, order_word[cslot[s->g->acc.order[k]]]));
            }
        }
    });
    if (int rc = upload(ctx, s->g->d_acc_prims, aprims.data(), aprims.size() * sizeof(float4))) return rc;
    clk.tick("accelerator: primitive records");
    {
        std::mutex lock;
        float mle[3] = {0.0f, 0.0f, 0.0f}, sq = 0.0f;
        parallel_for(s->g->prims.size(), [&](size_t i0, size_t i1) {
            float m[3] = {0.0f, 0.0f, 0.0f}, q = 0.0f;
            for (size_t i = i0; i < i1; ++i) {
                const HostPrim& p = s->g->prims[i];
                if (p.kind != 0 || (p.meta & PRIM_DEGENERATE)) continue;
                float e[3];
                for (int c = 0; c < 3; ++c) e[c] = std::fmax(std::fmax(p.v[c], p.v[3 + c]), p.v[6 + c]) - std::fmin(std::fmin(p.v[c], p.v[3 + c]), p.v[6 + c]);
                if (e[0] == 0.0f || e[1] == 0.0f || e[2] == 0.0f) {
                    double ab[3], ac[3];
                    for (int c = 0; c < 3; ++c) {
                        ab[c] = (double)p.v[3 + c] - p.v[c];
                        ac[c] = (double)p.v[6 + c] - p.v[c];
                    }
                    const double bc[3] = {ac[0] - ab[0], ac[1] - ab[1], ac[2] - ab[2]};
                    const double l2 = std::max({ab[0] * ab[0] + ab[1] * ab[1] + ab[2] * ab[2], ac[0] * ac[0] + ac[1] * ac[1] + ac[2] * ac[2], bc[0] * bc[0] + bc[1] * bc[1] + bc[2] * bc[2]});
                    const double cx = ab[1] * ac[2] - ab[2] * ac[1], cy = ab[2] * ac[0] - ab[0] * ac[2], cz = ab[0] * ac[1] - ab[1] * ac[0];
                    const double area2 = std::sqrt(cx * cx + cy * cy + cz * cz);
                    if (area2 > 0.0) q = std::fmax(q, (float)(l2 * std::sqrt(l2) / area2) * 1.0001f);
                } else {
                    for (int a = 0; a < 3; ++a)
                        if (e[a] < INFINITY) m[a] = std::fmax(m[a], e[a]);
                }
            }
            std::lock_guard<std::mutex> g(lock);
            for (int a = 0; a < 3; ++a) mle[a] = std::fmax(mle[a], m[a]);
            sq = std::fmax(sq, q);
        });
        for (int a = 0; a < 3; ++a) s->cert.mle_small[a] = mle[a];
        s->cert.sq_flat = sq;
        if (std::getenv("TRHIP_COMMIT_TIMING")) std::fprintf(stderr, "[commit] certificate: mle %g %g %g, sq_flat %g\n", mle[0], mle[1], mle[2], sq);
    }
    std::vector<uint32_t> widx;
    const uint32_t n_int = wide_node_order(s->g->acc, ctx->node_layout, widx);
    if (n_int >= (1u << 24)) return 0;
    std::vector<uint8_t> has_sphere(n_anodes, 0);
    for (uint32_t i = n_anodes; i-- > 0;) {
        if ((s->g->acc.flags[i] & 3u) == 3u) {
            const uint32_t first = s->g->acc.a[i], cnt = s->g->acc.flags[i] >> 2;
            if (!s->g->spheres.empty())
                for (uint32_t k = first; k < first + cnt; ++k) has_sphere[i] |= is_sphere[k];
        } else {
            has_sphere[i] = has_sphere[i + 1] | has_sphere[s->g->acc.a[i]];
        }
    }
    RawArray<float4> wn((size_t)n_int * 4);
    if (ctx->node_layout == 1) std::memset((void*)wn.data(), 0, (size_t)n_int * 4 * sizeof(float4));
    parallel_for(n_anodes, [&](size_t i0, size_t i1) {
        for (size_t i = i0; i < i1; ++i) {
            if ((s->g->acc.flags[i] & 3u) == 3u) continue;
            const uint32_t c[2] = {(uint32_t)i + 1, s->g->acc.a[i]};
            uint32_t ref[2], cnt[2];
            for (int k = 0; k < 2; ++k) {
                if ((s->g->acc.flags[c[k]] & 3u) == 3u) {
                    ref[k] = s->g->acc.a[c[k]];
                    cnt[k] = s->g->acc.flags[c[k]] >> 2;
                } else {
                    ref[k] = widx[c[k]];
                    cnt[k] = 0;
                }
            }
            const float* l = &s->g->acc.bounds[6 * (size_t)c[0]];
            const float* r = &s->g->acc.bounds[6 * (size_t)c[1]];
            float4* w = &wn[4 * (size_t)widx[i]];
            w[0] = make_float4(l[0], l[3], l[1], l[4]);
            w[1] = make_float4(l[2], l[5], r[0], r[3]);
            w[2] = make_float4(r[1], r[4], r[2], r[5]);
            w[3] = make_float4(__builtin_bit_cast(float, ref[0] | (cnt[0] << 24)), __builtin_bit_cast(float, ref[1] | (cnt[1] << 24)),
                               __builtin_bit_cast(float, (s->g->acc.flags[i] & 3u) | ((uint32_t)has_sphere[c[0]] << 2) | ((uint32_t)has_sphere[c[1]] << 3)), 0.0f);
        }
    });
    if (int rc = upload(ctx, s->g->d_acc_wnodes, wn.data(), wn.size() * sizeof(float4))) return rc;
    s->wide_acc.wnodes = (const float4*)s->g->d_acc_wnodes.p;
    s->wide_acc.n_wnodes = n_int;
// ... 740 lines not shown
```

Measured before the change: 6108.

## Encode fast-material class bit in hit word and prefetch next hit in shade loop

Trace kernels now pack a PRIM_FAST-derived class bit into the hit's primitive slot word, so the shade kernel can classify hits without a dependent gather from the shade record table. The shade loop is restructured to load the next iteration's hit ahead of time (a one-stage software pipeline), with an optional two-stage variant that also preloads ray and shade records. This aims to cut dependent-load latency in k_shade_path, at the cost of extra registers and reserving the top slot bit, which caps usable slot indices.

```diff
diff --git a/trace.jl_amd/csrc/th_host.h b/trace.jl_amd/csrc/th_host.h
--- a/trace.jl_amd/csrc/th_host.h
+++ b/trace.jl_amd/csrc/th_host.h
@@ -59,6 +59,7 @@
     double bvh_device_ms = 0.0;
     int bvh_builder = -1;
     bool film_transpose = false;
+    bool shade_class_bit = true;
     bool occluder_pretest = true;
     int stream2_priority = -1;
     bool leaf_kernel = true;
diff --git a/trace.jl_amd/csrc/th_kernels.h b/trace.jl_amd/csrc/th_kernels.h
--- a/trace.jl_amd/csrc/th_kernels.h
+++ b/trace.jl_amd/csrc/th_kernels.h
@@ -334,6 +334,9 @@
     return found;
 }
 
+constexpr uint32_t kHitClassBit = 1u << 30, kHitSlotMask = kHitClassBit - 1u;
+static_assert(PRIM_FAST << 2 == kHitClassBit, "hit_slot_word shifts the flag into place");
+TH_D uint32_t hit_slot_word(uint32_t slot, uint32_t meta, uint32_t class_bit) { return class_bit ? slot | ((meta & PRIM_FAST) << 2) : slot; }
 template <bool COUNT>
 __global__ __launch_bounds__(kBlock) void k_trace_closest(DeviceScene sc, SegQueue q, const float4* __restrict__ ro, const float4* __restrict__ rd, const float* __restrict__ tmax_or_null,
                                                           float4* __restrict__ hits, Counters* ctr) {
@@ -423,12 +426,18 @@
     }
 }
 
+struct ShadeRec {
+    float4 p0, p1, p2, na, nb, nc, cn, cs;
+};
+TH_D ShadeRec load_shade_rec(const DeviceScene& sc, int prim) {
+    const float4* rec = sc.shade + 8 * (size_t)prim;
+    return ShadeRec{rec[0], rec[1], rec[2], rec[3], rec[4], rec[5], rec[6], rec[7]};
+}
 template <bool TRI_ONLY = false, bool TAN = true>
-TH_D bool rebuild_shading(const DeviceScene& sc, int prim, f3 o, f3 d, Shading& sh, uint32_t& material, const float4* bary = nullptr, f3* fast_r = nullptr) {
-    const float4* rec = sc.shade + 8 * (size_t)prim;
-    const float4 p0 = rec[0], p1 = rec[1], p2 = rec[2];
-    const float4 na = rec[3], nb = rec[4], nc = rec[5];
-    const float4 cn = rec[6], cs = rec[7];
+TH_D bool rebuild_shading_rec(const DeviceScene& sc, int prim, const ShadeRec& rec, f3 o, f3 d, Shading& sh, uint32_t& material, const float4* bary = nullptr, f3* fast_r = nullptr) {
+    const float4 p0 = rec.p0, p1 = rec.p1, p2 = rec.p2;
+    const float4 na = rec.na, nb = rec.nb, nc = rec.nc;
+    const float4 cn = rec.cn, cs = rec.cs;
     const uint32_t meta = __float_as_uint(p0.w);
     material = meta & PRIM_MATERIAL_MASK;
     if (fast_r) *fast_r = mk3(na.w, nb.w, nc.w);
@@ -450,6 +459,10 @@
     const float4* tan = (TAN && sc.tri_tan && (meta & PRIM_HAS_TANGENTS)) ? sc.tri_tan + 3 * (size_t)prim : nullptr;
     sh = shade_triangle(v0, v1, v2, has_n, mk3(na.x, na.y, na.z), mk3(nb.x, nb.y, nb.z), mk3(nc.x, nc.y, nc.z), (meta & PRIM_FLIP) != 0, tt.bary, d, &tc, tan);
     return true;
+}
+template <bool TRI_ONLY = false, bool TAN = true>
+TH_D bool rebuild_shading(const DeviceScene& sc, int prim, f3 o, f3 d, Shading& sh, uint32_t& material, const float4* bary = nullptr, f3* fast_r = nullptr) {
+    return rebuild_shading_rec<TRI_ONLY, TAN>(sc, prim, load_shade_rec(sc, prim), o, d, sh, material, bary, fast_r);
 }
 template <int TH_ONE_COPY = 0> __global__ __launch_bounds__(kBlock) void k_shade_constants(float4* __restrict__ shade, const float4* __restrict__ prims, const float4* __restrict__ nrm, const float4* __restrict__ uv, uint32_t n_prims) {
     for (uint32_t k = blockIdx.x * kBlock + threadIdx.x; k < n_prims; k += gridDim.x * kBlock) {
@@ -491,20 +504,30 @@
     float4 so4, sd4, sc4, no4, nd4, nb4;
     uint32_t next_depth;
 };
+struct VertexIn {
+    float4 h4, o4, d4, b4;
+    uint32_t tag;
+};
+template <bool STREAM>
+TH_D void load_vertex_ray(const PathQueue& qin, const ShadeStream& ss, uint32_t i, VertexIn& v) {
+    v.o4 = qin.o[i];
+    v.d4 = qin.d[i];
+    v.b4 = qin.beta[i];
+    v.tag = STREAM ? ss.tags_in[i] : 0u;
+}
 template <bool STREAM, bool FAST, bool TAN = true, bool DIRL = false>
-TH_D void shade_vertex(const DeviceScene& sc, const PathQueue& qin, const float4* __restrict__ hits, float4* __restrict__ L, uint32_t i, int depth_fixed, int max_depth,
-                       uint32_t hits_have_bary, const ShadeStream& ss, ShadeOut& out) {
-    const float4 h4 = hits[i];
-    const int prim = __float_as_int(h4.y);
-    const float4 o4 = qin.o[i], d4 = qin.d[i], b4 = qin.beta[i];
-    const int depth = STREAM ? (int)ss.tags_in[i] : depth_fixed;
+TH_D void shade_vertex_in(const DeviceScene& sc, const VertexIn& vin, const ShadeRec& rec, int prim, float4* __restrict__ L, int depth_fixed, int max_depth, uint32_t hits_have_bary,
+                          const ShadeStream& ss, ShadeOut& out) {
+    const float4 h4 = vin.h4;
+    const float4 o4 = vin.o4, d4 = vin.d4, b4 = vin.b4;
+    const int depth = STREAM ? (int)vin.tag : depth_fixed;
     const uint32_t slot = STREAM ? (uint32_t)(depth - 1) * ss.term_stride + __float_as_uint(o4.w) : __float_as_uint(o4.w);
     const f3 o = mk3(o4.x, o4.y, o4.z), d = mk3(d4.x, d4.y, d4.z);
     f3 beta = mk3(b4.x, b4.y, b4.z);
     Shading sh;
     uint32_t material;
     f3 fast_r;
-    if (!(rebuild_shading<FAST, TAN>(sc, prim, o, d, sh, material, hits_have_bary ? &h4 : nullptr, &fast_r) && material != PRIM_NO_MATERIAL)) return;
+    if (!(rebuild_shading_rec<FAST, TAN>(sc, prim, rec, o, d, sh, material, hits_have_bary ? &h4 : nullptr, &fast_r) && material != PRIM_NO_MATERIAL)) return;
     const LobeSet& bsdf = sc.materials[FAST ? 0u : material].set[1];
     const bool lambert = FAST || bsdf_is_single_lambert(bsdf);
     Lobe lam;
@@ -586,10 +609,23 @@
     }
 }
 
+template <bool STREAM, bool FAST, bool TAN = true, bool DIRL = false>
+TH_D void shade_vertex(const DeviceScene& sc, const PathQueue& qin, const float4* __restrict__ hits, float4* __restrict__ L, uint32_t i, int depth_fixed, int max_depth,
+                       uint32_t hits_have_bary, uint32_t hits_have_class, const ShadeStream& ss, ShadeOut& out) {
+    VertexIn v;
+    v.h4 = hits[i];
+    const int prim = hits_have_class ? (int)(__float_as_uint(v.h4.y) & kHitSlotMask) : __float_as_int(v.h4.y);
+    load_vertex_ray<STREAM>(qin, ss, i, v);
+    shade_vertex_in<STREAM, FAST, TAN, DIRL>(sc, v, load_shade_rec(sc, prim), prim, L, depth_fixed, max_depth, hits_have_bary, ss, out);
+}
+
+#ifndef TH_SHADE_PIPE
+#define TH_SHADE_PIPE 1
+#endif
 template <bool STREAM, bool TAN = true, bool DIRL = false>
 __global__ __launch_bounds__(kBlock) __attribute__((amdgpu_waves_per_eu(TH_SHADE_WAVES))) void k_shade_path(DeviceScene sc, const DeviceSensor* __restrict__ sep, PathQueue qin, PathQueue qout, ShadowQueue sq, uint32_t cap,
                                                        const float4* __restrict__ hits, float4* __restrict__ L, Counters* ctr, int row, int depth_fixed, int max_depth, uint32_t hits_have_bary,
-                                                       ShadeStream ss) {
+                                                       uint32_t hits_have_class, ShadeStream ss) {
     __shared__ SegView sv;
     __shared__ uint32_t s_ring[kBlock / 64][128];
     const SegQueue qv{ctr->n_queue[row], cap, 0u};
@@ -616,24 +652,7 @@
             if (STREAM) ss.tags_out[ni] = e.next_depth;
         }
     };
-    uint32_t seg_in = 0;
-    for (uint32_t flat = blockIdx.x * kBlock + threadIdx.x; flat < total; flat += gridDim.x * kBlock) {
-        uint32_t lb;
-        seg_locate_from(sv, flat & ~63u, seg_in, lb);
-        const uint32_t local = lb + (flat & 63u);
-        const uint32_t i = seg_in * cap + local;
-        int cls = 0;
-        if (local < sv.count[seg_in]) {
-            const int prim = __float_as_int(hits[i].y);
-            if (prim >= 0) {
-                cls = (__float_as_uint(sc.shade[8 * (size_t)prim].w) & PRIM_FAST) ? 1 : 2;
-            }
-        }
-        ShadeOut e;
-        e.want_shadow = e.want_next = false;
-        e.next_depth = 0;
-        if (cls == 1) shade_vertex<STREAM, true, TAN, DIRL>(sc, qin, hits, L, i, depth_fixed, max_depth, hits_have_bary, ss, e);
-        emit(e);
+    auto park = [&](int cls, uint32_t i) {
         const unsigned long long m2 = __ballot(cls == 2);
         if (m2) {
             if (cls == 2) s_ring[wv][(ring_head + ring_cnt + (uint32_t)__popcll(m2 & lt_mask)) & 127u] = i;
@@ -644,19 +663,111 @@
                 ShadeOut g;
                 g.want_shadow = g.want_next = false;
                 g.next_depth = 0;
-                shade_vertex<STREAM, false, TAN, DIRL>(sc, qin, hits, L, j, depth_fixed, max_depth, hits_have_bary, ss, g);
+                shade_vertex<STREAM, false, TAN, DIRL>(sc, qin, hits, L, j, depth_fixed, max_depth, hits_have_bary, hits_have_class, ss, g);
                 emit(g);
                 ring_head = (ring_head + 64u) & 127u;
                 ring_cnt -= 64u;
                 __builtin_amdgcn_fence(__ATOMIC_ACQ_REL, "wavefront");
             }
         }
-    }
+    };
+    const float4 no_hit = make_float4(0.0f, __int_as_float(-1), 0.0f, 0.0f);
+    const uint32_t stride = gridDim.x * kBlock;
+    uint32_t seg_in = 0;
+    auto fetch_hit = [&](uint32_t flat, uint32_t& i, float4& h4) {
+        uint32_t lb;
+        seg_locate_from(sv, flat & ~63u, seg_in, lb);
+        const uint32_t local = lb + (flat & 63u);
+        i = seg_in * cap + local;
+        h4 = no_hit;
+        if (local < sv.count[seg_in]) h4 = hits[i];
+    };
+    auto classify = [&](const float4& h4) -> int {
+        const int w = __float_as_int(h4.y);
+        if (w < 0) return 0;
+#ifdef TH_DIAG_SHADE_ALL_FAST
+        return 1;
+#endif
+        if (hits_have_class) return ((uint32_t)w & kHitClassBit) ? 1 : 2;
+        return (__float_as_uint(sc.shade[8 * (size_t)w].w) & PRIM_FAST) ? 1 : 2;
+    };
+    auto slot_of = [&](const float4& h4) -> int { return hits_have_class ? (int)(__float_as_uint(h4.y) & kHitSlotMask) : __float_as_int(h4.y); };
+    uint32_t flat = blockIdx.x * kBlock + threadIdx.x;
+    uint32_t i = 0;
+    float4 h4 = no_hit;
+    if (flat < total) fetch_hit(flat, i, h4);
+#if TH_SHADE_PIPE == 2
+    int cls = classify(h4);
+    VertexIn vin;
+    ShadeRec rec;
+    vin.h4 = h4;
+    if (cls == 1) {
+        load_vertex_ray<STREAM>(qin, ss, i, vin);
+        rec = load_shade_rec(sc, slot_of(h4));
+    }
+    uint32_t i_n = 0;
+    float4 h4_n = no_hit;
+    if (flat < total && flat + stride < total) fetch_hit(flat + stride, i_n, h4_n);
+    for (; flat < total; flat += stride) {
+        uint32_t i_nn = 0;
+        float4 h4_nn = no_hit;
+        if (flat + stride < total && flat + 2u * stride < total) fetch_hit(flat + 2u * stride, i_nn, h4_nn);
+        const int cls_n = classify(h4_n);
+        VertexIn vin_n;
+        ShadeRec rec_n;
+        vin_n.h4 = h4_n;
+        if (cls_n == 1) {
+            load_vertex_ray<STREAM>(qin, ss, i_n, vin_n);
+            rec_n = load_shade_rec(sc, slot_of(h4_n));
+        }
+        ShadeOut e;
+        e.want_shadow = e.want_next = false;
+        e.next_depth = 0;
+        if (cls == 1) shade_vertex_in<STREAM, true, TAN, DIRL>(sc, vin, rec, slot_of(vin.h4), L, depth_fixed, max_depth, hits_have_bary, ss, e);
+        emit(e);
+        park(cls, i);
+        cls = cls_n;
+        i = i_n;
+        vin = vin_n;
+        rec = rec_n;
+        i_n = i_nn;
+        h4_n = h4_nn;
+    }
+#else
+    while (flat < total) {
+        const uint32_t flat_n = flat + stride;
+#if TH_SHADE_PIPE == 1
+        uint32_t i_n = 0;
+        float4 h4_n = no_hit;
+        if (flat_n < total) fetch_hit(flat_n, i_n, h4_n);
+#endif
+        const int cls = classify(h4);
+        ShadeOut e;
+        e.want_shadow = e.want_next = false;
+        e.next_depth = 0;
+        if (cls == 1) {
+            VertexIn vin;
+            vin.h4 = h4;
+            const int prim = slot_of(h4);
+            load_vertex_ray<STREAM>(qin, ss, i, vin);
+            shade_vertex_in<STREAM, true, TAN, DIRL>(sc, vin, load_shade_rec(sc, prim), prim, L, depth_fixed, max_depth, hits_have_bary, ss, e);
+        }
+        emit(e);
+        park(cls, i);
+        flat = flat_n;
+#if TH_SHADE_PIPE == 1
+        i = i_n;
+        h4 = h4_n;
+#else
+        if (flat < total) fetch_hit(flat, i, h4);
+#endif
+    }
+#endif
     if (ring_cnt) {
         ShadeOut g;
         g.want_shadow = g.want_next = false;
         g.next_depth = 0;
-        if (lane < ring_cnt) shade_vertex<STREAM, false, TAN, DIRL>(sc, qin, hits, L, s_ring[wv][(ring_head + lane) & 127u], depth_fixed, max_depth, hits_have_bary, ss, g);
+        if (lane < ring_cnt) shade_vertex<STREAM, false, TAN, DIRL>(sc, qin, hits, L, s_ring[wv][(ring_head + lane) & 127u], depth_fixed, max_depth, hits_have_bary, hits_have_class, ss, g);
         emit(g);
     }
 }
diff --git a/trace.jl_amd/csrc/th_trace2.h b/trace.jl_amd/csrc/th_trace2.h
--- a/trace.jl_amd/csrc/th_trace2.h
+++ b/trace.jl_amd/csrc/th_trace2.h
@@ -85,6 +85,7 @@
     uint32_t zero_mode;
     uint32_t* zero_flag;
     uint32_t any_acc_hint;
+    uint32_t class_bit;
 };
 
 struct SuspendList {
@@ -296,7 +297,7 @@
                             }
                             t_max = tt.t;
                             found = true;
-                            hit_prim = (int)slot;
+                            hit_prim = (int)hit_slot_word(slot, meta, out.class_bit);
                             b1 = tt.bary.x;
                             b2 = tt.bary.y;
                             hx = out.bary_mode ? tt.bary.z : tt.t;
@@ -518,7 +519,7 @@
                             live = false;
                         } else {
                             t_max = tt.t;
-                            hit_prim = (int)slot;
+                            hit_prim = (int)hit_slot_word(slot, meta, out.class_bit);
                             b1 = tt.bary.x;
                             b2 = tt.bary.y;
                             hx = out.bary_mode ? tt.bary.z : tt.t;
@@ -1224,7 +1225,7 @@
                         }
                         t_max = tt.t;
                         found = true;
-                        out.hits[idx] = make_float4(out.bary_mode ? tt.bary.z : tt.t, __int_as_float((int)slot), tt.bary.x, tt.bary.y);
+                        out.hits[idx] = make_float4(out.bary_mode ? tt.bary.z : tt.t, __uint_as_float(hit_slot_word(slot, meta, out.class_bit)), tt.bary.x, tt.bary.y);
                     }
                 }
             }
diff --git a/trace.jl_amd/csrc/th_trace3c.h b/trace.jl_amd/csrc/th_trace3c.h
--- a/trace.jl_amd/csrc/th_trace3c.h
+++ b/trace.jl_amd/csrc/th_trace3c.h
@@ -497,7 +497,7 @@
                         } else if (!flagged) {
                             t_lim = tt.t + 2.0f * dt;
                             s_st[tid] = st | 3u;
-                            out.hits[s_idx[tid]] = make_float4(out.bary_mode ? tt.bary.z : tt.t, p1.w , tt.bary.x, tt.bary.y);
+                            out.hits[s_idx[tid]] = make_float4(out.bary_mode ? tt.bary.z : tt.t, __uint_as_float(hit_slot_word(__float_as_uint(p1.w) , meta, out.class_bit)), tt.bary.x, tt.bary.y);
                         }
                     }
                 }
@@ -655,7 +655,7 @@
             t_lim = acc ? tt.t + 2.0f * dt : t_lim;
             best_slot = acc ? slot : best_slot;
             best_r4.x = acc ? (out.bary_mode ? tt.bary.z : tt.t) : best_r4.x;
-            best_r4.y = acc ? __int_as_float((int)slot) : best_r4.y;
+            best_r4.y = acc ? __uint_as_float(hit_slot_word(slot, meta, out.class_bit)) : best_r4.y;
             best_r4.z = acc ? tt.bary.x : best_r4.z;
             best_r4.w = acc ? tt.bary.y : best_r4.w;
         }
@@ -699,7 +699,7 @@
                     if (tri_intersect_sheared<true>(mk3(p0.x, p0.y, p0.z), mk3(p1.x, p1.y, p1.z), mk3(p2.x, p2.y, p2.z), o, shear, t_lim, &tt)) {
                         cand = true;
                         t_c = tt.t;
-                        r4 = make_float4(out.bary_mode ? tt.bary.z : tt.t, __int_as_float((int)slot), tt.bary.x, tt.bary.y);
+                        r4 = make_float4(out.bary_mode ? tt.bary.z : tt.t, __uint_as_float(hit_slot_word(slot, meta, out.class_bit)), tt.bary.x, tt.bary.y);
                     }
                 }
             } else if (COUNT && live) {
@@ -757,7 +757,7 @@
                     if (tri_intersect_sheared<true>(mk3(p0.x, p0.y, p0.z), mk3(p1.x, p1.y, p1.z), mk3(p2.x, p2.y, p2.z), o, shear, t_lim, &tt)) {
                         cand = true;
                         t_c = tt.t;
-                        r4 = make_float4(out.bary_mode ? tt.bary.z : tt.t, __int_as_float((int)slot), tt.bary.x, tt.bary.y);
+                        r4 = make_float4(out.bary_mode ? tt.bary.z : tt.t, __uint_as_float(hit_slot_word(slot, meta, out.class_bit)), tt.bary.x, tt.bary.y);
                     }
                 }
             } else if (COUNT && live) {
diff --git a/trace.jl_amd/csrc/th_trace3c4.h b/trace.jl_amd/csrc/th_trace3c4.h
--- a/trace.jl_amd/csrc/th_trace3c4.h
+++ b/trace.jl_amd/csrc/th_trace3c4.h
@@ -547,7 +547,7 @@
                         } else if (!flagged) {
                             t_lim = tt.t + 2.0f * dt;
                             s_st[tid] = st | 3u;
-                            out.hits[s_idx[tid]] = make_float4(out.bary_mode ? tt.bary.z : tt.t, p1.w , tt.bary.x, tt.bary.y);
+                            out.hits[s_idx[tid]] = make_float4(out.bary_mode ? tt.bary.z : tt.t, __uint_as_float(hit_slot_word(__float_as_uint(p1.w) , meta, out.class_bit)), tt.bary.x, tt.bary.y);
                         }
                     }
                 }
diff --git a/trace.jl_amd/csrc/tu_api.hip b/trace.jl_amd/csrc/tu_api.hip
--- a/trace.jl_amd/csrc/tu_api.hip
+++ b/trace.jl_amd/csrc/tu_api.hip
@@ -192,6 +192,8 @@
         ctx->hybrid = value != 0;
     else if (!std::strcmp(name, "film_transpose"))
         ctx->film_transpose = value != 0;
+    else if (!std::strcmp(name, "shade_class_bit"))
+        ctx->shade_class_bit = value != 0;
     else if (!std::strcmp(name, "band_tile_rows"))
         ctx->band_tile_rows = (int)std::max<int64_t>(0, value);
     else if (!std::strcmp(name, "compose_spheres"))
diff --git a/trace.jl_amd/csrc/tu_path.hip b/trace.jl_amd/csrc/tu_path.hip
--- a/trace.jl_amd/csrc/tu_path.hip
+++ b/trace.jl_amd/csrc/tu_path.hip
@@ -137,6 +137,13 @@
 }
 
 namespace {
+uint32_t path_class_bit(const trhip_ctx* ctx, const trhip_scene* scene) {
+#ifdef TRHIP_EXPERIMENTS
+    return 0u;
+#else
+    return (ctx->shade_class_bit && ctx->traversal >= 2 && scene->wide_ok && scene->dev.n_prims < kHitClassBit) ? 1u : 0u;
+#endif
+}
 int render_stream_impl(trhip_ctx* ctx, const trhip_scene* scene, const trhip_sensor* sensor, const DeviceSensor& ds, uint32_t spp, int max_depth, uint64_t seed, uint32_t sample_offset, void* out,
                        bool out_is_device, trhip_stats* stats, bool* declined) {
     *declined = true;
@@ -240,6 +247,7 @@
     hipLaunchKernelGGL(k_fill_u32, dim3(grid_for(ctx, Pphys, 8)), dim3(kBlock), 0, ps, tags[0], Pphys, 1u);
     tm.end(0, ps);
     const int g_shade = ctx->num_cu * 8;
+    const uint32_t class_bit = path_class_bit(ctx, scene);
     int cur = 0;
     for (int r = 0; r < R; ++r) {
         const uint32_t budget_min = r < R_b ? ctx->stream_budget_min : 0u;
@@ -250,7 +258,8 @@
         StreamCtl sc_c{list_of(0, in_pg), list_of(0, out_pg), &lc[in_pg], &lc[2], &lc[out_pg], budget_min, ctx->stream_budget_shift, pq[cur].beta, tags[cur], pq[cur].o, pq[cur].d, pq[cur].beta, hits, tags[cur],
                        ctr->n_queue[r], cap};
         const SegQueue qc{frozen, cap, 0u};
-        const TraceOut oc{hits, nullptr, nullptr, nullptr, 1u};
+        TraceOut oc{hits, nullptr, nullptr, nullptr, 1u};
+        oc.class_bit = class_bit;
         tm.begin(1, ps);
         launch_trace2_stream(ctx, ps, scene, false, qc, pq[cur].o, pq[cur].d, oc, ctr->work_closest[r], pp.overflow[0].p, ctr, sc_c);
         tm.end(1, ps);
@@ -259,13 +268,13 @@
         const ShadeStream sst{tags[cur], tags[cur ^ 1], (uint32_t)total_slots};
         if (has_directional_light(scene)) {
             if (scene->dev.tri_tan)
-                hipLaunchKernelGGL((k_shade_path<true, true, true>), dim3(g_shade), dim3(kBlock), 0, ps, scene->dev, dsp, pq[cur], pq[cur ^ 1], sq, cap, hits, terms, ctr, r, 0, max_depth, 1u, sst);
+                hipLaunchKernelGGL((k_shade_path<true, true, true>), dim3(g_shade), dim3(kBlock), 0, ps, scene->dev, dsp, pq[cur], pq[cur ^ 1], sq, cap, hits, terms, ctr, r, 0, max_depth, 1u, class_bit, sst);
             else
-                hipLaunchKernelGGL((k_shade_path<true, false, true>), dim3(g_shade), dim3(kBlock), 0, ps, scene->dev, dsp, pq[cur], pq[cur ^ 1], sq, cap, hits, terms, ctr, r, 0, max_depth, 1u, sst);
+                hipLaunchKernelGGL((k_shade_path<true, false, true>), dim3(g_shade), dim3(kBlock), 0, ps, scene->dev, dsp, pq[cur], pq[cur ^ 1], sq, cap, hits, terms, ctr, r, 0, max_depth, 1u, class_bit, sst);
         } else if (scene->dev.tri_tan) {
-            hipLaunchKernelGGL(k_shade_path<true>, dim3(g_shade), dim3(kBlock), 0, ps, scene->dev, dsp, pq[cur], pq[cur ^ 1], sq, cap, hits, terms, ctr, r, 0, max_depth, 1u, sst);
+            hipLaunchKernelGGL(k_shade_path<true>, dim3(g_shade), dim3(kBlock), 0, ps, scene->dev, dsp, pq[cur], pq[cur ^ 1], sq, cap, hits, terms, ctr, r, 0, max_depth, 1u, class_bit, sst);
         } else {
-            hipLaunchKernelGGL((k_shade_path<true, false>), dim3(g_shade), dim3(kBlock), 0, ps, scene->dev, dsp, pq[cur], pq[cur ^ 1], sq, cap, hits, terms, ctr, r, 0, max_depth, 1u, sst);
+            hipLaunchKernelGGL((k_shade_path<true, false>), dim3(g_shade), dim3(kBlock), 0, ps, scene->dev, dsp, pq[cur], pq[cur ^ 1], sq, cap, hits, terms, ctr, r, 0, max_depth, 1u, class_bit, sst);
         }
         tm.end(2, ps);
         if (ps2 != ps) {
@@ -489,6 +498,7 @@
     HIP_TRY(ctx, hipEventRecord(ev_start, st));
     const int g_shade = ctx->num_cu * 8;
     const uint32_t bary_mode = (ctx->traversal >= 2 && scene->wide_ok) ? 1u : 0u;
+    const uint32_t class_bit = path_class_bit(ctx, scene);
     uint32_t n_batches = 0;
     for (int pi = 0; pi < NP; ++pi) {
         HIP_TRY(ctx, hipStreamWaitEvent(ctx->pipes[pi].st, ev_start, 0));
@@ -515,21 +525,22 @@
         for (int depth = 1; depth <= max_depth; ++depth) {
             const ShadowQueue& sq = sqs[depth & 1];
             tm.begin(1, ps);
-            launch_trace(ctx, ps, scene, false, SegQueue{ctr->n_queue[depth - 1], cap, 0u}, pq[cur].o, pq[cur].d, nullptr,
-                         TraceOut{hits, nullptr, nullptr, nullptr, bary_mode, depth == 1 && far_camera(scene, sensor) ? 1u : 0u}, ctr->work_closest[depth - 1], ctr, pp.overflow[0].p);
+            TraceOut oc{hits, nullptr, nullptr, nullptr, bary_mode, depth == 1 && far_camera(scene, sensor) ? 1u : 0u};
+            oc.class_bit = class_bit;
+            launch_trace(ctx, ps, scene, false, SegQueue{ctr->n_queue[depth - 1], cap, 0u}, pq[cur].o, pq[cur].d, nullptr, oc, ctr->work_closest[depth - 1], ctr, pp.overflow[0].p);
             tm.end(1, ps);
             if (two && depth > 2) HIP_TRY(ctx, hipStreamWaitEvent(ps, ev_anys[depth & 1], 0));
             tm.begin(2, ps);
             const ShadeStream sst{nullptr, nullptr, 0u, two ? (uint8_t*)ctx->poison.p : nullptr};
             if (has_directional_light(scene)) {
                 if (scene->dev.tri_tan)
-                    hipLaunchKernelGGL((k_shade_path<false, true, true>), dim3(g_shade), dim3(kBlock), 0, ps, scene->dev, dsp, pq[cur], pq[cur ^ 1], sq, cap, hits, L, ctr, depth - 1, depth, max_depth, bary_mode, sst);
+                    hipLaunchKernelGGL((k_shade_path<false, true, true>), dim3(g_shade), dim3(kBlock), 0, ps, scene->dev, dsp, pq[cur], pq[cur ^ 1], sq, cap, hits, L, ctr, depth - 1, depth, max_depth, bary_mode, class_bit, sst);
                 else
-                    hipLaunchKernelGGL((k_shade_path<false, false, true>), dim3(g_shade), dim3(kBlock), 0, ps, scene->dev, dsp, pq[cur], pq[cur ^ 1], sq, cap, hits, L, ctr, depth - 1, depth, max_depth, bary_mode, sst);
+                    hipLaunchKernelGGL((k_shade_path<false, false, true>), dim3(g_shade), dim3(kBlock), 0, ps, scene->dev, dsp, pq[cur], pq[cur ^ 1], sq, cap, hits, L, ctr, depth - 1, depth, max_depth, bary_mode, class_bit, sst);
             } else if (scene->dev.tri_tan) {
-                hipLaunchKernelGGL(k_shade_path<false>, dim3(g_shade), dim3(kBlock), 0, ps, scene->dev, dsp, pq[cur], pq[cur ^ 1], sq, cap, hits, L, ctr, depth - 1, depth, max_depth, bary_mode, sst);
+                hipLaunchKernelGGL(k_shade_path<false>, dim3(g_shade), dim3(kBlock), 0, ps, scene->dev, dsp, pq[cur], pq[cur ^ 1], sq, cap, hits, L, ctr, depth - 1, depth, max_depth, bary_mode, class_bit, sst);
             } else {
-                hipLaunchKernelGGL((k_shade_path<false, false>), dim3(g_shade), dim3(kBlock), 0, ps, scene->dev, dsp, pq[cur], pq[cur ^ 1], sq, cap, hits, L, ctr, depth - 1, depth, max_depth, bary_mode, sst);
+                hipLaunchKernelGGL((k_shade_path<false, false>), dim3(g_shade), dim3(kBlock), 0, ps, scene->dev, dsp, pq[cur], pq[cur ^ 1], sq, cap, hits, L, ctr, depth - 1, depth, max_depth, bary_mode, class_bit, sst);
             }
             tm.end(2, ps);
             if (two) {
diff --git a/trace.jl_amd/csrc/tu_scene.hip b/trace.jl_amd/csrc/tu_scene.hip
--- a/trace.jl_amd/csrc/tu_scene.hip
+++ b/trace.jl_amd/csrc/tu_scene.hip
@@ -224,6 +224,10 @@
                 if (s->g->prims[s->g->bvh.order[k]].kind == 1) return true;
     return false;
 }
+bool prim_is_fast(const trhip_scene* s, const HostPrim& p) {
+    const uint32_t mat = p.meta & PRIM_MATERIAL_MASK;
+    return p.kind != 1 && mat != PRIM_NO_MATERIAL && mat < s->g->materials.size() && s->g->materials[mat].set[1].n == 1 && s->g->materials[mat].set[1].lobe[0].kind == LOBE_LAMBERT_R;
+}
 }
 
 int upload_scene(trhip_scene* s) {
@@ -250,7 +254,7 @@
                 prims[3 * k + 1] = make_float4(p.v[3], p.v[4], p.v[5], 0);
                 prims[3 * k + 2] = make_float4(p.v[6], p.v[7], p.v[8], 0);
                 const uint32_t mat = p.meta & PRIM_MATERIAL_MASK;
-                const bool fast = mat != PRIM_NO_MATERIAL && mat < s->g->materials.size() && s->g->materials[mat].set[1].n == 1 && s->g->materials[mat].set[1].lobe[0].kind == LOBE_LAMBERT_R;
+                const bool fast = prim_is_fast(s, p);
                 if (fast) prims[3 * k].w = __builtin_bit_cast(float, p.meta | PRIM_FAST);
                 for (int j = 0; j < 3; ++j) nrm[3 * k + j] = make_float4(p.n[3 * j], p.n[3 * j + 1], p.n[3 * j + 2], fast ? s->g->materials[mat].set[1].lobe[0].r[j] : 0.0f);
             }
@@ -917,7 +921,7 @@
                 aprims[3 * k + 2] = make_float4(0, 0, 0, 0);
                 is_sphere[k] = 1;
             } else {
-                aprims[3 * k] = make_float4(p.v[0], p.v[1], p.v[2], __builtin_bit_cast(float, p.meta));
+                aprims[3 * k] = make_float4(p.v[0], p.v[1], p.v[2], __builtin_bit_cast(float, prim_is_fast(s, p) ? p.meta | PRIM_FAST : p.meta));
                 aprims[3 * k + 1] = make_float4(p.v[3], p.v[4], p.v[5], cs);
                 aprims[3 * k + 2] = make_float4(p.v[6], p.v[7], p.v[8], __builtin_bit_cast(float, order_word[cslot[s->g->acc.order[k]]]));
             }
```

Result: no change. 6149, median of 6 (+0.7%).
